# rsinghlab/GNN-Tumor-Seg

Measured on AMD Instinct MI355X. Metric: supervoxel-graphs/sec training, 7xSAGE-pool-256, 15k-node graphs, higher is better.
Workload: dtype f32; 1 GPU; C2: 7xGraphSAGE-pool-256 (8 SAGEConv), fwd+weighted-CE+bwd+AdamW, 4 x 15000-node/86350-edge lattice graphs per GPU, 4-chan feat, fp32; global_batch=4, nodes_per_batch=60000, edges_per_batch=345400, parallelism=dp1

## Files before the change

### gnn-tumor-seg_amd/csrc/gts_gemm.hip

```cpp
#include "gts_gemm_tiles.h"
#include "gts_gemm_panel.h"
#include "gts_gemm_wgrad.h"
#include "gts_gemm_small.h"

namespace gts {
namespace {

template <bool AKC, bool BKC>
int pick_plain_variant(const GemmArgs& p) {
  int variant = BKC ? g_fwd_variant : g_igrad_variant;
  if (p.rb <= 128 && variant < 9) return 0;
  const bool row_count_invariant = variant == -2;
  if (variant < 0) {
    const int64_t cols = (p.rb + 255) / 256;
    const int64_t big_tiles = static_cast<int64_t>((p.ra + 255) / 256) * cols;
    variant = big_tiles >= 192 ? 8 : 3;
    if constexpr (AKC && BKC) {
      const int h = panel_rows_for(p.ra, cols);
      const int64_t panels = static_cast<int64_t>((p.ra + h - 1) / h) * cols;
      const int64_t rows256 = (big_tiles + 255) / 256 * 256, rows_panel = (panels + 255) / 256 * h;
      if (variant == 8 && rows_panel < rows256 && !row_count_invariant) variant = 10;
      if (variant == 3 && panels >= 192 && panels <= 256 && !row_count_invariant) variant = 10;
    }
  }
  return variant;
}

template <bool BKC>
inline bool skinny_forward(const GemmArgs& p) {
  const bool automatic = BKC ? g_fwd_variant < 0 : g_igrad_variant <= 1;
  return automatic && (p.rb == 4 || p.rb == 8) && p.ldc == p.rb && p.kseg[0] + p.kseg[1] >= 64 && p.mask == nullptr &&
         p.c2 == nullptr && p.sc_l == nullptr && p.bits_out == nullptr &&
         (BKC || (p.ldb[0] == p.rb && (p.kseg[1] == 0 || p.ldb[1] == p.rb)));
}

inline bool tiny_forward(const GemmArgs& p) {
  return (p.rb == 4 || p.rb == 8) && p.ldc == p.rb && p.kseg[0] + p.kseg[1] <= 16 && p.mask == nullptr && p.c2 == nullptr &&
         p.sc_l == nullptr && p.bits_out == nullptr && g_fwd_variant < 0;
}

template <bool AKC, bool BKC>
int launch_plain_tiles(const GemmArgs& p, int variant, hipStream_t st) {
  if constexpr (AKC && BKC) {
    if (tiny_forward(p)) {
      const unsigned blocks = static_cast<unsigned>((p.ra + 255) / 256);
      if (p.rb == 4) tiny_fwd_kernel<4><<<blocks, 256, 0, st>>>(p);
      else tiny_fwd_kernel<8><<<blocks, 256, 0, st>>>(p);
      return launch_status();
    }
  }
  if constexpr (AKC) {
    if (skinny_forward<BKC>(p)) {
      const unsigned blocks = static_cast<unsigned>((p.ra + 15) / 16);
      if (p.rb == 4) skinny_fwd_kernel<4, BKC><<<blocks, 256, 0, st>>>(p);
      else skinny_fwd_kernel<8, BKC><<<blocks, 256, 0, st>>>(p);
      return launch_status();
    }
  }
  if (p.rb <= 64) return launch_tiles<128, 64, 2, 2, AKC, BKC>(p, 1, 1, st);
  if (p.rb <= 128) return launch_tiles<128, 128, 2, 2, AKC, BKC>(p, 1, 1, st);
  switch (variant) {
    case 3: return launch_tiles<64, 256, 2, 4, AKC, BKC>(p, 1, 1, st);
    case 5: return launch_tiles<256, 128, 4, 2, AKC, BKC>(p, 1, 1, st);
    case 8: return launch_tiles<256, 256, 4, 4, AKC, BKC, true>(p, 1, 1, st);
    default: return launch_tiles<128, 256, 2, 4, AKC, BKC>(p, 1, 1, st);
  }
}

template <bool AKC, bool BKC>
int launch_plain(const GemmArgs& p, hipStream_t st) {
  const int variant = pick_plain_variant<AKC, BKC>(p);
  if constexpr (AKC && BKC) {
    if (p.c2 != nullptr && !(variant == 10 && p.rb <= kC240 && p.rb2 <= kC240 && p.rb2 > 128)) {
      GemmArgs first = p, next{};
      first.c2 = nullptr;
      int rc = launch_plain<true, true>(first, st);
      if (rc != GTS_OK) return rc;
      next.a[0] = next.a[1] = p.c, next.b[0] = next.b[1] = p.b2, next.bp[0] = p.bp2;
      first.bp2 = nullptr;
      next.lda[0] = next.lda[1] = p.ldc, next.ldb[0] = next.ldb[1] = p.ldb2;
      next.kseg[0] = p.rb, next.kseg[1] = 0;
      next.ra = p.ra, next.rb = p.rb2, next.c = p.c2, next.ldc = p.ldc2, next.bias = p.bias2, next.relu = p.relu2;
      next.tiles_per_split = (p.rb + kBK - 1) / kBK;
      return launch_plain<true, true>(next, st);
    }
    if (variant == 10) {
      switch (panel_rows_for(p.ra, (p.rb + kC240 - 1) / kC240)) {
        case 144: return launch_panel_direct<3, 4, 1, NoProbe, 144>(p, st);
        case 192: return launch_panel_direct<3, 4, 1, NoProbe, 192>(p, st);
        default: return launch_panel_direct<3, 4, 1>(p, st);
      }
    }
  }
  int rc = launch_plain_tiles<AKC, BKC>(p, variant, st);
  if (rc != GTS_OK || p.bits_out == nullptr) return rc;
  const long long words = static_cast<long long>((p.ra + 3) / 4) * (p.rb >> 6);
  relu_bits_kernel<<<static_cast<unsigned>((words + 3) / 4), 256, 0, st>>>(p.c, p.bits_out, p.ra, p.rb);
  return launch_status();
}

struct PlainProblem {
  const float *a0, *b0, *a1, *b1;
  float* c;
  int64_t m, rb, k0, k1;
  bool missing() const { return !a0 || !b0 || !c || ((a1 == nullptr) != (b1 == nullptr)); }
  bool bad_shape() const {
    return m < 0 || rb <= 0 || k0 <= 0 || k1 < 0 || m >= (1LL << 31) || rb >= (1 << 20) || k0 >= (1 << 20) || k1 >= (1 << 20) ||
           !aligned4(k0) || !aligned4(k1) || (a1 && k1 == 0);
  }
  GemmArgs args(int64_t ldb0, int64_t ldb1, const float* const* packed) const {
    GemmArgs p{};
    p.a[0] = a0, p.b[0] = b0, p.lda[0] = p.kseg[0] = static_cast<int>(k0), p.ldb[0] = static_cast<int>(ldb0);
    p.a[1] = a1 ? a1 : a0, p.b[1] = b1 ? b1 : b0, p.lda[1] = static_cast<int>(k1), p.ldb[1] = static_cast<int>(ldb1);
    p.kseg[1] = a1 ? static_cast<int>(k1) : 0;
    p.ra = static_cast<int>(m), p.rb = static_cast<int>(rb), p.c = c, p.ldc = static_cast<int>(rb);
    p.tiles_per_split = (p.kseg[0] + kBK - 1) / kBK + (p.kseg[1] + kBK - 1) / kBK;
    if (packed != nullptr) p.bp[0] = packed[0], p.bp[1] = a1 ? packed[1] : nullptr;
    return p;
  }
};

void chain_second(GemmArgs* p, const float* b2, const float* bias2, float* c2, int64_t rb2, int relu2,
                  const float* const* packed) {
  p->b2 = b2, p->bias2 = bias2, p->c2 = c2, p->rb2 = static_cast<int>(rb2), p->ldb2 = p->rb;
  p->ldc2 = static_cast<int>(rb2), p->relu2 = relu2;
  if (packed != nullptr) p->bp2 = packed[2];
}

__global__ __launch_bounds__(kBlock) void sum_parts_kernel(const float* __restrict__ in_l, const float* __restrict__ in_r,
                                                           float* __restrict__ out_l, float* __restrict__ out_r,
                                                           int64_t n, int parts) {
  const int64_t i = static_cast<int64_t>(blockIdx.x) * kBlock + threadIdx.x;
  if (i >= n) return;
  float sl = 0.f, sr = 0.f;
  for (int q = 0; q < parts; ++q) sl += in_l[i * parts + q], sr += in_r[i * parts + q];
  out_l[i] = sl, out_r[i] = sr;
}

}
}

extern "C" int32_t gts_linear_fwd_f32(const float* a0, const float* w0, const float* a1, const float* w1, const float* bias,
                                      float* out, int64_t m, int64_t n, int64_t k0, int64_t k1, int32_t relu,
                                      uint64_t* relu_bits, const float* const* packed, void* stream) {
  using namespace gts;
  const PlainProblem q{a0, w0, a1, w1, out, m, n, k0, k1};
  if (q.missing()) return GTS_ERR_NULL;
  if (q.bad_shape() || (relu_bits && n % 64 != 0)) return GTS_ERR_SHAPE;
  if (m == 0) return GTS_OK;
  GemmArgs p = q.args(k0, k1, packed);
  p.bias = bias, p.relu = relu, p.bits_out = reinterpret_cast<unsigned long long*>(relu_bits);
  return launch_plain<true, true>(p, static_cast<hipStream_t>(stream));
}

extern "C" int32_t gts_relu_bits_pay(int64_t m, int64_t n) {
  using namespace gts;
  if (m <= 0 || n <= 0 || n % 64 != 0 || m >= (1LL << 31) || n >= (1 << 20)) return 0;
  GemmArgs p{};
  p.ra = static_cast<int>(m), p.rb = static_cast<int>(n);
  const int variant = pick_plain_variant<true, true>(p);
  return variant >= 10 && variant <= 12 ? 1 : 0;
}

extern "C" int64_t gts_relu_bits_bytes(int64_t m, int64_t n) {
  if (m < 0 || n <= 0 || n % 64 != 0) return 0;
  return (m + 3) / 4 * (n / 64) * 4 * static_cast<int64_t>(sizeof(uint64_t));
}

extern "C" int64_t gts_gat_fc_scores_workspace(int64_t m, int64_t heads, int64_t dim) {
  if (m <= 0 || heads <= 0 || dim <= 0 || dim % 64 != 0) return 0;
  return 2 * m * heads * (dim / 64) * static_cast<int64_t>(sizeof(float));
}

extern "C" int32_t gts_gat_fc_scores_f32(const float* h, const float* w_fc, const float* attn_l, const float* attn_r,
                                         float* ft, float* el, float* er, float* workspace, int64_t workspace_bytes,
                                         int64_t m, int64_t heads, int64_t dim, int64_t k, const float* w_fc_packed,
                                         void* stream) {
  using namespace gts;
  const int64_t n = heads * dim;
  const float* const packed[2] = {w_fc_packed, nullptr};
  const PlainProblem q{h, w_fc, nullptr, nullptr, ft, m, n, k, 0};
  if (q.missing() || !attn_l || !attn_r || !el || !er) return GTS_ERR_NULL;
  if (q.bad_shape() || heads <= 0 || dim <= 0) return GTS_ERR_SHAPE;
  if (m == 0) return GTS_OK;
  GemmArgs p = q.args(k, 0, packed);
  hipStream_t st = static_cast<hipStream_t>(stream);
  const int parts = static_cast<int>(dim / 64);
  const bool fuse = dim % 64 == 0 && pick_plain_variant<true, true>(p) == 10 &&
                    (parts == 1 || (workspace && workspace_bytes >= gts_gat_fc_scores_workspace(m, heads, dim)));
  if (!fuse) {
    const int rc = launch_plain<true, true>(p, st);
    return rc != GTS_OK ? rc : gts_gat_scores_f32(ft, attn_l, attn_r, el, er, m, heads, dim, stream);
  }
  p.sc_l = attn_l, p.sc_r = attn_r;
  p.sc_el = parts == 1 ? el : workspace, p.sc_er = parts == 1 ? er : workspace + m * heads * parts;
  const int rc = launch_plain<true, true>(p, st);
  if (rc != GTS_OK || parts == 1) return rc;
  const int64_t rows = m * heads;
  sum_parts_kernel<<<static_cast<unsigned>((rows + kBlock - 1) / kBlock), kBlock, 0, st>>>(p.sc_el, p.sc_er, el, er, rows, parts);
  return launch_status();
}

extern "C" int32_t gts_linear_fwd_chain_f32(const float* a0, const float* w0, const float* a1, const float* w1,
                                            const float* bias, float* out, const float* w2, const float* bias2, float* out2,
                                            int64_t m, int64_t n, int64_t k0, int64_t k1, int32_t relu, int64_t n2,
                                            int32_t relu2, uint64_t* relu_bits, const float* const* packed, void* stream) {
  using namespace gts;
  const PlainProblem q{a0, w0, a1, w1, out, m, n, k0, k1};
  if (q.missing() || !w2 || !out2) return GTS_ERR_NULL;
  if (q.bad_shape() || n2 <= 0 || n2 >= (1 << 20) || !aligned4(n) || (relu_bits && n % 64 != 0)) return GTS_ERR_SHAPE;
  if (m == 0) return GTS_OK;
  GemmArgs p = q.args(k0, k1, packed);
  p.bias = bias, p.relu = relu, p.bits_out = reinterpret_cast<unsigned long long*>(relu_bits);
  chain_second(&p, w2, bias2, out2, n2, relu2, packed);
  return launch_plain<true, true>(p, static_cast<hipStream_t>(stream));
}

extern "C" int32_t gts_linear_bwd_input_chain_t_f32(const float* g0, const float* w0t, const float* g1, const float* w1t,
                                                    const float* relu_mask, const uint64_t* relu_bits, float* gin,
                                                    const float* w2t, float* gin2, int64_t m, int64_t k, int64_t n0,
                                                    int64_t n1, int64_t k2, const float* const* packed, void* stream) {
  using namespace gts;
  const PlainProblem q{g0, w0t, g1, w1t, gin, m, k, n0, n1};
  if (q.missing() || !w2t || !gin2 || (relu_bits && !relu_mask)) return GTS_ERR_NULL;
  if (q.bad_shape() || k2 <= 0 || k2 >= (1 << 20) || !aligned4(k) || (relu_bits && k % 64 != 0)) return GTS_ERR_SHAPE;
  if (m == 0) return GTS_OK;
  GemmArgs p = q.args(n0, n1, packed);
  p.mask = relu_mask, p.bits_in = reinterpret_cast<const unsigned long long*>(relu_bits);
  chain_second(&p, w2t, nullptr, gin2, k2, 0, packed);
  return launch_plain<true, true>(p, static_cast<hipStream_t>(stream));
}

extern "C" int32_t gts_linear_bwd_input_f32(const float* g0, const float* w0, const float* g1, const float* w1,
                                            const float* relu_mask, float* gin, int64_t m, int64_t k, int64_t n0,
                                            int64_t n1, void* stream) {
  using namespace gts;
  const PlainProblem q{g0, w0, g1, w1, gin, m, k, n0, n1};
  if (q.missing()) return GTS_ERR_NULL;
  if (q.bad_shape() || !aligned4(k)) return GTS_ERR_SHAPE;
  if (m == 0) return GTS_OK;
  GemmArgs p = q.args(k, k, nullptr);
  p.mask = relu_mask;
  return launch_plain<true, false>(p, static_cast<hipStream_t>(stream));
}

extern "C" int32_t gts_linear_bwd_input_t_f32(const float* g0, const float* w0t, const float* g1, const float* w1t,
                                              const float* relu_mask, const uint64_t* relu_bits, float* gin, int64_t m,
                                              int64_t k, int64_t n0, int64_t n1, const float* const* packed, void* stream) {
  using namespace gts;
  const PlainProblem q{g0, w0t, g1, w1t, gin, m, k, n0, n1};
  if (q.missing() || (relu_bits && !relu_mask)) return GTS_ERR_NULL;
  if (q.bad_shape() || !aligned4(k) || (relu_bits && k % 64 != 0)) return GTS_ERR_SHAPE;
  if (m == 0) return GTS_OK;
  GemmArgs p = q.args(n0, n1, packed);
  p.mask = relu_mask, p.bits_in = reinterpret_cast<const unsigned long long*>(relu_bits);
  return launch_plain<true, true>(p, static_cast<hipStream_t>(stream));
}

static bool act_fold_in_epilogue(const gts::GemmArgs& p) {
  return gts::pick_plain_variant<true, true>(p) == 10 && p.rb % gts::kC240 == 0;
}

extern "C" int64_t gts_linear_bwd_input_t_act_workspace(int64_t m, int64_t k) {
  if (m <= 0 || k <= 0) return 0;
  const int64_t row_blocks = (m + 143) / 144 * 3;
  const int64_t pass = gts_gat_reduce_workspace(m, k) / 2;
  const int64_t fold = row_blocks * k * static_cast<int64_t>(sizeof(float));
  return fold > pass ? fold : pass;
}

extern "C" int32_t gts_linear_bwd_input_t_act_f32(const float* g0, const float* w0t, const float* g1, const float* w1t,
                                                  const float* act_out, int32_t activation, float* gin, float* g_bias,
                                                  float* workspace, int64_t workspace_bytes, int64_t m, int64_t k,
                                                  int64_t n0, int64_t n1, const float* const* packed, void* stream) {
  using namespace gts;
  const PlainProblem q{g0, w0t, g1, w1t, gin, m, k, n0, n1};
  if (q.missing() || !act_out || (g_bias && !workspace)) return GTS_ERR_NULL;
  if (activation != 1 && activation != 2) return GTS_ERR_ARGKIND;
  if (q.bad_shape() || !aligned4(k)) return GTS_ERR_SHAPE;
  if (g_bias && workspace_bytes < gts_linear_bwd_input_t_act_workspace(m, k)) return GTS_ERR_SHAPE;
  if (m == 0) return GTS_OK;
  hipStream_t st = static_cast<hipStream_t>(stream);
  GemmArgs p = q.args(n0, n1, packed);
  if (activation == 1 && g_bias && act_fold_in_epilogue(p)) {
    const int rows = panel_rows_for(p.ra, p.rb / kC240);
    const int row_blocks = (p.ra + rows - 1) / rows * 3;
    p.mask = act_out, p.mask_kind = 1, p.col_partial = workspace;
    const int rc = launch_plain<true, true>(p, st);
    if (rc != GTS_OK) return rc;
    return sum_chunks(workspace, g_bias, p.rb, row_blocks, st);
  }
  const int rc = launch_plain<true, true>(p, st);
  if (rc != GTS_OK) return rc;
  return gts_gat_act_bwd_f32(gin, act_out, activation, gin, g_bias, workspace, workspace_bytes, m, k, stream);
}

extern "C" int64_t gts_linear_bwd_weight_workspace(int64_t m, int64_t n, int64_t k, int32_t n_problems) {
  using namespace gts;
  if (m <= 0 || n <= 0 || k <= 0 || n_problems < 1 || n_problems > kMaxProblems) return 0;
  const int64_t splits = wgrad_plan(m, n, k, n_problems).splits;
  const int64_t slabs = n_problems * splits * (n * k + n);
  const int64_t skinny = skinny_workspace_floats(m, n, k) + kSkinnyChunks * (n < k ? n : 0);
  return (slabs > skinny ? slabs : skinny) * static_cast<int64_t>(sizeof(float));
}

extern "C" int32_t gts_linear_bwd_weight_f32(const float* const* g, const float* const* a, float* const* gw,
                                             float* const* gb, int32_t n_problems, float* workspace,
                                             int64_t workspace_bytes, int64_t m, int64_t n, int64_t k, void* stream) {
  using namespace gts;
  if (!g || !a || !gw || !workspace) return GTS_ERR_NULL;
  if (n_problems < 1 || n_problems > kMaxProblems) return GTS_ERR_ARGKIND;
  if (m <= 0 || n <= 0 || k <= 0 || m >= (1LL << 31) || n >= (1 << 20) || k >= (1 << 20) || !aligned4(n) || !aligned4(k))
    return GTS_ERR_SHAPE;
  if (workspace_bytes < gts_linear_bwd_weight_workspace(m, n, k, n_problems)) return GTS_ERR_SHAPE;
  bool any_bias = false;
  for (int q = 0; q < n_problems; ++q) {
    if (!g[q] || !a[q] || !gw[q]) return GTS_ERR_NULL;
    any_bias = any_bias || (gb && gb[q]);
  }
  hipStream_t st = static_cast<hipStream_t>(stream);
  if (skinny_workspace_floats(m, n, k) > 0) {
    for (int q = 0; q < n_problems; ++q)
      skinny_wgrad(g[q], a[q], gw[q], gb ? gb[q] : nullptr, workspace, m, n, k, st);
    return launch_status();
  }
  const WgradPlan plan = wgrad_plan(m, n, k, n_problems);
  const int splits = plan.splits;
  const int tiles = static_cast<int>((m + kBK - 1) / kBK);
  GemmArgs p{};
  for (int q = 0; q < n_problems; ++q) p.pa[q] = g[q], p.pb[q] = a[q];
  p.a[0] = p.a[1] = g[0], p.b[0] = p.b[1] = a[0];
  p.lda[0] = p.lda[1] = static_cast<int>(n), p.ldb[0] = p.ldb[1] = static_cast<int>(k);
  p.kseg[0] = static_cast<int>(m), p.kseg[1] = 0;
  p.ra = static_cast<int>(n), p.rb = static_cast<int>(k);
  p.c = workspace, p.ldc = static_cast<int>(k);
  p.colsum = any_bias ? workspace + static_cast<size_t>(n_problems) * splits * n * k : nullptr;
  for (int q = 0; q < n_problems && any_bias; ++q)
    if (gb[q]) p.colsum_mask |= 1u << q;
  p.n_problems = n_problems, p.n_splits = splits;
  p.tiles_per_split = (tiles + splits - 1) / splits;
  int rc = launch_wgrad(p, plan, st);
  if (rc != GTS_OK) return rc;
  ReduceArgs r{};
  r.splits = splits;
  int jobs = 0;
  for (int q = 0; q < n_problems; ++q, ++jobs) {
    r.slabs[jobs] = workspace + static_cast<size_t>(q) * splits * n * k;
    r.out[jobs] = gw[q], r.n4[jobs] = static_cast<int>(n * k / 4);
  }
  for (int q = 0; q < n_problems && any_bias; ++q) {
    if (!gb[q]) continue;
    r.slabs[jobs] = p.colsum + static_cast<size_t>(q) * splits * n;
    r.out[jobs] = gb[q], r.n4[jobs] = static_cast<int>(n / 4);
    ++jobs;
  }
  reduce_slabs_kernel<<<dim3(static_cast<unsigned>((n * k / 4 + 63) / 64), jobs), kBlock, 0, st>>>(r);
  return launch_status();
}
```

### gnn-tumor-seg_amd/csrc/gts_gemm_args.h

```cpp
#pragma once
#include "gts_common.h"

namespace gts {

inline int g_gemm_sched = 1;
inline int g_fwd_variant = -1;
inline int g_igrad_variant = 1;
inline int g_wgrad_variant = -1;
inline int g_panel_rows = 0;

namespace {

typedef float v16f __attribute__((ext_vector_type(16)));
typedef float v4f __attribute__((ext_vector_type(4)));

constexpr int kBK = 32;
constexpr int kMaxProblems = 32;
constexpr unsigned kOutOfRange = 0x7FFFFFF0u;

struct GemmArgs {
  const float* a[2];
  const float* b[2];
  int lda[2], ldb[2];
  int kseg[2];
  int ra, rb;
  float* c;
  int ldc;
  const float* bias;
  int relu;
  const float* mask;
  const float* pa[kMaxProblems];
  const float* pb[kMaxProblems];
  float* colsum;
  unsigned colsum_mask;
  int n_problems;
  int tiles_n;
  int n_splits;
  int tiles_per_split;
  int sched;
  const float* b2;
  const float* bias2;
  float* c2;
  int rb2, ldb2, ldc2, relu2;
  const float* sc_l;
  const float* sc_r;
  float* sc_el;
  float* sc_er;
  unsigned long long* bits_out;
  const unsigned long long* bits_in;
  int mask_kind;
  float* col_partial;
  const float* bp[2];
  const float* bp2;
};

struct NoProbe {
  __device__ __forceinline__ static void mark(int ) {}
};

inline bool aligned4(int64_t x) { return (x & 3) == 0; }

}
}
```

### gnn-tumor-seg_amd/csrc/gts_gemm_skinny.h

```cpp
#pragma once
#include "gts_gemm_args.h"

namespace gts {
namespace {

constexpr int kSkinnyMax = 9;
constexpr int kSkinnyChunks = 512;

template <int S>
__global__ __launch_bounds__(kBlock) void skinny_wgrad_kernel(const float* __restrict__ skinny, int s_cols,
                                                             const float* __restrict__ wide,
                                                             float* __restrict__ partial, int64_t m,
                                                             int w, int64_t rows_per_chunk) {
  __shared__ v4f red[kBlock];
  const int cols4 = w >> 2;
  const int lanes = cols4 >= kBlock ? 1 : kBlock / cols4;
  const int rl = cols4 >= kBlock ? 0 : threadIdx.x / cols4;
  const int64_t row0 = blockIdx.x * rows_per_chunk, row1 = min(m, row0 + rows_per_chunk);
  for (int q0 = 0; q0 < cols4; q0 += kBlock) {
    const int q = q0 + (cols4 >= kBlock ? threadIdx.x : threadIdx.x % cols4);
    const bool live = q < cols4 && rl < lanes;
    v4f acc[S];
#pragma unroll
    for (int i = 0; i < S; ++i) acc[i] = v4f{0.f, 0.f, 0.f, 0.f};
    if (live) {
#pragma unroll 4
      for (int64_t row = row0 + rl; row < row1; row += lanes) {
        const v4f f = *reinterpret_cast<const v4f*>(wide + static_cast<size_t>(row) * w + 4 * q);
#pragma unroll
        for (int i = 0; i < S; ++i) acc[i] += (i < s_cols ? skinny[row * s_cols + i] : 1.0f) * f;
      }
    }
#pragma unroll
    for (int i = 0; i < S; ++i) {
      v4f total = acc[i];
      if (lanes > 1) {
        __syncthreads();
        red[threadIdx.x] = acc[i];
        __syncthreads();
        if (rl == 0 && live) {
          for (int l = 1; l < lanes; ++l) total += red[l * cols4 + q];
        }
      }
      if (rl == 0 && live)
        *reinterpret_cast<v4f*>(partial + (static_cast<size_t>(blockIdx.x) * S + i) * w + 4 * q) = total;
    }
  }
}

__global__ __launch_bounds__(kBlock) void skinny_sum_kernel(const float* __restrict__ partial,
                                                           float* __restrict__ dst0,
                                                           float* __restrict__ dst1, int rows, int s_cols,
                                                           int w, int chunks, int transposed) {
  __shared__ float part[16][16];
  const int o = threadIdx.x & 15, lane = threadIdx.x >> 4;
  const int idx = blockIdx.x * 16 + o;
  const int total_out = rows * w;
  float acc = 0.f;
  if (idx < total_out) {
#pragma unroll 8
    for (int c = lane; c < chunks; c += 16) acc += partial[static_cast<size_t>(c) * total_out + idx];
  }
  part[lane][o] = acc;
  __syncthreads();
  if (lane != 0 || idx >= total_out) return;
  float sum = part[0][o];
#pragma unroll
  for (int l = 1; l < 16; ++l) sum += part[l][o];
  const int i = idx / w, j = idx - i * w;
  if (i < s_cols)
    dst0[transposed ? j * s_cols + i : i * w + j] = sum;
  else if (dst1 != nullptr)
    dst1[j] = sum;
}

}
}
```

### gnn-tumor-seg_amd/csrc/gts_gemm_wgrad.h

```cpp
#pragma once
#include <type_traits>

#include "gts_gemm_tiles.h"

namespace gts {
namespace {

typedef float v2f __attribute__((ext_vector_type(2)));

template <int O0, int O1>
__device__ __forceinline__ v2f lds_read2st64(unsigned addr) {
  static_assert(O0 >= 0 && O1 <= 255, "ds_read2st64_b32 offsets are 8 bits");
  v2f r;
  asm volatile("ds_read2st64_b32 %0, %1 offset0:%2 offset1:%3" : "=v"(r) : "v"(addr), "n"(O0), "n"(O1));
  return r;
}

template <class Probe = NoProbe>
__global__ __launch_bounds__(1024, 4) void wgrad_stream_kernel(const GemmArgs p) {
  constexpr int BM = 256, BN = 256, WM = 4, WN = 4, WTM = 64, WTN = 64, TM = 2, TN = 2;
  constexpr int kPlane = kBK * BM;
  static_assert(BM == BN && kPlane * 4 == 128 * 256, "image I of an operand sits 128 offset units above image 0");
  __shared__ float lds[4 * kPlane];
  const int lane = threadIdx.x & 63, wave = __builtin_amdgcn_readfirstlane(threadIdx.x >> 6);
  const int wm = wave / WN, wn = wave % WN;
  const int i = lane & 31, h = lane >> 5;
  const int problem = blockIdx.y / p.tiles_n, tile_n = blockIdx.y % p.tiles_n;
  const int m0 = blockIdx.x * BM, n0 = tile_n * BN;
  const float* g = kernarg_entry<const float*>(offsetof(GemmArgs, pa), problem);
  const float* act = kernarg_entry<const float*>(offsetof(GemmArgs, pb), problem);
  const int ldg = p.lda[0], lda = p.ldb[0];
  const int n_tiles_all = (p.kseg[0] + kBK - 1) / kBK;
  const int t_beg = min(n_tiles_all, static_cast<int>(blockIdx.z) * p.tiles_per_split);
  const int t_end = min(n_tiles_all, t_beg + p.tiles_per_split);
  const int row_beg = t_beg * kBK, rows = min(p.kseg[0], t_end * kBK) - row_beg;
  const int n_tiles = t_end - t_beg;
  const bool g_ok = m0 + 4 * lane < p.ra, a_ok = n0 + 4 * lane < p.rb;
  const unsigned vg0 = g_ok ? static_cast<unsigned>(wave * ldg + m0 + 4 * lane) * 4 : kOutOfRange;
  const unsigned vg1 = g_ok ? static_cast<unsigned>((wave + 16) * ldg + m0 + 4 * lane) * 4 : kOutOfRange;
  const unsigned va0 = a_ok ? static_cast<unsigned>(wave * lda + n0 + 4 * lane) * 4 : kOutOfRange;
  const unsigned va1 = a_ok ? static_cast<unsigned>((wave + 16) * lda + n0 + 4 * lane) * 4 : kOutOfRange;
  auto dma = [&](int t, int image) __attribute__((always_inline)) {
    const int r0 = row_beg + t * kBK, nr = min(kBK, rows - t * kBK);
    __amdgpu_buffer_rsrc_t rg = __builtin_amdgcn_make_buffer_rsrc(const_cast<float*>(g + static_cast<size_t>(r0) * ldg), 0,
                                                                  nr * ldg * 4, 0x00020000);
    __amdgpu_buffer_rsrc_t ract = __builtin_amdgcn_make_buffer_rsrc(const_cast<float*>(act + static_cast<size_t>(r0) * lda), 0,
                                                                    nr * lda * 4, 0x00020000);
    float* ia = lds + image * kPlane + wave * BM;
    float* ib = lds + (2 + image) * kPlane + wave * BN;
    __builtin_amdgcn_raw_ptr_buffer_load_lds(rg, ia, 16, vg0, 0, 0, 0);
    __builtin_amdgcn_raw_ptr_buffer_load_lds(rg, ia + 16 * BM, 16, vg1, 0, 0, 0);
    __builtin_amdgcn_raw_ptr_buffer_load_lds(ract, ib, 16, va0, 0, 0, 0);
    __builtin_amdgcn_raw_ptr_buffer_load_lds(ract, ib + 16 * BN, 16, va1, 0, 0, 0);
  };

  v16f acc[TM][TN];
#pragma unroll
  for (int tm = 0; tm < TM; ++tm)
#pragma unroll
    for (int tn = 0; tn < TN; ++tn)
#pragma unroll
      for (int r = 0; r < 16; ++r) acc[tm][tn][r] = 0.f;
  float csum[TM] = {0.f, 0.f};
  const bool want_colsum = p.colsum != nullptr && tile_n == 0 && wn == wm && ((p.colsum_mask >> problem) & 1u) != 0;

  const unsigned lds0 = static_cast<unsigned>(reinterpret_cast<uintptr_t>((__attribute__((address_space(3))) float*)lds));
  const unsigned a_addr0 = lds0 + static_cast<unsigned>(4 * h * BM + wm * WTM + i) * 4, a_addr1 = a_addr0 + 128;
  const unsigned b_addr0 = lds0 + static_cast<unsigned>(2 * kPlane + 4 * h * BN + wn * WTN + i) * 4, b_addr1 = b_addr0 + 128;
  v2f fa[2][TM], fb[2][TN];
  fa[0][0] = fa[0][1] = fa[1][0] = fa[1][1] = v2f{0.f, 0.f};
  fb[0][0] = fb[0][1] = fb[1][0] = fb[1][1] = v2f{0.f, 0.f};

  auto issue = [&](auto img_c, auto pair_c) __attribute__((always_inline)) {
    constexpr int IMG = decltype(img_c)::value, Q = decltype(pair_c)::value;
    constexpr int O = 4 * (8 * (Q / 2) + 2 * (Q % 2)) + 128 * IMG;
    fa[Q & 1][0] = lds_read2st64<O, O + 4>(a_addr0);
    fa[Q & 1][1] = lds_read2st64<O, O + 4>(a_addr1);
    fb[Q & 1][0] = lds_read2st64<O, O + 4>(b_addr0);
    fb[Q & 1][1] = lds_read2st64<O, O + 4>(b_addr1);
  };
  auto multiply = [&](int slot) __attribute__((always_inline)) {
#pragma unroll
    for (int e = 0; e < 2; ++e)
#pragma unroll
      for (int tm = 0; tm < TM; ++tm)
#pragma unroll
        for (int tn = 0; tn < TN; ++tn)
          acc[tm][tn] = __builtin_amdgcn_mfma_f32_32x32x2f32(fa[slot][tm][e], fb[slot][tn][e], acc[tm][tn], 0, 0, 0);
  };
  float half_sum[TM] = {0.f, 0.f};
  auto tile = [&](auto img_c, auto cs_c, int t) __attribute__((always_inline)) {
    constexpr int IMG = decltype(img_c)::value;
    constexpr bool CS = decltype(cs_c)::value;
    auto pair = [&](auto pair_c) __attribute__((always_inline)) {
      constexpr int Q = decltype(pair_c)::value, S = Q & 1;
      if constexpr (Q < 7) {
        issue(img_c, std::integral_constant<int, Q + 1>{});
        asm volatile("s_waitcnt lgkmcnt(4)" : "+v"(fa[S][0]), "+v"(fa[S][1]), "+v"(fb[S][0]), "+v"(fb[S][1]));
      } else {
        asm volatile("s_waitcnt vmcnt(0) lgkmcnt(0)\n\ts_barrier"
                     : "+v"(fa[S][0]), "+v"(fa[S][1]), "+v"(fb[S][0]), "+v"(fb[S][1]) : : "memory");
        if (t + 2 < n_tiles) dma(t + 2, IMG);
        if (t + 1 < n_tiles) issue(std::integral_constant<int, IMG ^ 1>{}, std::integral_constant<int, 0>{});
      }
      if constexpr (Q % 2 == 0) {
        if constexpr (Q == 0) __builtin_amdgcn_s_setprio(3);
        else if constexpr (Q == 2) __builtin_amdgcn_s_setprio(2);
        else if constexpr (Q == 4) __builtin_amdgcn_s_setprio(1);
        else __builtin_amdgcn_s_setprio(0);
      }
      if constexpr (CS) {
#pragma unroll
        for (int tm = 0; tm < TM; ++tm) {
          if constexpr (Q % 2 == 0) {
            asm volatile("v_add_f32 %0, %1, %2" : "=v"(half_sum[tm]) : "v"(fa[S][tm][0]), "v"(fa[S][tm][1]));
          } else {
            float upper;
            asm volatile("v_add_f32 %0, %1, %2" : "=v"(upper) : "v"(fa[S][tm][0]), "v"(fa[S][tm][1]));
            asm volatile("v_add_f32 %0, %1, %2" : "=v"(upper) : "v"(half_sum[tm]), "v"(upper));
            asm volatile("v_add_f32 %0, %1, %2" : "+v"(csum[tm]) : "v"(csum[tm]), "v"(upper));
          }
        }
      }
      multiply(S);
    };
    pair(std::integral_constant<int, 0>{}), pair(std::integral_constant<int, 1>{}), pair(std::integral_constant<int, 2>{}),
        pair(std::integral_constant<int, 3>{}), pair(std::integral_constant<int, 4>{}), pair(std::integral_constant<int, 5>{}),
        pair(std::integral_constant<int, 6>{}), pair(std::integral_constant<int, 7>{});
  };
  auto reduce = [&](auto cs_c) __attribute__((always_inline)) {
    int t = 0;
    for (; t + 1 < n_tiles; t += 2) {
      tile(std::integral_constant<int, 0>{}, cs_c, t);
      tile(std::integral_constant<int, 1>{}, cs_c, t + 1);
    }
    if (t < n_tiles) tile(std::integral_constant<int, 0>{}, cs_c, t);
  };

  Probe::mark(0);
  if (n_tiles > 0) {
    dma(0, 0);
    if (n_tiles > 1) dma(1, 1);
    asm volatile("s_waitcnt vmcnt(0)\n\ts_barrier" ::: "memory");
    issue(std::integral_constant<int, 0>{}, std::integral_constant<int, 0>{});
  }
  Probe::mark(1);
  if (want_colsum) reduce(std::true_type{});
  else reduce(std::false_type{});
  __builtin_amdgcn_s_setprio(0);
  Probe::mark(2);
  const size_t slab = static_cast<size_t>(problem) * p.n_splits + blockIdx.z;
  write_tile<BM, BN, WM, WN>(p, lds, p.c + slab * p.ra * p.ldc, acc, m0, n0);
  Probe::mark(3);
  if (want_colsum) {
#pragma unroll
    for (int tm = 0; tm < TM; ++tm) {
      const float total = csum[tm] + __shfl_xor(csum[tm], 32, kWave);
      const int row = m0 + wm * WTM + tm * 32 + i;
      if (h == 0 && row < p.ra) p.colsum[slab * p.ra + row] = total;
    }
  }
}

struct ReduceArgs {
  const float* slabs[2 * kMaxProblems];
  float* out[2 * kMaxProblems];
  int n4[2 * kMaxProblems];
  int splits;
};

__global__ __launch_bounds__(kBlock) void reduce_slabs_kernel(const ReduceArgs p) {
  __shared__ v4f part[4][64];
  const int col = threadIdx.x & 63, grp = threadIdx.x >> 6;
  const int q = blockIdx.y;
  const float* slabs = kernarg_entry<const float*>(offsetof(ReduceArgs, slabs), q);
  float* out = kernarg_entry<float*>(offsetof(ReduceArgs, out), q);
  const int n4 = kernarg_entry<int>(offsetof(ReduceArgs, n4), q);
  const int i = blockIdx.x * 64 + col;
  if (blockIdx.x * 64 >= n4) return;
  v4f acc = {0.f, 0.f, 0.f, 0.f};
  if (i < n4) {
    const v4f* src = reinterpret_cast<const v4f*>(slabs) + i;
#pragma unroll 8
    for (int s = grp; s < p.splits; s += 4) acc += src[static_cast<size_t>(s) * n4];
  }
  part[grp][col] = acc;
  __syncthreads();
  if (grp == 0 && i < n4) {
    const v4f total = (part[0][col] + part[1][col]) + (part[2][col] + part[3][col]);
    reinterpret_cast<v4f*>(out)[i] = total;
  }
}

}
}
#include "gts_gemm_skinny.h"
namespace gts {
namespace {

inline int64_t skinny_workspace_floats(int64_t m, int64_t n, int64_t k) {
  const int64_t small = n < k ? n : k, big = n < k ? k : n;
  if (small + 1 > kSkinnyMax || big < 64) return 0;
  return static_cast<int64_t>(kSkinnyChunks) * (small + 1) * big;
}

template <int S>
void launch_skinny(const float* skinny, int s_cols, const float* wide, float* partial, int64_t m, int w,
                   int chunks, int64_t rpc, hipStream_t st) {
  skinny_wgrad_kernel<S><<<chunks, kBlock, 0, st>>>(skinny, s_cols, wide, partial, m, w, rpc);
}

inline bool skinny_wgrad(const float* g, const float* a, float* gw, float* gb, float* workspace, int64_t m,
                  int64_t n, int64_t k, hipStream_t st) {
  if (skinny_workspace_floats(m, n, k) == 0) return false;
  const bool g_is_skinny = n < k;
  const float* skinny = g_is_skinny ? g : a;
  const float* wide = g_is_skinny ? a : g;
  const int s_cols = static_cast<int>(g_is_skinny ? n : k), w = static_cast<int>(g_is_skinny ? k : n);
  const bool ones_row = !g_is_skinny && gb != nullptr;
  const int rows = s_cols + (ones_row ? 1 : 0);
  const int64_t rpc = (m + kSkinnyChunks - 1) / kSkinnyChunks;
  const int chunks = static_cast<int>((m + rpc - 1) / rpc);
  switch (rows) {
    case 1: launch_skinny<1>(skinny, s_cols, wide, workspace, m, w, chunks, rpc, st); break;
    case 2: launch_skinny<2>(skinny, s_cols, wide, workspace, m, w, chunks, rpc, st); break;
    case 3: launch_skinny<3>(skinny, s_cols, wide, workspace, m, w, chunks, rpc, st); break;
    case 4: launch_skinny<4>(skinny, s_cols, wide, workspace, m, w, chunks, rpc, st); break;
    case 5: launch_skinny<5>(skinny, s_cols, wide, workspace, m, w, chunks, rpc, st); break;
    case 6: launch_skinny<6>(skinny, s_cols, wide, workspace, m, w, chunks, rpc, st); break;
    case 7: launch_skinny<7>(skinny, s_cols, wide, workspace, m, w, chunks, rpc, st); break;
    case 8: launch_skinny<8>(skinny, s_cols, wide, workspace, m, w, chunks, rpc, st); break;
    default: launch_skinny<9>(skinny, s_cols, wide, workspace, m, w, chunks, rpc, st); break;
  }
  skinny_sum_kernel<<<(rows * w + 15) / 16, kBlock, 0, st>>>(
      workspace, gw, ones_row ? gb : nullptr, rows, s_cols, w, chunks, g_is_skinny ? 0 : 1);
  if (g_is_skinny && gb != nullptr) {
    float* part = workspace + static_cast<size_t>(chunks) * rows * w;
    skinny_wgrad_kernel<1><<<chunks, kBlock, 0, st>>>(nullptr, 0, g, part, m, static_cast<int>(n), rpc);
    skinny_sum_kernel<<<(static_cast<int>(n) + 15) / 16, kBlock, 0, st>>>(
        part, nullptr, gb, 1, 0, static_cast<int>(n), chunks, 0);
  }
  return true;
}

struct WgradPlan {
  int variant, bm, bn, splits;
};

inline void wgrad_candidate(int variant, int64_t k, int* bm, int* bn, int64_t* slots) {
  *bm = 128, *bn = k <= 64 ? 64 : 128, *slots = 512;
  if (k <= 64) return;
  if (variant == 2) *bn = 256;
  if (variant == 4 || variant == 6) *bm = 256, *bn = 256, *slots = 256;
}

inline WgradPlan wgrad_plan(int64_t m, int64_t n, int64_t k, int n_problems) {
  const int64_t tiles = (m + kBK - 1) / kBK;
  static const int kMany[2] = {6, 2};
  static const int kFewLarge[2] = {6, 1};
  const bool few = n_problems <= 4;
  const bool large = n * k * n_problems >= (1 << 20);
  const int n_candidates = g_wgrad_variant >= 0 || (few && !large) ? 1 : 2;
  WgradPlan best{};
  double best_fill = -1.0;
  for (int c = 0; c < n_candidates; ++c) {
    WgradPlan plan{};
    plan.variant = g_wgrad_variant >= 0 ? g_wgrad_variant : (few ? (large ? kFewLarge[c] : 1) : kMany[c]);
    int64_t slots;
    wgrad_candidate(plan.variant, k, &plan.bm, &plan.bn, &slots);
    const int64_t out_tiles = ((n + plan.bm - 1) / plan.bm) * ((k + plan.bn - 1) / plan.bn) * n_problems;
    int64_t splits = out_tiles >= slots ? 1 : slots / out_tiles;
    if (splits > tiles) splits = tiles;
    plan.splits = static_cast<int>(splits < 1 ? 1 : splits);
    const int64_t groups = out_tiles * plan.splits;
    const int64_t rounds = (groups + slots - 1) / slots;
    const double fill = static_cast<double>(groups) / static_cast<double>(rounds * slots);
    if (fill > best_fill + 1e-9) best = plan, best_fill = fill;
  }
  return best;
}

inline int launch_wgrad(const GemmArgs& p, const WgradPlan& plan, hipStream_t st) {
  const int np = p.n_problems, splits = plan.splits;
  if (p.rb <= 64) return launch_tiles<128, 64, 2, 2, false, false>(p, np, splits, st);
  switch (plan.variant) {
    case 2: return launch_tiles<128, 256, 2, 4, false, false>(p, np, splits, st);
    case 4: return launch_tiles<256, 256, 4, 4, false, false, true>(p, np, splits, st);
    case 6: {
      GemmArgs q = p;
      q.tiles_n = (p.rb + 255) / 256;
      dim3 grid((p.ra + 255) / 256, q.tiles_n * np, splits);
      wgrad_stream_kernel<><<<grid, 1024, 0, st>>>(q);
      return launch_status();
    }
    default: return launch_tiles<128, 128, 2, 4, false, false>(p, np, splits, st);
  }
}

}
}
```

### gnn-tumor-seg_amd/csrc/gts_narrow.hip

```cpp
#include "gts_gemm_skinny.h"

namespace gts {
namespace {

constexpr int kFirstW = 256, kFirstS = 4;

__global__ __launch_bounds__(kBlock) void first_layer_bwd_kernel(const float* __restrict__ g, const float* __restrict__ x,
                                                                const float* __restrict__ m0,
                                                                const float* __restrict__ w_neigh, float* __restrict__ gm,
                                                                float* __restrict__ part_x, float* __restrict__ part_m,
                                                                int64_t m, int64_t rows_per_chunk) {
  constexpr int W = kFirstW, S = kFirstS;
  __shared__ v4f red[kWavesPerBlock - 1][2 * S + 1][kWave];
  const int lane = threadIdx.x & (kWave - 1), rl = threadIdx.x / kWave;
  const int64_t row0 = blockIdx.x * rows_per_chunk, row1 = min(m, row0 + rows_per_chunk);
  v4f wn[S];
#pragma unroll
  for (int e = 0; e < 4; ++e) {
    const v4f t = *reinterpret_cast<const v4f*>(w_neigh + static_cast<size_t>(4 * lane + e) * S);
#pragma unroll
    for (int j = 0; j < S; ++j) wn[j][e] = t[j];
  }
  v4f ax[S + 1], am[S];
#pragma unroll
  for (int i = 0; i <= S; ++i) ax[i] = v4f{0.f, 0.f, 0.f, 0.f};
#pragma unroll
  for (int i = 0; i < S; ++i) am[i] = v4f{0.f, 0.f, 0.f, 0.f};
  const bool upper32 = (lane & 32) != 0, upper16 = (lane & 16) != 0;
  auto take_row = [&](int64_t row, const v4f f, const v4f xs, const v4f ms) __attribute__((always_inline)) {
#pragma unroll
    for (int i = 0; i < S; ++i) ax[i] += xs[i] * f;
    ax[S] += 1.0f * f;
#pragma unroll
    for (int i = 0; i < S; ++i) am[i] += ms[i] * f;
    float d[S];
#pragma unroll
    for (int n = 0; n < S; ++n) {
      d[n] = 0.f;
#pragma unroll
      for (int e = 0; e < 4; ++e) d[n] = __builtin_fmaf(f[e], wn[n][e], d[n]);
    }
    const float keep0 = upper32 ? d[2] : d[0], keep1 = upper32 ? d[3] : d[1];
    const float send0 = upper32 ? d[0] : d[2], send1 = upper32 ? d[1] : d[3];
    const float a = keep0 + __shfl_xor(send0, 32, kWave), b = keep1 + __shfl_xor(send1, 32, kWave);
    float c = (upper16 ? b : a) + __shfl_xor(upper16 ? a : b, 16, kWave);
#pragma unroll
    for (int o = 8; o > 0; o >>= 1) c += __shfl_xor(c, o, kWave);
    if ((lane & 15) == 0) gm[static_cast<size_t>(row) * S + (lane >> 4)] = c;
  };
  constexpr int kAhead = 4;
  for (int64_t first = row0 + rl; first < row1; first += kAhead * kWavesPerBlock) {
    v4f f[kAhead], xs[kAhead], ms[kAhead];
#pragma unroll
    for (int u = 0; u < kAhead; ++u) {
      const int64_t row = first + u * kWavesPerBlock < row1 ? first + u * kWavesPerBlock : first;
      f[u] = *reinterpret_cast<const v4f*>(g + static_cast<size_t>(row) * W + 4 * lane);
      xs[u] = *reinterpret_cast<const v4f*>(x + static_cast<size_t>(row) * S);
      ms[u] = *reinterpret_cast<const v4f*>(m0 + static_cast<size_t>(row) * S);
    }
#pragma unroll
    for (int u = 0; u < kAhead; ++u)
      if (first + u * kWavesPerBlock < row1) take_row(first + u * kWavesPerBlock, f[u], xs[u], ms[u]);
  }
  if (rl > 0) {
#pragma unroll
    for (int i = 0; i <= S; ++i) red[rl - 1][i][lane] = ax[i];
#pragma unroll
    for (int i = 0; i < S; ++i) red[rl - 1][S + 1 + i][lane] = am[i];
  }
  __syncthreads();
  if (rl != 0) return;
#pragma unroll
  for (int i = 0; i <= S; ++i) {
    v4f total = ax[i];
    for (int l = 1; l < kWavesPerBlock; ++l) total += red[l - 1][i][lane];
    *reinterpret_cast<v4f*>(part_x + (static_cast<size_t>(blockIdx.x) * (S + 1) + i) * W + 4 * lane) = total;
  }
#pragma unroll
  for (int i = 0; i < S; ++i) {
    v4f total = am[i];
    for (int l = 1; l < kWavesPerBlock; ++l) total += red[l - 1][S + 1 + i][lane];
    *reinterpret_cast<v4f*>(part_m + (static_cast<size_t>(blockIdx.x) * S + i) * W + 4 * lane) = total;
  }
}

inline bool first_layer_shape(int64_t m, int64_t w, int64_t s0, int64_t s1) {
  return m > 0 && m < (1LL << 31) && w == kFirstW && s0 == kFirstS && s1 == kFirstS;
}

}
}

extern "C" int64_t gts_sage_first_layer_bwd_workspace(int64_t m, int64_t w, int64_t s0, int64_t s1) {
  using namespace gts;
  if (!first_layer_shape(m, w, s0, s1)) return 0;
  return static_cast<int64_t>(kSkinnyChunks) * (s0 + 1 + s1) * w * static_cast<int64_t>(sizeof(float));
}

extern "C" int32_t gts_sage_first_layer_bwd_f32(const float* g, const float* x, const float* m0, const float* w_neigh,
                                                float* gm, float* gw_self, float* g_bias, float* gw_neigh,
                                                float* workspace, int64_t workspace_bytes, int64_t m, int64_t w,
                                                int64_t s0, int64_t s1, void* stream) {
  using namespace gts;
  if (!g || !x || !m0 || !w_neigh || !gm || !gw_self || !g_bias || !gw_neigh || !workspace) return GTS_ERR_NULL;
  if (!first_layer_shape(m, w, s0, s1)) return GTS_ERR_SHAPE;
  if (workspace_bytes < gts_sage_first_layer_bwd_workspace(m, w, s0, s1)) return GTS_ERR_SHAPE;
  hipStream_t st = static_cast<hipStream_t>(stream);
  const int64_t rpc = (m + kSkinnyChunks - 1) / kSkinnyChunks;
  const int chunks = static_cast<int>((m + rpc - 1) / rpc);
  const int W = kFirstW, S = kFirstS;
  float* part_x = workspace;
  float* part_m = workspace + static_cast<size_t>(chunks) * (S + 1) * W;
  first_layer_bwd_kernel<<<chunks, kBlock, 0, st>>>(g, x, m0, w_neigh, gm, part_x, part_m, m, rpc);
  skinny_sum_kernel<<<((S + 1) * W + 15) / 16, kBlock, 0, st>>>(part_x, gw_self, g_bias, S + 1, S, W, chunks, 1);
  skinny_sum_kernel<<<(S * W + 15) / 16, kBlock, 0, st>>>(part_m, gw_neigh, nullptr, S, S, W, chunks, 1);
  return launch_status();
}
```

### gnn-tumor-seg_amd/csrc/gts_optim.hip

```cpp
#include "gts_common.h"

namespace gts {
namespace {

typedef float v4f __attribute__((ext_vector_type(4)));

struct AdamWConsts {
  float decay;
  float w1;
  float beta2, w2;
  float step_size;
  float inv_bc2_sqrt_den;
  float eps;
};

__device__ __forceinline__ void adamw_one(float& p, float g, float& m, float& v, const AdamWConsts& c) {
  p = p * c.decay;
  m = m + c.w1 * (g - m);
  v = c.beta2 * v + c.w2 * (g * g);
  const float denom = sqrtf(v) / c.inv_bc2_sqrt_den + c.eps;
  p = p - c.step_size * (m / denom);
}

__global__ __launch_bounds__(kBlock) void adamw_kernel(float* __restrict__ param,
                                                      const float* __restrict__ grad,
                                                      float* __restrict__ exp_avg,
                                                      float* __restrict__ exp_avg_sq, int64_t n,
                                                      AdamWConsts c, int vector_ok) {
  const int64_t n4 = vector_ok ? n / 4 : 0;
  for (int64_t q = static_cast<int64_t>(blockIdx.x) * kBlock + threadIdx.x; q < n4;
       q += static_cast<int64_t>(gridDim.x) * kBlock) {
    v4f p = reinterpret_cast<v4f*>(param)[q];
    const v4f g = reinterpret_cast<const v4f*>(grad)[q];
    v4f m = reinterpret_cast<v4f*>(exp_avg)[q];
    v4f v = reinterpret_cast<v4f*>(exp_avg_sq)[q];
#pragma unroll
    for (int e = 0; e < 4; ++e) {
      float pe = p[e], me = m[e], ve = v[e];
      adamw_one(pe, g[e], me, ve, c);
      p[e] = pe, m[e] = me, v[e] = ve;
    }
    reinterpret_cast<v4f*>(param)[q] = p;
    reinterpret_cast<v4f*>(exp_avg)[q] = m;
    reinterpret_cast<v4f*>(exp_avg_sq)[q] = v;
  }
  for (int64_t i = 4 * n4 + static_cast<int64_t>(blockIdx.x) * kBlock + threadIdx.x; i < n;
       i += static_cast<int64_t>(gridDim.x) * kBlock)
    adamw_one(param[i], grad[i], exp_avg[i], exp_avg_sq[i], c);
}

}
}

extern "C" int32_t gts_adamw_f32(float* param, const float* grad, float* exp_avg, float* exp_avg_sq,
                                 int64_t n, double lr, double beta1, double beta2, double eps,
                                 double weight_decay, int64_t step, void* stream) {
  using namespace gts;
  if (n < 0 || step < 1 || !(beta1 >= 0.0 && beta1 < 1.0) || !(beta2 >= 0.0 && beta2 < 1.0))
    return GTS_ERR_SHAPE;
  if (n == 0) return GTS_OK;
  if (!param || !grad || !exp_avg || !exp_avg_sq) return GTS_ERR_NULL;
  const double bc1 = 1.0 - pow(beta1, static_cast<double>(step));
  const double bc2 = 1.0 - pow(beta2, static_cast<double>(step));
  AdamWConsts c;
  c.decay = static_cast<float>(1.0 - lr * weight_decay);
  c.w1 = static_cast<float>(1.0 - beta1);
  c.beta2 = static_cast<float>(beta2);
  c.w2 = static_cast<float>(1.0 - beta2);
  c.step_size = static_cast<float>(lr / bc1);
  c.inv_bc2_sqrt_den = static_cast<float>(sqrt(bc2));
  c.eps = static_cast<float>(eps);
  const int vector_ok = ((reinterpret_cast<uintptr_t>(param) | reinterpret_cast<uintptr_t>(grad) |
                          reinterpret_cast<uintptr_t>(exp_avg) | reinterpret_cast<uintptr_t>(exp_avg_sq)) & 15) == 0;
  int64_t blocks = (n / 4 + kBlock - 1) / kBlock;
  blocks = blocks < 1 ? 1 : (blocks > 4096 ? 4096 : blocks);
  adamw_kernel<<<static_cast<unsigned>(blocks), kBlock, 0, static_cast<hipStream_t>(stream)>>>(
      param, grad, exp_avg, exp_avg_sq, n, c, vector_ok);
  return launch_status();
}
```

### gnn-tumor-seg_amd/csrc/gts_stack.hip

```cpp
#include <algorithm>
#include <vector>

#include "gts_gemm_args.h"

namespace {

constexpr int kMaxLayers = 64;

inline int64_t align256(int64_t bytes) { return (bytes + 255) & ~255LL; }

inline bool bad_stack(int64_t n_rows, const int64_t* widths, int32_t n_layers) {
  if (!widths || n_layers < 1 || n_layers > kMaxLayers || n_rows < 0 || n_rows >= (1LL << 31)) return true;
  for (int i = 0; i <= n_layers; ++i)
    if (widths[i] <= 0 || widths[i] % 4 != 0 || widths[i] >= (1 << 20)) return true;
  return false;
}

struct FwdPlan {
  int64_t m[kMaxLayers], arg[kMaxLayers], out[kMaxLayers], bits[kMaxLayers];
  int64_t p[2];
  int64_t wp[kMaxLayers][3];
  int64_t counters;
  int64_t total;
};

inline bool packs(int64_t out_cols) { return out_cols > 128; }

inline FwdPlan plan_forward(int64_t n, const int64_t* w, int n_layers, bool training, int arg_bytes, bool relu_bits) {
  FwdPlan p{};
  int64_t at = 0, widest = 0;
  auto take = [&](int64_t bytes) { const int64_t o = at; at += align256(bytes); return o; };
  for (int i = 0; i < n_layers; ++i) {
    const bool last = i == n_layers - 1;
    widest = std::max(widest, w[i]);
    p.m[i] = take(4 * n * w[i]);
    p.arg[i] = training ? take(static_cast<int64_t>(arg_bytes) * n * w[i]) : -1;
    p.out[i] = take(4 * n * w[i + 1]);
    const bool bits = relu_bits && training && !last && gts_relu_bits_pay(n, w[i + 1]) == 1;
    p.bits[i] = bits ? take(gts_relu_bits_bytes(n, w[i + 1])) : -1;
  }
  p.p[0] = take(4 * n * widest);
  p.p[1] = take(4 * n * widest);
  for (int i = 0; i < n_layers; ++i) {
    p.wp[i][0] = packs(w[i]) ? take(4 * gts_packed_weight_floats(w[i], w[i])) : -1;
    p.wp[i][1] = packs(w[i + 1]) ? take(4 * gts_packed_weight_floats(w[i + 1], w[i])) : -1;
    p.wp[i][2] = packs(w[i + 1]) ? take(4 * gts_packed_weight_floats(w[i + 1], w[i])) : -1;
  }
  p.counters = take(4 * GTS_CLUSTER_COUNTER_WORDS);
  p.total = at;
  return p;
}

inline bool chainable(int64_t n, int64_t k0, int64_t k1, int64_t n2) {
  return n % 4 == 0 && k0 % 4 == 0 && k1 % 4 == 0 && n <= 256 && n2 <= 256;
}

inline bool turns(int64_t rows, int64_t cols) { return cols >= 128 && rows % 4 == 0 && cols % 4 == 0; }

struct BwdPlan {
  int64_t wt[kMaxLayers][3];
  int64_t wtp[kMaxLayers][3];
  int64_t g[kMaxLayers], gp[kMaxLayers];
  int64_t gm[2];
  int64_t workspace, workspace_bytes;
  bool first_fused;
  int64_t counters;
  int64_t total;
};

struct ByShape {
  struct Group {
    int64_t rows, cols;
    std::vector<const float*> in[2];
    std::vector<float*> out[2];
    int count() const { return static_cast<int>(in[0].size()); }
  };
  std::vector<Group> groups;
  void add(int64_t rows, int64_t cols, const float* in0, const float* in1, float* out0, float* out1) {
    auto it = std::find_if(groups.begin(), groups.end(), [&](const Group& c) { return c.rows == rows && c.cols == cols; });
    if (it == groups.end()) it = groups.insert(it, Group{rows, cols, {}, {}});
    it->in[0].push_back(in0), it->in[1].push_back(in1), it->out[0].push_back(out0), it->out[1].push_back(out1);
  }
};

constexpr int kWeightSlot[3] = {0, 2, 3};
inline int64_t weight_rows(const int64_t* w, int i, int q) { return q == 0 ? w[i] : w[i + 1]; }

inline BwdPlan plan_backward(int64_t n, const int64_t* w, int n_layers) {
  BwdPlan p{};
  int64_t at = 0, widest = 0;
  auto take = [&](int64_t bytes) { const int64_t o = at; at += align256(bytes); return o; };
  ByShape wgrads;
  for (int i = 0; i < n_layers; ++i) {
    const int64_t fin = w[i];
    widest = std::max(widest, fin);
    for (int q = 0; q < 3; ++q) p.wt[i][q] = turns(weight_rows(w, i, q), fin) ? take(4 * weight_rows(w, i, q) * fin) : -1;
    for (int q = 0; q < 3; ++q)
      p.wtp[i][q] = p.wt[i][q] >= 0 ? take(4 * gts_packed_weight_floats(fin, weight_rows(w, i, q))) : -1;
    p.g[i] = i > 0 ? take(4 * n * fin) : -1;
    p.gp[i] = take(4 * n * fin);
    for (int q = 0; q < 3; ++q) wgrads.add(weight_rows(w, i, q), fin, nullptr, nullptr, nullptr, nullptr);
  }
  p.gm[0] = take(4 * n * widest);
  p.gm[1] = take(4 * n * widest);
  int64_t ws = 0;
  if (n > 0)
    for (const auto& grp : wgrads.groups)
      for (int first = 0; first < grp.count(); first += gts::kMaxProblems)
        ws = std::max(ws, gts_linear_bwd_weight_workspace(n, grp.rows, grp.cols, std::min(gts::kMaxProblems, grp.count() - first)));
  const int64_t first = n > 0 ? gts_sage_first_layer_bwd_workspace(n, w[1], w[0], w[0]) : 0;
  p.first_fused = first > 0;
  ws = std::max(ws, first);
  p.workspace_bytes = ws;
  p.workspace = take(ws);
  p.counters = take(4 * GTS_CLUSTER_COUNTER_WORDS);
  p.total = at;
  return p;
}

inline int32_t zero_counters(const int32_t* sched_rec, int64_t clusters, int32_t rows, int32_t srcs, int32_t loc_words,
                             int32_t backward, void* at, void* stream, uint32_t** counters) {
  *counters = nullptr;
  if (sched_rec == nullptr || gts_cluster_uses_counters(clusters, rows, srcs, loc_words, backward) == 0) return GTS_OK;
  if (hipMemsetAsync(at, 0, 4 * GTS_CLUSTER_COUNTER_WORDS, static_cast<hipStream_t>(stream)) != hipSuccess) return gts::launch_status();
  *counters = static_cast<uint32_t*>(at);
  return GTS_OK;
}

#define GTS_TRY(call)                    \
  do {                                   \
    const int32_t code_ = (call);        \
    if (code_ != GTS_OK) return code_;   \
  } while (0)

}

extern "C" int64_t gts_sage_pool_stack_fwd_arena(int64_t n_rows, const int64_t* widths, int32_t n_layers, int32_t training,
                                                 int32_t arg_bytes, int32_t relu_bits, int64_t* offsets) {
  if (bad_stack(n_rows, widths, n_layers) || (training && arg_bytes != 1 && arg_bytes != 4)) return -1;
  const FwdPlan p = plan_forward(n_rows, widths, n_layers, training != 0, arg_bytes, relu_bits != 0);
  if (offsets != nullptr) {
    for (int i = 0; i < n_layers; ++i)
      offsets[4 * i] = p.m[i], offsets[4 * i + 1] = p.arg[i], offsets[4 * i + 2] = p.out[i], offsets[4 * i + 3] = p.bits[i];
    offsets[4 * n_layers] = p.p[0], offsets[4 * n_layers + 1] = p.p[1];
  }
  return p.total;
}

extern "C" int32_t gts_sage_pool_stack_fwd_f32(const int32_t* indptr, const int32_t* indices, const int32_t* sched_rec,
                                               int64_t sched_clusters, int32_t sched_rows, int32_t sched_srcs,
                                               int32_t sched_loc_words, const float* x, const float* const* params,
                                               int64_t n_rows, const int64_t* widths, int32_t n_layers, int32_t training,
                                               int32_t arg_bytes, int32_t relu_bits, void* arena, int64_t arena_bytes,
                                               void* stream) {
  if (!indptr || !x || !params || !arena) return GTS_ERR_NULL;
  if (bad_stack(n_rows, widths, n_layers)) return GTS_ERR_SHAPE;
  if (training && arg_bytes != 1 && arg_bytes != 4) return GTS_ERR_ARGKIND;
  for (int i = 0; i < 5 * n_layers; ++i)
    if (!params[i]) return GTS_ERR_NULL;
  const bool train = training != 0;
  const FwdPlan plan = plan_forward(n_rows, widths, n_layers, train, arg_bytes, relu_bits != 0);
  if (arena_bytes < plan.total) return GTS_ERR_SHAPE;
  if (n_rows == 0) return GTS_OK;
  char* base = static_cast<char*>(arena);
  auto f32 = [&](int64_t off) { return reinterpret_cast<float*>(base + off); };
  uint32_t* counters;
  GTS_TRY(zero_counters(sched_rec, sched_clusters, sched_rows, sched_srcs, sched_loc_words, 0, base + plan.counters, stream, &counters));
  {
    ByShape packs;
    for (int i = 0; i < n_layers; ++i)
      for (int q = 0; q < 3; ++q)
        if (plan.wp[i][q] >= 0)
          packs.add(weight_rows(widths, i, q), widths[i], params[5 * i + kWeightSlot[q]], nullptr, f32(plan.wp[i][q]), nullptr);
    for (const auto& b : packs.groups)
      GTS_TRY(gts_pack_weights_f32(b.in[0].data(), b.out[0].data(), nullptr, b.count(), b.rows, b.cols, 0, stream));
  }
  auto wp = [&](int i, int q) -> const float* { return plan.wp[i][q] >= 0 ? f32(plan.wp[i][q]) : nullptr; };
  const float* h = x;
  float* p = nullptr;
  int cur = 0;
  for (int i = 0; i < n_layers; ++i) {
    const float* w_pool = params[5 * i];
    const float* b_pool = params[5 * i + 1];
    const float* w_self = params[5 * i + 2];
    const float* w_neigh = params[5 * i + 3];
    const float* bias = params[5 * i + 4];
    const int64_t fin = widths[i], fout = widths[i + 1];
    const bool last = i == n_layers - 1;
    if (p == nullptr) {
      p = f32(plan.p[cur]);
      const float* packed[2] = {wp(i, 0), nullptr};
      GTS_TRY(gts_linear_fwd_f32(h, w_pool, nullptr, nullptr, b_pool, p, n_rows, fin, fin, 0, 1, nullptr, packed, stream));
    }
    float* m = f32(plan.m[i]);
    void* arg = train ? static_cast<void*>(base + plan.arg[i]) : nullptr;
    const int ab = train ? arg_bytes : 0;
    if (sched_rec != nullptr && fin == 256 && ab != 4 && n_rows * 1024 < (1LL << 32)) {
      GTS_TRY(gts_spmm_max_fwd_cluster_f32(sched_rec, sched_clusters, sched_rows, sched_srcs, sched_loc_words, p, m, arg, ab,
                                           1, n_rows, fin, counters, stream));
    } else {
      GTS_TRY(gts_spmm_max_fwd_f32(indptr, indices, p, m, arg, ab, 1, n_rows, fin, stream));
    }
    uint64_t* bits = plan.bits[i] >= 0 ? reinterpret_cast<uint64_t*>(base + plan.bits[i]) : nullptr;
    float* out = f32(plan.out[i]);
    if (!last && chainable(fout, fin, fin, fout)) {
      float* p_next = f32(plan.p[cur ^ 1]);
      const float* packed[3] = {wp(i, 1), wp(i, 2), wp(i + 1, 0)};
      GTS_TRY(gts_linear_fwd_chain_f32(h, w_self, m, w_neigh, bias, out, params[5 * (i + 1)], params[5 * (i + 1) + 1], p_next,
                                       n_rows, fout, fin, fin, 1, fout, 1, bits, packed, stream));
      p = p_next, cur ^= 1;
    } else {
      const float* packed[2] = {wp(i, 1), wp(i, 2)};
      GTS_TRY(gts_linear_fwd_f32(h, w_self, m, w_neigh, bias, out, n_rows, fout, fin, fin, last ? 0 : 1, bits, packed, stream));
      p = nullptr;
    }
    h = out;
  }
  return GTS_OK;
}

extern "C" int64_t gts_sage_pool_stack_bwd_scratch(int64_t n_rows, const int64_t* widths, int32_t n_layers,
                                                   int32_t ) {
  if (bad_stack(n_rows, widths, n_layers)) return -1;
  return plan_backward(n_rows, widths, n_layers).total;
}

extern "C" int32_t gts_sage_pool_stack_bwd_f32(const int32_t* t_indptr, const int32_t* t_indices, const int32_t* t_slot,
                                               const int32_t* sched_rec, int64_t sched_clusters, int32_t sched_rows,
                                               int32_t sched_srcs, int32_t sched_loc_words, const float* gout, const float* x,
                                               const float* const* params, int64_t n_rows, const int64_t* widths,
                                               int32_t n_layers, int32_t arg_bytes, int32_t relu_bits, const void* fwd_arena,
                                               float* const* grads, float* gx, void* scratch, int64_t scratch_bytes,
                                               void* stream) {
  if (!t_indptr || !gout || !x || !params || !fwd_arena || !grads || !scratch) return GTS_ERR_NULL;
  if (bad_stack(n_rows, widths, n_layers)) return GTS_ERR_SHAPE;
  if (arg_bytes != 1 && arg_bytes != 4) return GTS_ERR_ARGKIND;
  for (int i = 0; i < 5 * n_layers; ++i)
    if (!params[i] || !grads[i]) return GTS_ERR_NULL;
  hipStream_t st = static_cast<hipStream_t>(stream);
  if (n_rows == 0) {
    for (int i = 0; i < n_layers; ++i) {
      const int64_t fin = widths[i], fout = widths[i + 1];
      const int64_t sizes[5] = {fin * fin, fin, fout * fin, fout * fin, fout};
      for (int q = 0; q < 5; ++q)
        if (hipMemsetAsync(grads[5 * i + q], 0, 4 * sizes[q], st) != hipSuccess) return gts::launch_status();
    }
    return GTS_OK;
  }
  const FwdPlan fwd = plan_forward(n_rows, widths, n_layers, true, arg_bytes, relu_bits != 0);
  const BwdPlan plan = plan_backward(n_rows, widths, n_layers);
  if (scratch_bytes < plan.total) return GTS_ERR_SHAPE;
  const char* acts = static_cast<const char*>(fwd_arena);
  char* base = static_cast<char*>(scratch);
  auto f32 = [&](int64_t off) { return reinterpret_cast<float*>(base + off); };
  uint32_t* counters;
  GTS_TRY(zero_counters(sched_rec, sched_clusters, sched_rows, sched_srcs, sched_loc_words, 1, base + plan.counters, stream, &counters));
  auto act = [&](int64_t off) { return reinterpret_cast<const float*>(acts + off); };
  auto input_of = [&](int i) { return i == 0 ? x : act(fwd.out[i - 1]); };

  {
    ByShape turned;
    for (int i = 0; i < n_layers; ++i)
      for (int q = 0; q < 3; ++q)
        if (plan.wt[i][q] >= 0)
          turned.add(weight_rows(widths, i, q), widths[i], params[5 * i + kWeightSlot[q]], nullptr, f32(plan.wt[i][q]),
                     f32(plan.wtp[i][q]));
    for (const auto& b : turned.groups)
      GTS_TRY(gts_pack_weights_f32(b.in[0].data(), b.out[1].data(), b.out[0].data(), b.count(), b.rows, b.cols, 1, stream));
  }
  auto wt = [&](int i, int q) -> const float* { return plan.wt[i][q] >= 0 ? f32(plan.wt[i][q]) : nullptr; };
  auto wtp = [&](int i, int q) -> const float* { return plan.wtp[i][q] >= 0 ? f32(plan.wtp[i][q]) : nullptr; };

  auto igrad = [&](const float* g0, const float* w0, const float* w0t, int64_t n0, const float* g1, const float* w1,
                   const float* w1t, int64_t n1, const float* relu_mask, const uint64_t* relu_bits, float* gin,
                   int64_t k, const float* w0tp, const float* w1tp) -> int32_t {
    if (w0t != nullptr && (g1 == nullptr || w1t != nullptr)) {
      const float* packed[2] = {w0tp, g1 ? w1tp : nullptr};
      return gts_linear_bwd_input_t_f32(g0, w0t, g1, g1 ? w1t : nullptr, relu_mask, relu_mask ? relu_bits : nullptr, gin,
                                        n_rows, k, n0, g1 ? n1 : 0, packed, stream);
    }
    return gts_linear_bwd_input_f32(g0, w0, g1, g1 ? w1 : nullptr, relu_mask, gin, n_rows, k, n0, g1 ? n1 : 0, stream);
  };

  ByShape wgrads;

  const float* g = gout;
  const float* gm = nullptr;
  int cur = 0;
  for (int i = n_layers - 1; i >= 0; --i) {
    const float* w_pool = params[5 * i];
    const float* w_self = params[5 * i + 2];
    const float* w_neigh = params[5 * i + 3];
    const int64_t fin = widths[i], fout = widths[i + 1];
    const float* h = input_of(i);
    const float* m = act(fwd.m[i]);
    const void* arg = acts + fwd.arg[i];
    const bool fused = i == 0 && plan.first_fused && gm == nullptr;
    const bool lowrank = i == n_layers - 1 && gm == nullptr && fout == 4 && fin == 256 && arg_bytes == 1;
    if (fused) {
      float* buf = f32(plan.gm[cur]);
      GTS_TRY(gts_sage_first_layer_bwd_f32(g, h, m, w_neigh, buf, grads[2], grads[4], grads[3], f32(plan.workspace),
                                           plan.workspace_bytes, n_rows, fout, fin, fin, stream));
      gm = buf;
    } else if (gm == nullptr && !lowrank) {
      float* buf = f32(plan.gm[cur]);
      GTS_TRY(igrad(g, w_neigh, wt(i, 2), fout, nullptr, nullptr, nullptr, 0, nullptr, nullptr, buf, fin, wtp(i, 2), nullptr));
      gm = buf;
    }
    float* gp = f32(plan.gp[i]);
    if (lowrank) {
      GTS_TRY(gts_spmm_max_bwd_lowrank_f32(t_indptr, t_indices, t_slot, g, w_neigh, arg, arg_bytes, gp, n_rows, fin, fout, stream));
    } else if (sched_rec != nullptr && fin == 256 && arg_bytes == 1 && n_rows * 1024 < (1LL << 32)) {
      GTS_TRY(gts_spmm_max_bwd_cluster_f32(sched_rec, sched_clusters, sched_rows, sched_srcs, sched_loc_words, gm, arg, 1, gp,
                                           n_rows, fin, counters, stream));
    } else {
      GTS_TRY(gts_spmm_max_bwd_f32(t_indptr, t_indices, t_slot, gm, arg, arg_bytes, nullptr, gp, n_rows, fin, stream));
    }
    gm = nullptr;
    wgrads.add(fin, fin, gp, h, grads[5 * i], grads[5 * i + 1]);
    if (!fused) {
      wgrads.add(fout, fin, g, h, grads[5 * i + 2], grads[5 * i + 4]);
      wgrads.add(fout, fin, g, m, grads[5 * i + 3], nullptr);
    }
    if (i > 0) {
      const int64_t below_in = widths[i - 1];
      const uint64_t* hbits = fwd.bits[i - 1] >= 0 ? reinterpret_cast<const uint64_t*>(acts + fwd.bits[i - 1]) : nullptr;
      float* g_next = f32(plan.g[i]);
      const float* below_t = wt(i - 1, 2);
      if (wt(i, 1) && wt(i, 0) && below_t && chainable(fin, fout, fin, below_in)) {
        float* gm_next = f32(plan.gm[cur ^ 1]);
        const float* packed[3] = {wtp(i, 1), wtp(i, 0), wtp(i - 1, 2)};
        GTS_TRY(gts_linear_bwd_input_chain_t_f32(g, wt(i, 1), gp, wt(i, 0), h, hbits, g_next, below_t, gm_next, n_rows, fin,
                                                 fout, fin, below_in, packed, stream));
        gm = gm_next, cur ^= 1;
      } else {
        GTS_TRY(igrad(g, w_self, wt(i, 1), fout, gp, w_pool, wt(i, 0), fin, h, hbits, g_next, fin, wtp(i, 1), wtp(i, 0)));
      }
      g = g_next;
    } else if (gx != nullptr) {
      GTS_TRY(igrad(g, w_self, wt(i, 1), fout, gp, w_pool, wt(i, 0), fin, nullptr, nullptr, gx, fin, wtp(i, 1), wtp(i, 0)));
    }
  }
  for (const auto& grp : wgrads.groups)
    for (int first = 0; first < grp.count(); first += gts::kMaxProblems)
      GTS_TRY(gts_linear_bwd_weight_f32(grp.in[0].data() + first, grp.in[1].data() + first, grp.out[0].data() + first,
                                        grp.out[1].data() + first, std::min(gts::kMaxProblems, grp.count() - first),
                                        f32(plan.workspace), plan.workspace_bytes, n_rows, grp.rows, grp.cols, stream));
  return GTS_OK;
}
```

### gnn-tumor-seg_amd/gts/dist.py

```python
import os

import torch
import torch.distributed as dist


COLLECTIVE_TIMER = None


def world():
    if dist.is_available() and dist.is_initialized():
        return dist.get_rank(), dist.get_world_size()
    return 0, 1


def init_from_env(backend=None):
    world_size = int(os.environ.get("WORLD_SIZE", "1"))
    rank = int(os.environ.get("RANK", "0"))
    local_rank = int(os.environ.get("LOCAL_RANK", "0"))
    use_gpu = torch.cuda.is_available()
    if use_gpu:
        local_rank = local_rank % torch.cuda.device_count()
        torch.cuda.set_device(local_rank)
    if world_size > 1 and not dist.is_initialized():
        os.environ.setdefault("MASTER_ADDR", "127.0.0.1")
        os.environ.setdefault("MASTER_PORT", "29500")
        os.environ.setdefault("HSA_ENABLE_IPC_MODE_LEGACY", "0")
        backend = backend or os.environ.get("GTS_DIST_BACKEND") or ("nccl" if use_gpu else "gloo")
        kwargs = {}
        if use_gpu and backend == "nccl":
            kwargs["device_id"] = torch.device("cuda", local_rank)
        dist.init_process_group(backend, rank=rank, world_size=world_size, **kwargs)
    return rank, world_size, local_rank


def shard_indices(perm, step, per_rank, rank, world_size, costs=None):
    g = per_rank * world_size
    chunk = list(perm[step * g:(step + 1) * g])
    if costs is None or world_size == 1:
        return chunk[rank::world_size]
    order = sorted(range(len(chunk)), key=lambda k: (-costs[chunk[k]], k))
    load, held = [0] * world_size, [[] for _ in range(world_size)]
    for k in order:
        r = min((r for r in range(world_size) if len(held[r]) < per_rank), key=lambda r: (load[r], r))
        held[r].append(k)
        load[r] += costs[chunk[k]]
    return [chunk[k] for k in sorted(held[rank])]


def sample_costs(dataset):
    indices = None
    while hasattr(dataset, "dataset") and hasattr(dataset, "indices"):
        own = list(dataset.indices)
        indices = own if indices is None else [own[i] for i in indices]
        dataset = dataset.dataset
    fn = getattr(dataset, "sample_costs", None)
    if fn is None:
        return None
    costs = list(fn())
    return costs if indices is None else [costs[i] for i in indices]


def rank_share(n_items):
    rank, w = world()
    return list(range(rank, n_items, w))


def gather_rows_in_order(n_items, mine):
    _, w = world()
    if w == 1:
        everyone = [mine]
    else:
        everyone = [None] * w
        dist.all_gather_object(everyone, mine)
    rows = {}
    for part in everyone:
        rows.update(part)
    missing = [i for i in range(n_items) if i not in rows]
    if missing:
        raise RuntimeError(f"items {missing[:8]} were evaluated by no rank")
    return [rows[i] for i in range(n_items)]


def broadcast_object(obj, src=0):
    if world()[1] == 1:
        return obj
    box = [obj]
    dist.broadcast_object_list(box, src=src)
    return box[0]


def assert_same_layout(params, what="parameters"):
    rank, w = world()
    if w == 1:
        return
    mine = [tuple(p.shape) for p in params]
    everyone = [None] * w
    dist.all_gather_object(everyone, mine)
    bad = [r for r, shapes in enumerate(everyone) if shapes != everyone[0]]
    if bad:
        raise RuntimeError(f"{what} differ between ranks: rank 0 holds {len(everyone[0])} tensors, "
                           f"ranks {bad} hold {[len(everyone[r]) for r in bad]} (or other shapes); "
                           "build the model from ONE set of hyper-parameters (gts.dist.broadcast_object)")


def broadcast_parameters(params, src=0):
    params = list(params)
    assert_same_layout(params)
    for p in params:
        dist.broadcast(p.data, src=src)


class FlatGradSync:

    def __init__(self, params, group=None):
        self.params = [p for p in params if p.requires_grad]
        if not self.params:
            raise ValueError("no trainable parameters")
        dev = self.params[0].device
        for p in self.params:
            if p.dtype != torch.float32 or p.device != dev:
                raise ValueError("FlatGradSync needs fp32 parameters on one device")
        self.n_grad = sum(p.numel() for p in self.params)
        self.group = group
        self.flat = None
        self._scalars = None
        self._sink = None

    def flat_gradients(self):
        if self.flat is None:
            raise RuntimeError("call all_reduce_and_normalise() first")
        return self.flat[:self.n_grad]

    def zero_grad(self):
        for p in self.params:
            p.grad = None

    def weighted_ce_backward(self, logits, labels, class_weights, cross_entropy_sum=None):
        if cross_entropy_sum is not None:
            num, den = cross_entropy_sum(logits, labels, class_weights)
            num.backward()
            self._scalars = (den.detach().reshape(1), num.detach().reshape(1))
            return
        from . import nn, ops
        grad, stats = ops.weighted_ce_numerator_grad(logits, labels, class_weights)
        if self._sink is None:
            self._sink = nn.GradSink(self.params, extra=2)
        self._sink.new_buffer()
        with nn.grad_sink(self._sink):
            logits.backward(grad)
        self._scalars = (stats[1:2], stats[0:1])

    def empty_step(self, device=None):
        for p in self.params:
            p.grad = None
        if self._sink is not None:
            self._sink.filled = False
        zeros = torch.zeros(2, dtype=torch.float32, device=device or self.params[0].device)
        self._scalars = (zeros[0:1], zeros[1:2])

    def all_reduce_and_normalise(self):
        if self._scalars is None:
            raise RuntimeError("call weighted_ce_backward() first")
        if self._sink is not None and self._sink.filled:
            self.flat = self._sink.flat
            self.flat[self.n_grad:self.n_grad + 1].copy_(self._scalars[0])
            self.flat[self.n_grad + 1:].copy_(self._scalars[1])
            self._sink.filled = False
        else:
            pieces = [(p.grad if p.grad is not None else torch.zeros_like(p)).reshape(-1) for p in self.params]
            self.flat = torch.cat(pieces + [t.to(pieces[0].dtype) for t in self._scalars])
        self._scalars = None
        _, w = world()
        if w > 1:
            reduce = lambda: dist.all_reduce(self.flat, op=dist.ReduceOp.SUM, group=self.group)
            if COLLECTIVE_TIMER is not None:
                COLLECTIVE_TIMER(reduce)
            else:
                reduce()
        den = self.flat[self.n_grad]
        loss = self.flat[self.n_grad + 1] / den
        self.flat[:self.n_grad].div_(den)
        off = 0
        for p in self.params:
            p.grad = self.flat[off:off + p.numel()].view_as(p)
            off += p.numel()
        return loss
```

### gnn-tumor-seg_amd/gts/nn.py

```python
import os

import torch
import torch.nn as nn
import torch.nn.functional as F

from . import dense, ops
from .graph import _DeviceSchedule


class GraphError(RuntimeError):
    """Counterpart of dgl.DGLError for the checks the layers make."""


def _is_relu(fn):
    return fn in (F.relu, torch.relu, torch.nn.functional.relu)


class _SagePoolLayer(torch.autograd.Function):

    @staticmethod
    def forward(ctx, g, h, w_pool, b_pool, w_self, w_neigh, bias, relu_out, need_bwd):
        h = h.contiguous()
        p = dense.linear_fwd(h, w_pool, bias=b_pool, relu=True)
        m, arg = ops.spmm_max_fwd(g, p, want_arg=need_bwd, relu_input=True)
        out = dense.linear_fwd(h, w_self, m, w_neigh, bias=bias, relu=relu_out)
        if need_bwd:
            ctx.g, ctx.relu_out = g, relu_out
            ctx.save_for_backward(h, m, arg, out if relu_out else None, w_pool, w_self, w_neigh)
        return out

    @staticmethod
    def backward(ctx, gout):
        h, m, arg, out, w_pool, w_self, w_neigh = ctx.saved_tensors
        if not ctx.relu_out:
            g = gout.contiguous()
        elif out.shape[1] % 4 == 0 and out.shape[0] > 0:
            g, _ = ops.gat_act_bwd(gout.contiguous(), out, 2, want_bias_grad=False)
        else:
            g = dense.relu_bwd(gout, out)
        need = ctx.needs_input_grad
        gm = dense.linear_bwd_input(g, w_neigh)
        gp = ops.spmm_max_bwd(ctx.g, gm, arg)
        g_ws, g_wn, g_wp, g_bias, g_bp = _pool_layer_weight_grads(g, gp, h, m, w_pool, w_self)
        gh = dense.linear_bwd_input(g, w_self, gp, w_pool) if need[1] else None
        return None, gh, g_wp, g_bp, g_ws, g_wn, g_bias, None, None


class _SageSumLayer(torch.autograd.Function):

    @staticmethod
    def forward(ctx, g, h, w_self, w_neigh, bias, mode, relu_out, need_bwd):
        h = h.contiguous()
        d = g.dev()
        fin, fout = w_neigh.shape[1], w_neigh.shape[0]
        lin_first = fin > fout
        div = d.deg_clamped if mode == "mean" else d.deg_plus1
        src = dense.linear_fwd(h, w_neigh) if lin_first else h
        neigh = ops.spmm_sum_raw(g, src, div_out=div, add_self=(mode == "gcn"))
        last_w = _identity(fout, h.device) if lin_first else w_neigh
        if w_self is not None:
            out = dense.linear_fwd(h, w_self, neigh, last_w, bias=bias, relu=relu_out)
        else:
            out = dense.linear_fwd(neigh, last_w, bias=bias, relu=relu_out)
        if need_bwd:
            ctx.g, ctx.mode, ctx.relu_out, ctx.lin_first = g, mode, relu_out, lin_first
            ctx.has_bias = bias is not None
            ctx.save_for_backward(h, neigh if not lin_first else None, out if relu_out else None, w_self, w_neigh)
        return out

    @staticmethod
    def backward(ctx, gout):
        h, neigh, out, w_self, w_neigh = ctx.saved_tensors
        g, mode = ctx.g, ctx.mode
        d = g.dev()
        div = d.deg_clamped if mode == "mean" else d.deg_plus1
        need = ctx.needs_input_grad
        g_pre, g_bias = ops.gat_act_bwd(gout.contiguous(), out, 2 if ctx.relu_out else 0, want_bias_grad=ctx.has_bias)

        def reduce_bwd(t, accum=None):
            return ops.spmm_sum_raw(g, t, transposed=True, div_in=div, add_self=(mode == "gcn"), accum=accum)

        g_ws = None
        if ctx.lin_first:
            gt = reduce_bwd(g_pre)
            if w_self is not None:
                (g_ws, _), (g_wn, _) = dense.linear_bwd_weight_multi([(g_pre, h, False), (gt, h, False)])
                gh = dense.linear_bwd_input(g_pre, w_self, gt, w_neigh) if need[1] else None
            else:
                g_wn, _ = dense.linear_bwd_weight(gt, h)
                gh = dense.linear_bwd_input(gt, w_neigh) if need[1] else None
        else:
            if w_self is not None:
                (g_ws, _), (g_wn, _) = dense.linear_bwd_weight_multi([(g_pre, h, False), (g_pre, neigh, False)])
            else:
                g_wn, _ = dense.linear_bwd_weight(g_pre, neigh)
            gh = None
            if need[1]:
                gneigh = dense.linear_bwd_input(g_pre, w_neigh)
                gself = dense.linear_bwd_input(g_pre, w_self) if w_self is not None else None
                gh = reduce_bwd(gneigh, accum=gself)
        return None, gh, g_ws, g_wn, g_bias, None, None, None


_identities = {}


def _identity(n, device):
    key = (n, device)
    if key not in _identities:
        _identities[key] = torch.eye(n, dtype=torch.float32, device=device)
    return _identities[key]


RELU_MASK_BITS = os.environ.get("GTS_RELU_BITS", "1") != "0"


def _chainable(a0, w0, a1, w2):
    n, k0, k1, n2 = w0.shape[0], a0.shape[1], a1.shape[1], w2.shape[0]
    return n % 4 == 0 and k0 % 4 == 0 and k1 % 4 == 0 and n <= 256 and n2 <= 256 and w2.shape[1] == n


def _pool_layer_weight_grads(g, gp, h, m, w_pool, w_self):
    if w_pool.shape == w_self.shape:
        (g_ws, g_bias), (g_wn, _), (g_wp, g_bp) = dense.linear_bwd_weight_multi(
            [(g, h, True), (g, m, False), (gp, h, True)])
    else:
        (g_ws, g_bias), (g_wn, _) = dense.linear_bwd_weight_multi([(g, h, True), (g, m, False)])
        g_wp, g_bp = dense.linear_bwd_weight(gp, h, want_bias_grad=True)
    return g_ws, g_wn, g_wp, g_bias, g_bp


def _pack_by_shape(weights, transposed, want_plain=False):
    by_shape, plain, fragment = {}, {}, {}
    for w in weights:
        by_shape.setdefault(tuple(w.shape), []).append(w)
    for ws in by_shape.values():
        copies = dense.pack_weights(ws, transposed=transposed, want_plain=want_plain)
        if want_plain:
            plain.update((id(w), wt) for w, wt in zip(ws, copies[0]))
            copies = copies[1]
        fragment.update((id(w), wp) for w, wp in zip(ws, copies))
    return (plain, fragment) if want_plain else fragment


class _SagePoolStack(torch.autograd.Function):

    @staticmethod
    def forward(ctx, g, x, need_bwd, *params):
        n_layers = len(params) // 5
        h = x.contiguous()
        saved = []
        hbits = None
        p = None
        fragment = _pack_by_shape([w for i in range(n_layers) for w in (params[5 * i], params[5 * i + 2], params[5 * i + 3])
                                   if w.shape[0] > 128 and w.shape[1] % 4 == 0], transposed=False)
        for i in range(n_layers):
            w_pool, b_pool, w_self, w_neigh, bias = params[5 * i:5 * i + 5]
            last = i == n_layers - 1
            if p is None:
                p = dense.linear_fwd(h, w_pool, bias=b_pool, relu=True, packed=(fragment.get(id(w_pool)), None))
            m, arg = ops.spmm_max_fwd(g, p, want_arg=need_bwd, relu_input=True)
            p = None
            nxt = params[5 * (i + 1):5 * (i + 1) + 2] if not last else None
            obits = dense.relu_bits_empty(h.shape[0], w_self.shape[0], h.device) \
                if RELU_MASK_BITS and need_bwd and not last and dense.relu_bits_pay(h.shape[0], w_self.shape[0]) else None
            if nxt is not None and _chainable(h, w_self, m, nxt[0]):
                out, p = dense.linear_fwd_chain(h, w_self, m, w_neigh, bias, True, nxt[0], nxt[1], True, relu_bits=obits,
                                                packed=(fragment.get(id(w_self)), fragment.get(id(w_neigh)), fragment.get(id(nxt[0]))))
            else:
                out = dense.linear_fwd(h, w_self, m, w_neigh, bias=bias, relu=not last, relu_bits=obits,
                                       packed=(fragment.get(id(w_self)), fragment.get(id(w_neigh))))
            saved += [h, m, arg, hbits]
            h, hbits = out, obits
        if need_bwd:
            ctx.g, ctx.n_layers = g, n_layers
            ctx.save_for_backward(*saved, *params)
        return h

    @staticmethod
    def backward(ctx, gout):
        n = ctx.n_layers
        tensors = ctx.saved_tensors
        acts, params = tensors[:4 * n], tensors[4 * n:]
        grads = [None] * (5 * n)
        g = gout.contiguous()
        gx = None
        deferred = {}

        turned, turned_fragment = _pack_by_shape(
            [w for w in (params[5 * i + j] for i in range(n) for j in (0, 2, 3))
             if w.shape[1] >= 128 and w.shape[0] % 4 == 0 and w.shape[1] % 4 == 0], transposed=True, want_plain=True)

        def igrad(g0, w0, g1=None, w1=None, relu_mask=None, relu_bits=None):
            if id(w0) in turned and (w1 is None or id(w1) in turned) and g0.is_contiguous():
                return dense.linear_bwd_input_t(g0, turned[id(w0)], g1, turned[id(w1)] if w1 is not None else None,
                                                relu_mask=relu_mask, relu_bits=relu_bits,
                                                packed=(turned_fragment[id(w0)], turned_fragment[id(w1)] if w1 is not None else None))
            return dense.linear_bwd_input(g0, w0, g1, w1, relu_mask=relu_mask)

        def defer(grad_out, act, slot, bias_slot):
            key = (grad_out.shape[1], act.shape[1])
            deferred.setdefault(key, []).append((grad_out, act, bias_slot is not None, slot, bias_slot))

        gm = None
        for i in reversed(range(n)):
            h, m, arg, hbits = acts[4 * i:4 * i + 4]
            w_pool, _b_pool, w_self, w_neigh, _bias = params[5 * i:5 * i + 5]
            narrow = gm is None and not ops.INSTRUMENTED
            fused = narrow and i == 0 and dense.first_layer_bwd_applies(g, h, m, w_neigh)
            if fused:
                gm, grads[2], grads[4], grads[3] = dense.sage_first_layer_bwd(g, h, m, w_neigh)
            elif narrow and i == n - 1 and ops.lowrank_bwd_applies(g, w_neigh, arg):
                gp = ops.spmm_max_bwd_lowrank(ctx.g, g, w_neigh, arg)
            elif gm is None:
                gm = igrad(g, w_neigh)
            if gm is not None:
                gp = ops.spmm_max_bwd(ctx.g, gm, arg)
            gm = None
            defer(gp, h, 5 * i, 5 * i + 1)
            if not fused:
                defer(g, h, 5 * i + 2, 5 * i + 4)
                defer(g, m, 5 * i + 3, None)
            if i > 0:
                below = params[5 * (i - 1) + 3]
                if all(id(w) in turned for w in (w_self, w_pool, below)) and _chainable(g, w_self.t(), gp, below.t()):
                    g, gm = dense.linear_bwd_input_chain_t(g, turned[id(w_self)], gp, turned[id(w_pool)], h,
                                                           turned[id(below)], relu_bits=hbits,
                                                           packed=(turned_fragment[id(w_self)], turned_fragment[id(w_pool)],
                                                                   turned_fragment[id(below)]))
                else:
                    g = igrad(g, w_self, gp, w_pool, relu_mask=h, relu_bits=hbits)
            elif ctx.needs_input_grad[1]:
                gx = igrad(g, w_self, gp, w_pool)
        for problems in deferred.values():
            results = dense.linear_bwd_weight_multi([(go, act, want) for go, act, want, _, _ in problems])
            for (gw, gb), (_, _, _, slot, bias_slot) in zip(results, problems):
                grads[slot] = gw
                if bias_slot is not None:
                    grads[bias_slot] = gb
        return (None, gx, None, *grads)


STACK_IN_ONE_CALL = os.environ.get("GTS_STACK_C", "1") != "0"


class GradSink:

    def __init__(self, params, extra=0):
        self.params = list(params)
        self.offsets, at = {}, 0
        for p in self.params:
            self.offsets[id(p)] = at
            at += p.numel()
        self.n, self.extra = at, int(extra)
        self.flat, self.filled = None, False

    def new_buffer(self):
        self.flat = torch.empty(self.n + self.extra, dtype=torch.float32, device=self.params[0].device)
        self.filled = False
        return self.flat


_active_sink = None


class grad_sink:
    def __init__(self, sink):
        self.sink = sink

    def __enter__(self):
        global _active_sink
        self.previous, _active_sink = _active_sink, self.sink
        return self.sink

    def __exit__(self, *exc):
        global _active_sink
        _active_sink = self.previous
        return False


_stack_tables = {}


def _stack_table(params, in_feats):
    import ctypes

    ptrs = [p.data_ptr() for p in params]
    key = (in_feats, *ptrs, *[tuple(p.shape) for p in params])
    hit = _stack_tables.get(key)
    if hit is None:
        n_layers = len(params) // 5
        widths = [in_feats] + [params[5 * i + 2].shape[0] for i in range(n_layers)]
        hit = ((ctypes.c_void_p * (5 * n_layers))(*ptrs), (ctypes.c_int64 * (n_layers + 1))(*widths), widths)
        if len(_stack_tables) > 64:
            _stack_tables.clear()
        _stack_tables[key] = hit
    return hit


class _SagePoolStackCall(torch.autograd.Function):

    @staticmethod
    def forward(ctx, g, x, need_bwd, *params):
        import ctypes

        from . import _lib
        from ._lib import check, current_stream, ptr

        lib = _lib.load()
        x = x.contiguous()
        n, n_layers = x.shape[0], len(params) // 5
        table, c_widths, widths = _stack_table(params, x.shape[1])
        relu_bits, ab = 1 if RELU_MASK_BITS else 0, g.arg_bytes
        d = g.dev()
        offsets = (ctypes.c_int64 * (4 * n_layers + 2))()
        total = lib.gts_sage_pool_stack_fwd_arena(n, c_widths, n_layers, 1 if need_bwd else 0, ab, relu_bits, offsets)
        if total < 0:
            raise _lib.GtsError("gts_sage_pool_stack_fwd_arena rejected the stack's shape")
        arena = torch.empty(max(int(total), 16), dtype=torch.uint8, device=x.device)
        ds = ops._cluster_schedule(g, "in", n, 256, ab if need_bwd else 0) if 256 in widths[:-1] else None
        check(lib.gts_sage_pool_stack_fwd_f32(
            ptr(d.indptr), ptr(d.indices), *_DeviceSchedule.launch_args(ds), ptr(x), table, n, c_widths, n_layers,
            1 if need_bwd else 0, ab, relu_bits, arena.data_ptr(), int(total), current_stream()),
            "gts_sage_pool_stack_fwd_f32")
        at = int(offsets[4 * (n_layers - 1) + 2])
        out = arena[at:at + 4 * n * widths[-1]].view(torch.float32).view(n, widths[-1])
        if need_bwd:
            ctx.g, ctx.widths, ctx.relu_bits, ctx.ab = g, widths, relu_bits, ab
            ctx.param_ids = [id(p) for p in params]
            ctx.save_for_backward(x, arena, *params)
        return out

    @staticmethod
    def backward(ctx, gout):
        import ctypes

        from . import _lib
        from ._lib import check, current_stream, ptr

        lib = _lib.load()
        x, arena, *params = ctx.saved_tensors
        g, widths, relu_bits, ab = ctx.g, ctx.widths, ctx.relu_bits, ctx.ab
        n, n_layers = x.shape[0], len(params) // 5
        gout = gout.contiguous()
        d = g.dev()
        sink = _active_sink
        if sink is not None and (len(ctx.param_ids) != len(sink.params) or
                                 not all(i in sink.offsets for i in ctx.param_ids)):
            sink = None
        sizes = [p.numel() for p in params]
        if sink is not None:
            flat, starts = sink.flat, [sink.offsets[i] for i in ctx.param_ids]
        else:
            flat = torch.empty(sum(sizes), dtype=torch.float32, device=x.device)
            starts = [0] * len(sizes)
            for q in range(1, len(sizes)):
                starts[q] = starts[q - 1] + sizes[q - 1]
        base = flat.data_ptr()
        grads = (ctypes.c_void_p * (5 * n_layers))(*[base + 4 * s for s in starts])
        table, c_widths, _ = _stack_table(params, x.shape[1])
        need = lib.gts_sage_pool_stack_bwd_scratch(n, c_widths, n_layers, relu_bits)
        scratch = torch.empty(max(int(need), 16), dtype=torch.uint8, device=x.device)
        gx = torch.empty_like(x) if ctx.needs_input_grad[1] else None
        ds = ops._cluster_schedule(g, "out", n, 256, ab) if 256 in widths[:-1] else None
        check(lib.gts_sage_pool_stack_bwd_f32(
            ptr(d.t_indptr), ptr(d.t_indices), ptr(d.t_slot), *_DeviceSchedule.launch_args(ds), ptr(gout), ptr(x), table, n,
            c_widths, n_layers, ab, relu_bits, arena.data_ptr(), grads, ptr(gx), scratch.data_ptr(), int(need),
            current_stream()), "gts_sage_pool_stack_bwd_f32")
        if sink is not None:
            sink.filled = True
            return (None, gx, None, *([None] * len(params)))
        return (None, gx, None, *[flat[s:s + k].view_as(p) for s, k, p in zip(starts, sizes, params)])


def sage_pool_stack(graph, features, layers):
    for i, layer in enumerate(layers):
        last = i == len(layers) - 1
        if not isinstance(layer, SAGEConv) or layer._aggre_type != "pool" or layer.bias is None \
                or layer.norm is not None or (layer.feat_drop.p > 0 and layer.training):
            return None
        if (layer.activation is not None) if last else (not _is_relu(layer.activation)):
            return None
    params = []
    for layer in layers:
        params += [layer.fc_pool.weight, layer.fc_pool.bias, layer.fc_self.weight,
                   layer.fc_neigh.weight, layer.bias]
    need_bwd = torch.is_grad_enabled() and (features.requires_grad or any(p.requires_grad for p in params))
    one_call = STACK_IN_ONE_CALL and not ops.INSTRUMENTED and features.shape[1] % 4 == 0 \
        and all(p.shape[-1] % 4 == 0 and p.shape[0] % 4 == 0 and p.is_contiguous() for p in params) \
        and features.dtype == torch.float32 and features.is_cuda
    return (_SagePoolStackCall if one_call else _SagePoolStack).apply(graph, features, need_bwd, *params)


class SAGEConv(nn.Module):

    def __init__(self, in_feats, out_feats, aggregator_type, feat_drop=0.0, bias=True, norm=None,
                 activation=None):
        super().__init__()
        if aggregator_type not in ("mean", "gcn", "pool"):
            raise KeyError(f"Invalid aggregator_type. Must be one of mean, gcn, pool. "
                           f"But got {aggregator_type!r} instead.")
        self._in_src_feats = self._in_dst_feats = int(in_feats)
        self._out_feats = int(out_feats)
        self._aggre_type = aggregator_type
        self.norm = norm
        self.feat_drop = nn.Dropout(feat_drop)
        self.activation = activation
        if aggregator_type == "pool":
            self.fc_pool = nn.Linear(in_feats, in_feats)
        if aggregator_type != "gcn":
            self.fc_self = nn.Linear(in_feats, out_feats, bias=False)
        self.fc_neigh = nn.Linear(in_feats, out_feats, bias=False)
        if bias:
            self.bias = nn.Parameter(torch.zeros(out_feats))
        else:
            self.register_buffer("bias", None)
        self.reset_parameters()

    def reset_parameters(self):
        gain = nn.init.calculate_gain("relu")
        if self._aggre_type == "pool":
            nn.init.xavier_uniform_(self.fc_pool.weight, gain=gain)
        if self._aggre_type != "gcn":
            nn.init.xavier_uniform_(self.fc_self.weight, gain=gain)
        nn.init.xavier_uniform_(self.fc_neigh.weight, gain=gain)

    def _load_from_state_dict(self, state_dict, prefix, *args, **kwargs):
        legacy = [prefix + "fc_self.bias", prefix + "fc_neigh.bias"]
        if prefix + "bias" not in state_dict and any(k in state_dict for k in legacy):
            folded = sum(state_dict.pop(k) for k in legacy if k in state_dict)
            state_dict[prefix + "bias"] = folded
        super()._load_from_state_dict(state_dict, prefix, *args, **kwargs)

    def forward(self, graph, feat):
        h = self.feat_drop(feat)
        fused_relu = _is_relu(self.activation)
        if self._aggre_type == "pool":
            bias = self.bias if self.bias is not None else torch.zeros(
                self._out_feats, dtype=h.dtype, device=h.device)
            need_bwd = torch.is_grad_enabled() and (
                h.requires_grad or any(p.requires_grad for p in self.parameters()))
            rst = _SagePoolLayer.apply(graph, h, self.fc_pool.weight, self.fc_pool.bias,
                                       self.fc_self.weight, self.fc_neigh.weight, bias,
                                       fused_relu, need_bwd)
        elif self._out_feats % 4 == 0 and h.shape[0] > 0:
            need_bwd = torch.is_grad_enabled() and (
                h.requires_grad or any(p.requires_grad for p in self.parameters()))
            w_self = self.fc_self.weight if self._aggre_type != "gcn" else None
            rst = _SageSumLayer.apply(graph, h, w_self, self.fc_neigh.weight, self.bias, self._aggre_type,
                                      fused_relu, need_bwd)
        else:
            lin_before_mp = self._in_src_feats > self._out_feats
            src = dense.linear(h, self.fc_neigh.weight) if lin_before_mp else h
            neigh = ops.spmm_reduce(graph, src, self._aggre_type)
            if not lin_before_mp:
                neigh = dense.linear(neigh, self.fc_neigh.weight)
            rst = neigh if self._aggre_type == "gcn" else dense.linear(h, self.fc_self.weight) + neigh
            if self.bias is not None:
                rst = rst + self.bias
            if fused_relu:
                rst = torch.relu(rst)
        if self.activation is not None and not fused_relu:
            rst = self.activation(rst)
        if self.norm is not None:
            rst = self.norm(rst)
        return rst


FUSE_GAT_LAYER = os.environ.get("GTS_FUSE_GAT", "1") != "0"
FUSE_GAT_SCORES = os.environ.get("GTS_FUSE_GAT_SCORES", "1") != "0"


FOLD_GAT_ACT_BWD = os.environ.get("GTS_FOLD_GAT_ACT", "1") != "0"


PACK_GAT_WEIGHTS = os.environ.get("GTS_PACK_GAT", "1") != "0"


def _turn(ws):
    if PACK_GAT_WEIGHTS:
        plain, packed = dense.pack_weights(ws, transposed=True, want_plain=True)
        return plain, tuple(packed) if len(packed) > 1 else (packed[0], None)
    return dense.transpose_batch(ws), (None, None)


class ActLink:
    __slots__ = ("folded", "g_bias", "armed")

    def __init__(self):
        self.folded, self.g_bias, self.armed = False, None, 0


class _GATLayer(torch.autograd.Function):

    @staticmethod
    def forward(ctx, g, h, w_fc, attn_l, attn_r, bias, w_res, identity_res, slope, act_code, heads, dim,
                need_bwd, below=None, above=None):
        h = h.contiguous()
        n = h.shape[0]
        al, ar = attn_l.reshape(heads, dim), attn_r.reshape(heads, dim)
        if FUSE_GAT_SCORES and h.shape[1] % 4 == 0:
            ft, el, er = ops.gat_fc_scores(h, w_fc, al, ar, heads, dim)
        else:
            ft = dense.linear_fwd(h, w_fc).view(n, heads, dim)
            el, er = ops.gat_scores(ft, al, ar)
        if w_res is not None:
            res = dense.linear_fwd(h, w_res)
        elif identity_res:
            res = h
        else:
            res = None
        out, attn = ops._gat_fwd(g, ft, el, er, slope, bias, res, act_code)
        if need_bwd:
            ctx.g, ctx.slope, ctx.act, ctx.identity_res = g, slope, act_code, identity_res
            ctx.save_for_backward(h, ft, el, er, attn, out if act_code else None, w_fc, al, ar, w_res)
            ctx.attn_shape = attn_l.shape
            ctx.below, ctx.above = below, above if act_code == 1 else None
            if ctx.above is not None:
                ctx.above.armed = act_code
        return out

    @staticmethod
    def backward(ctx, gout):
        h, ft, el, er, attn, out, w_fc, al, ar, w_res = ctx.saved_tensors
        n, heads, dim = ft.shape
        need = ctx.needs_input_grad
        if ctx.above is not None and ctx.above.folded:
            g_pre, g_bias = gout.reshape(n, heads * dim), ctx.above.g_bias if need[5] else None
            ctx.above.folded, ctx.above.g_bias, ctx.above.armed = False, None, 0
        else:
            g_pre, g_bias = ops.gat_act_bwd(gout.reshape(n, heads * dim),
                                            out.view(n, heads * dim) if out is not None else None, ctx.act,
                                            want_bias_grad=need[5])
        gft, gel, ger = ops._gat_bwd(ctx.g, ft, el, er, attn, g_pre.view(n, heads, dim), ctx.slope, al, ar)
        g_al, g_ar = ops.gat_param_grad(ft, gel, ger)
        gft2 = gft.view(n, heads * dim)
        g_wres = None
        turn = need[1] and w_fc.shape[1] >= 128 and w_fc.shape[0] % 4 == 0 \
            and w_fc.shape[1] % 4 == 0 and n >= 4096
        fold = turn and ctx.below is not None and ctx.below.armed == 1 and not ctx.identity_res and FOLD_GAT_ACT_BWD
        act_below = ctx.below.armed if fold else 0
        if w_res is not None:
            (g_wfc, _), (g_wres, _) = dense.linear_bwd_weight_multi([(gft2, h, False), (g_pre, h, False)])
            if fold:
                wt, wtp = _turn([w_fc, w_res])
                gh, ctx.below.g_bias = dense.linear_bwd_input_t_act(gft2, wt[0], h, act_below, g_pre, wt[1], packed=wtp)
                ctx.below.folded = True
            elif turn:
                wt, wtp = _turn([w_fc, w_res])
                gh = dense.linear_bwd_input_t(gft2, wt[0], g_pre, wt[1], packed=wtp)
            else:
                gh = dense.linear_bwd_input(gft2, w_fc, g_pre, w_res) if need[1] else None
        else:
            g_wfc, _ = dense.linear_bwd_weight(gft2, h)
            if fold:
                wt, wtp = _turn([w_fc])
                gh, ctx.below.g_bias = dense.linear_bwd_input_t_act(gft2, wt[0], h, act_below, packed=(wtp[0], None))
                ctx.below.folded = True
            elif turn:
                wt, wtp = _turn([w_fc])
                gh = dense.linear_bwd_input_t(gft2, wt[0], packed=(wtp[0], None))
            else:
                gh = dense.linear_bwd_input(gft2, w_fc) if need[1] else None
            if gh is not None and ctx.identity_res:
                gh = gh + g_pre
        return (None, gh, g_wfc, g_al.view(ctx.attn_shape), g_ar.view(ctx.attn_shape), g_bias, g_wres,
                None, None, None, None, None, None, None, None)


class GATConv(nn.Module):

    def __init__(self, in_feats, out_feats, num_heads, feat_drop=0.0, attn_drop=0.0,
                 negative_slope=0.2, residual=False, activation=None,
                 allow_zero_in_degree=False, bias=True):
        super().__init__()
        self._in_feats, self._out_feats, self._num_heads = int(in_feats), int(out_feats), int(num_heads)
        self._allow_zero_in_degree = allow_zero_in_degree
        self.fc = nn.Linear(in_feats, out_feats * num_heads, bias=False)
        self.attn_l = nn.Parameter(torch.empty(1, num_heads, out_feats))
        self.attn_r = nn.Parameter(torch.empty(1, num_heads, out_feats))
        self.feat_drop = nn.Dropout(feat_drop)
        self.attn_drop = nn.Dropout(attn_drop)
        self.negative_slope = negative_slope
        if bias:
            self.bias = nn.Parameter(torch.empty(num_heads * out_feats))
        else:
            self.register_buffer("bias", None)
        if residual:
            if in_feats != out_feats * num_heads:
                self.res_fc = nn.Linear(in_feats, num_heads * out_feats, bias=False)
            else:
                self.res_fc = nn.Identity()
        else:
            self.register_buffer("res_fc", None)
        self.activation = activation
        self.reset_parameters()

    def reset_parameters(self):
        gain = nn.init.calculate_gain("relu")
        nn.init.xavier_normal_(self.fc.weight, gain=gain)
        nn.init.xavier_normal_(self.attn_l, gain=gain)
        nn.init.xavier_normal_(self.attn_r, gain=gain)
        if self.bias is not None:
            nn.init.constant_(self.bias, 0)
        if isinstance(self.res_fc, nn.Linear):
            nn.init.xavier_normal_(self.res_fc.weight, gain=gain)

    def forward(self, graph, feat, below=None, above=None):
        if not self._allow_zero_in_degree and graph.min_in_degree == 0:
            raise GraphError(
                "There are 0-in-degree nodes in the graph, output for those nodes will be invalid. "
                "Adding self-loop on the input graph resolves the issue; setting "
                "allow_zero_in_degree=True suppresses the check.")
        if self.attn_drop.p > 0 and self.training:
            raise NotImplementedError("attention dropout is not built (the reference never sets it: "
                                      "model/networks.py:77-78 passes no dropout to GAT)")
        n = feat.shape[0]
        h = self.feat_drop(feat)
        if above is not None:
            above.armed = 0
        act_code = 0 if self.activation is None else 1 if self.activation in (F.elu, torch.nn.functional.elu) else -1
        if FUSE_GAT_LAYER and act_code >= 0 and self._out_feats % 4 == 0 and feat.dim() == 2:
            w_res = self.res_fc.weight if isinstance(self.res_fc, nn.Linear) else None
            identity_res = isinstance(self.res_fc, nn.Identity)
            need_bwd = torch.is_grad_enabled() and (
                h.requires_grad or any(p.requires_grad for p in self.parameters()))
            if self.feat_drop.p > 0 and self.training:
                below = None
            return _GATLayer.apply(graph, h, self.fc.weight, self.attn_l, self.attn_r, self.bias, w_res,
                                   identity_res, self.negative_slope, act_code, self._num_heads,
                                   self._out_feats, need_bwd, below, above)
        ft = dense.linear(h, self.fc.weight).view(n, self._num_heads, self._out_feats)
        el = (ft * self.attn_l).sum(dim=-1)
        er = (ft * self.attn_r).sum(dim=-1)
        rst = ops.gat_aggregate(graph, ft, el, er, self.negative_slope)
        if self.res_fc is not None:
            res = dense.linear(h, self.res_fc.weight) if isinstance(self.res_fc, nn.Linear) else h
            rst = rst + res.view(n, -1, self._out_feats)
        if self.bias is not None:
            rst = rst + self.bias.view(1, self._num_heads, self._out_feats)
        if self.activation is not None:
            rst = self.activation(rst)
        return rst
```

### gnn-tumor-seg_amd/gts/optim.py

```python
import torch

from . import _lib
from ._lib import check, current_stream, ptr


class FlatAdamW(torch.optim.Optimizer):
    def __init__(self, params, lr=1e-3, betas=(0.9, 0.999), eps=1e-8, weight_decay=1e-2):
        params = [p for p in params if p.requires_grad]
        if not params:
            raise ValueError("optimizer got an empty parameter list")
        dev = params[0].device
        for p in params:
            if p.dtype != torch.float32 or p.device != dev or not p.is_cuda:
                raise _lib.GtsError("FlatAdamW needs fp32 parameters on one AMD GPU (no CPU fallback)")
        super().__init__(params, dict(lr=lr, betas=betas, eps=eps, weight_decay=weight_decay))
        self._params = params
        self._sizes = [p.numel() for p in params]
        self.n = sum(self._sizes)
        self.flat_param = torch.cat([p.detach().reshape(-1) for p in params])
        off = 0
        for p, n in zip(params, self._sizes):
            p.data = self.flat_param[off:off + n].view_as(p)
            off += n
        self.exp_avg = torch.zeros_like(self.flat_param)
        self.exp_avg_sq = torch.zeros_like(self.flat_param)
        self.steps = 0

    def _still_flat(self):
        base, off = self.flat_param.data_ptr(), 0
        for p, n in zip(self._params, self._sizes):
            if p.data_ptr() != base + 4 * off:
                return False
            off += n
        return True

    @torch.no_grad()
    def step(self, closure=None, flat_grad=None):
        loss = None
        if closure is not None:
            with torch.enable_grad():
                loss = closure()
        if not self._still_flat():
            raise _lib.GtsError("parameters were re-allocated after FlatAdamW was built (e.g. net.to(...)): "
                                "create the optimizer after moving the network")
        if flat_grad is None:
            missing = [i for i, p in enumerate(self._params) if p.grad is None]
            if missing:
                raise _lib.GtsError(f"parameters {missing} received no gradient this step")
            flat_grad = torch.cat([p.grad.reshape(-1) for p in self._params])
        if flat_grad.numel() != self.n or flat_grad.dtype != torch.float32 or not flat_grad.is_contiguous():
            raise _lib.GtsError("flat_grad must be one contiguous fp32 tensor with one entry per parameter")
        group = self.param_groups[0]
        self.steps += 1
        check(_lib.load().gts_adamw_f32(ptr(self.flat_param), ptr(flat_grad), ptr(self.exp_avg),
                                        ptr(self.exp_avg_sq), self.n, float(group["lr"]),
                                        float(group["betas"][0]), float(group["betas"][1]), float(group["eps"]),
                                        float(group["weight_decay"]), self.steps, current_stream()),
              "gts_adamw_f32")
        return loss
```

### include/gts_hip.h

```cpp
#ifndef GTS_HIP_H
#define GTS_HIP_H

#include <stdint.h>

#ifdef __cplusplus
extern "C" {
#endif

#define GTS_OK 0
#define GTS_ERR_NULL (-1)
#define GTS_ERR_SHAPE (-2)
#define GTS_ERR_ARGKIND (-3)

int32_t gts_abi_version(void);
const char* gts_error_string(int32_t code);

int32_t gts_spmm_max_fwd_f32(const int32_t* indptr, const int32_t* indices, const float* x,
                             float* out, void* arg, int32_t arg_bytes, int32_t relu_input,
                             int64_t n_dst, int64_t n_feat, void* stream);

int32_t gts_spmm_max_bwd_f32(const int32_t* t_indptr, const int32_t* t_indices,
                             const int32_t* t_slot, const float* gout, const void* arg,
                             int32_t arg_bytes, const float* relu_src, float* gx,
                             int64_t n_src, int64_t n_feat, void* stream);
int32_t gts_spmm_max_bwd_lowrank_f32(const int32_t* t_indptr, const int32_t* t_indices,
                                     const int32_t* t_slot, const float* g, const float* w, const void* arg,
                                     int32_t arg_bytes, float* gx, int64_t n_src, int64_t n_feat,
                                     int64_t rank, void* stream);

int64_t gts_cluster_record_words(int32_t max_rows, int32_t max_srcs, int32_t loc_words, int32_t with_tag);
int32_t gts_cluster_schedule(const int32_t* indptr, const int32_t* indices, const int32_t* t_indptr,
                             const int32_t* t_indices, const int32_t* edge_tag, int64_t n_rows,
                             int32_t max_rows, int32_t max_srcs, int32_t max_edges, int32_t* rec,
                             int64_t rec_capacity, int64_t* n_clusters, int64_t* n_staged,
                             int32_t* max_cluster_edges);
int64_t gts_cluster_lds_bytes(int32_t max_rows, int32_t max_srcs, int32_t loc_words, int32_t kind);
int32_t gts_spmm_max_fwd_cluster_f32(const int32_t* rec, int64_t n_clusters, int32_t max_rows, int32_t max_srcs,
                                     int32_t loc_words, const float* x, float* out, void* arg,
                                     int32_t arg_bytes, int32_t relu_input, int64_t n_rows, int64_t n_feat,
                                     uint32_t* counters, void* stream);
int32_t gts_spmm_max_bwd_cluster_f32(const int32_t* rec, int64_t n_clusters, int32_t max_rows, int32_t max_srcs,
                                     int32_t loc_words, const float* gout, const void* arg, int32_t arg_bytes,
                                     float* gx, int64_t n_rows, int64_t n_feat, uint32_t* counters, void* stream);
#define GTS_CLUSTER_COUNTER_WORDS 256
int32_t gts_cluster_uses_counters(int64_t n_clusters, int32_t max_rows, int32_t max_srcs, int32_t loc_words, int32_t backward);

int32_t gts_spmm_sum_f32(const int32_t* indptr, const int32_t* indices, const float* x,
                         float* out, const float* div_in, const float* div_out, const float* accum,
                         int32_t add_self, int64_t n_out, int64_t n_feat, void* stream);

int32_t gts_gat_fwd_f32(const int32_t* indptr, const int32_t* indices, const float* ft,
                        const float* el, const float* er, float negative_slope, const float* bias,
                        const float* residual, int32_t activation, float* out, float* attn,
                        int64_t n, int64_t heads, int64_t dim, void* stream);
int32_t gts_gat_scores_f32(const float* ft, const float* attn_l, const float* attn_r, float* el,
                           float* er, int64_t n, int64_t heads, int64_t dim, void* stream);

int32_t gts_gat_bwd_edge_f32(const int32_t* indptr, const int32_t* indices, const float* ft,
                             const float* el, const float* er, const float* attn,
                             const float* gout, float negative_slope, float* ge, float* ger,
                             int64_t n, int64_t heads, int64_t dim, void* stream);
int32_t gts_gat_bwd_src_f32(const int32_t* t_indptr, const int32_t* t_indices,
                            const int32_t* t_pos, const float* attn, const float* ge,
                            const float* gout, const float* attn_l, const float* attn_r,
                            const float* ger, float* gft, float* gel, int64_t n, int64_t heads,
                            int64_t dim, void* stream);
int64_t gts_gat_reduce_workspace(int64_t n, int64_t cols);
int32_t gts_gat_act_bwd_f32(const float* gout, const float* out, int32_t activation, float* g_pre,
                            float* g_bias, float* workspace, int64_t workspace_bytes, int64_t n,
                            int64_t cols, void* stream);
int32_t gts_gat_param_grad_f32(const float* ft, const float* gel, const float* ger, float* g_attn_l,
                               float* g_attn_r, float* workspace, int64_t workspace_bytes, int64_t n,
                               int64_t heads, int64_t dim, void* stream);

int64_t gts_gat_cluster_workspace(int64_t n_clusters, int32_t max_rows, int32_t loc_words, int64_t heads, int32_t backward);
int32_t gts_gat_attn_f32(const int32_t* indptr, const int32_t* indices, const float* el, const float* er,
                         float negative_slope, float* attn, int64_t n, int64_t heads, int64_t max_degree, void* stream);
int32_t gts_gat_fwd_cluster_f32(const int32_t* indptr, const int32_t* indices, const int32_t* rec, int64_t n_clusters,
                                int32_t max_rows, int32_t max_srcs, int32_t loc_words, int32_t tagged, const float* ft,
                                const float* el, const float* er, float negative_slope, const float* bias,
                                int32_t activation, float* out, float* attn, float* workspace, int64_t workspace_bytes,
                                int64_t n, int64_t heads, int64_t dim, int64_t max_degree, void* stream);
int32_t gts_gat_bwd_edge_cluster_f32(const int32_t* indptr, const int32_t* indices, const int32_t* rec, int64_t n_clusters,
                                     int32_t max_rows, int32_t max_srcs, int32_t loc_words, int32_t tagged, const float* ft,
                                     const float* el, const float* er, const float* attn, const float* gout,
                                     float negative_slope, float* ge, float* ger, float* workspace, int64_t workspace_bytes,
                                     int64_t n, int64_t heads, int64_t dim, int64_t max_degree, void* stream);
int32_t gts_gat_bwd_src_cluster_f32(const int32_t* t_indptr, const int32_t* t_pos, const int32_t* rec, int64_t n_clusters,
                                    int32_t max_rows, int32_t max_srcs, int32_t loc_words, int32_t tagged,
                                    const float* attn, const float* ge, const float* gout, const float* attn_lr,
                                    const float* ger, float* gft, float* gel, float* workspace, int64_t workspace_bytes,
                                    int64_t n, int64_t heads, int64_t dim, int64_t max_degree, void* stream);

int32_t gts_project_rows_i16(const int16_t* svs, const void* table, const void* bg_row,
                             void* out, int64_t n_vox, int64_t n_rows, int32_t row_bytes,
                             void* stream);
int32_t gts_project_argmax_i16(const int16_t* svs, const float* logits, const int16_t* relabel,
                               int16_t* out, int64_t n_vox, int64_t n_rows, int64_t n_classes,
                               void* stream);

int32_t gts_project_argmax_occupancy_i16(const int16_t* svs, const float* logits, int16_t* out,
                                         uint8_t* occupancy, int64_t dim_x, int64_t dim_y,
                                         int64_t dim_z, int64_t n_rows, int64_t n_classes,
                                         void* stream);

int32_t gts_crop_concat_f32(const float* img, const int16_t* svs, const float* table,
                            const float* bg_row, const int32_t* xs, const int32_t* ys,
                            const int32_t* zs, float* out, int64_t cx, int64_t cy, int64_t cz,
                            int64_t dim_y, int64_t dim_z, int64_t n_rows, int64_t img_channels,
                            int64_t row_channels, void* stream);
int32_t gts_argmax_scatter_i16(const float* scores, const int16_t* relabel, const int32_t* xs,
                               const int32_t* ys, const int32_t* zs, int16_t* out, int64_t cx,
                               int64_t cy, int64_t cz, int64_t dim_y, int64_t dim_z,
                               int64_t n_classes, void* stream);
int32_t gts_crop_concat_rows_f32(const float* img, const int16_t* svs, const float* table,
                                 const float* bg_row, const int32_t* xs, const int32_t* ys,
                                 const int32_t* zs, float* out, int64_t cx, int64_t cy, int64_t cz,
                                 int64_t dim_y, int64_t dim_z, int64_t n_rows, int64_t img_channels,
                                 int64_t row_channels, void* stream);
int32_t gts_crop_concat_rows_bwd_f32(const float* dx, const int32_t* list_ptr, const int32_t* list_vox,
                                     const int32_t* inv_x, const int32_t* inv_y, const int32_t* inv_z,
                                     float* d_table, int64_t cx, int64_t cy, int64_t cz, int64_t dim_x,
                                     int64_t dim_y, int64_t dim_z, int64_t n_rows, int64_t img_channels,
                                     int64_t row_channels, void* stream);

int32_t gts_adamw_f32(float* param, const float* grad, float* exp_avg, float* exp_avg_sq, int64_t n,
                      double lr, double beta1, double beta2, double eps, double weight_decay,
                      int64_t step, void* stream);

int64_t gts_label_confusion_workspace(int64_t n);
int32_t gts_label_confusion_i16(const int16_t* pred, const int16_t* truth, int64_t* counts,
                                void* workspace, int64_t workspace_bytes, int64_t n, void* stream);

int64_t gts_relu_bits_bytes(int64_t m, int64_t n);
int32_t gts_relu_bits_pay(int64_t m, int64_t n);
int32_t gts_linear_fwd_f32(const float* a0, const float* w0, const float* a1, const float* w1,
                           const float* bias, float* out, int64_t m, int64_t n, int64_t k0,
                           int64_t k1, int32_t relu, uint64_t* relu_bits, const float* const* packed,
                           void* stream);
int64_t gts_packed_weight_floats(int64_t n, int64_t k);
int32_t gts_pack_weights_f32(const float* const* src, float* const* dst, float* const* plain_t, int32_t n_mats,
                             int64_t rows, int64_t cols, int32_t transposed, void* stream);
int32_t gts_linear_bwd_input_f32(const float* g0, const float* w0, const float* g1, const float* w1,
                                 const float* relu_mask, float* gin, int64_t m, int64_t k,
                                 int64_t n0, int64_t n1, void* stream);
int32_t gts_linear_bwd_input_t_f32(const float* g0, const float* w0t, const float* g1, const float* w1t,
                                   const float* relu_mask, const uint64_t* relu_bits, float* gin, int64_t m,
                                   int64_t k, int64_t n0, int64_t n1, const float* const* packed, void* stream);
int64_t gts_linear_bwd_input_t_act_workspace(int64_t m, int64_t k);
int32_t gts_linear_bwd_input_t_act_f32(const float* g0, const float* w0t, const float* g1, const float* w1t,
                                       const float* act_out, int32_t activation, float* gin, float* g_bias,
                                       float* workspace, int64_t workspace_bytes, int64_t m, int64_t k,
                                       int64_t n0, int64_t n1, const float* const* packed,
                                       void* stream);
int64_t gts_gat_fc_scores_workspace(int64_t m, int64_t heads, int64_t dim);
int32_t gts_gat_fc_scores_f32(const float* h, const float* w_fc, const float* attn_l, const float* attn_r,
                              float* ft, float* el, float* er, float* workspace, int64_t workspace_bytes,
                              int64_t m, int64_t heads, int64_t dim, int64_t k, const float* w_fc_packed, void* stream);
int32_t gts_linear_fwd_chain_f32(const float* a0, const float* w0, const float* a1, const float* w1,
                                 const float* bias, float* out, const float* w2, const float* bias2,
                                 float* out2, int64_t m, int64_t n, int64_t k0, int64_t k1, int32_t relu,
                                 int64_t n2, int32_t relu2, uint64_t* relu_bits, const float* const* packed,
                                 void* stream);
int32_t gts_linear_bwd_input_chain_t_f32(const float* g0, const float* w0t, const float* g1,
                                         const float* w1t, const float* relu_mask, const uint64_t* relu_bits,
                                         float* gin, const float* w2t, float* gin2, int64_t m, int64_t k,
                                         int64_t n0, int64_t n1, int64_t k2, const float* const* packed,
                                         void* stream);
int32_t gts_transpose_batch_f32(const float* const* src, float* const* dst, int32_t n_mats,
                                int64_t rows, int64_t cols, void* stream);
int64_t gts_linear_bwd_weight_workspace(int64_t m, int64_t n, int64_t k, int32_t n_problems);
int32_t gts_linear_bwd_weight_f32(const float* const* g, const float* const* a, float* const* gw,
                                  float* const* gb, int32_t n_problems, float* workspace,
                                  int64_t workspace_bytes, int64_t m, int64_t n, int64_t k,
                                  void* stream);
int64_t gts_sage_first_layer_bwd_workspace(int64_t m, int64_t w, int64_t s0, int64_t s1);
int32_t gts_sage_first_layer_bwd_f32(const float* g, const float* x, const float* m0, const float* w_neigh, float* gm,
                                     float* gw_self, float* g_bias, float* gw_neigh, float* workspace,
                                     int64_t workspace_bytes, int64_t m, int64_t w, int64_t s0, int64_t s1, void* stream);

int64_t gts_sage_pool_stack_fwd_arena(int64_t n_rows, const int64_t* widths, int32_t n_layers, int32_t training,
                                      int32_t arg_bytes, int32_t relu_bits, int64_t* offsets);
int32_t gts_sage_pool_stack_fwd_f32(const int32_t* indptr, const int32_t* indices, const int32_t* sched_rec,
                                    int64_t sched_clusters, int32_t sched_rows, int32_t sched_srcs,
                                    int32_t sched_loc_words, const float* x, const float* const* params,
                                    int64_t n_rows, const int64_t* widths, int32_t n_layers, int32_t training,
                                    int32_t arg_bytes, int32_t relu_bits, void* arena, int64_t arena_bytes, void* stream);
int64_t gts_sage_pool_stack_bwd_scratch(int64_t n_rows, const int64_t* widths, int32_t n_layers, int32_t relu_bits);
int32_t gts_sage_pool_stack_bwd_f32(const int32_t* t_indptr, const int32_t* t_indices, const int32_t* t_slot,
                                    const int32_t* sched_rec, int64_t sched_clusters, int32_t sched_rows,
                                    int32_t sched_srcs, int32_t sched_loc_words, const float* gout, const float* x,
                                    const float* const* params, int64_t n_rows, const int64_t* widths,
                                    int32_t n_layers, int32_t arg_bytes, int32_t relu_bits, const void* fwd_arena,
                                    float* const* grads, float* gx, void* scratch, int64_t scratch_bytes,
                                    void* stream);

int64_t gts_weighted_ce_workspace(int64_t n);
int32_t gts_weighted_ce_f32(const float* logits, const int64_t* labels, const float* class_w,
                            float* grad_unscaled, float* workspace, int64_t workspace_bytes,
                            float* out3, int64_t n, int64_t n_classes, void* stream);

#define GTS_DICE_CE_MAX_GROUPS 8
#define GTS_DICE_CE_STATS_FLOATS 40
#define GTS_DICE_CE_STATS_LOSS 0
#define GTS_DICE_CE_STATS_CE 1
#define GTS_DICE_CE_STATS_LDICE 2
#define GTS_DICE_CE_STATS_CE_NUM 3
#define GTS_DICE_CE_STATS_CE_DEN 4
#define GTS_DICE_CE_STATS_DICE 8
#define GTS_DICE_CE_STATS_I 16
#define GTS_DICE_CE_STATS_S 24
#define GTS_DICE_CE_STATS_T 32
int64_t gts_dice_ce_workspace(int64_t n, int32_t n_groups);
int32_t gts_dice_ce_fwd_f32(const float* logits, const int64_t* labels, const float* class_w,
                            const uint32_t* group_masks, int32_t n_groups, double ce_weight,
                            double dice_weight, double smooth, float* stats, void* workspace,
                            int64_t workspace_bytes, int64_t n, int64_t n_classes, void* stream);
int32_t gts_dice_ce_bwd_f32(const float* logits, const int64_t* labels, const float* class_w,
                            const uint32_t* group_masks, int32_t n_groups, double ce_weight,
                            double dice_weight, double smooth, const float* stats,
                            const float* grad_scale, float* grad, int64_t n, int64_t n_classes,
                            void* stream);

int32_t gts_augment_crop_f32(const float* x, const int64_t* labels, const float* params, float* x_out,
                             int64_t* labels_out, int64_t cx, int64_t cy, int64_t cz, int64_t channels,
                             int64_t image_channels, int32_t flip_mask, uint64_t seed, uint64_t step,
                             void* stream);
int32_t gts_augment_features_f32(const float* feats, const int64_t* row_ptr, const int64_t* row_ptr_host,
                                 const float* params, float* out, int64_t n_rows, int64_t n_feats,
                                 int64_t modalities, int64_t n_graphs, double sigma, uint64_t seed,
                                 uint64_t step, void* stream);

int32_t gts_augment_spatial_f32(const float* x, const int64_t* labels, const float* params,
                                const double* matrix, float* x_out, int64_t* labels_out, int64_t cx,
                                int64_t cy, int64_t cz, int64_t channels, int64_t image_channels,
                                int32_t flip_mask, uint64_t seed, uint64_t step, void* stream);
int32_t gts_augment_spatial_bwd_f32(const float* dy, const double* matrix, float* dx, int64_t cx, int64_t cy,
                                    int64_t cz, int64_t channels, int32_t flip_mask, void* stream);

#define GTS_OPT_GEMM_TILE 1
#define GTS_OPT_WGRAD_TILE 2
#define GTS_OPT_IGRAD_TILE 3
#define GTS_OPT_PROJECT_STREAMING 6
#define GTS_OPT_SPMM_ROWS_PER_WAVE 4
#define GTS_OPT_SPMM_STREAMING 5
#define GTS_OPT_GEMM_SCHED 7
#define GTS_OPT_CLUSTER_STREAMING 8
#define GTS_OPT_GAT_WALK 14
#define GTS_OPT_GAT_CLUSTER_WAVES 15
#define GTS_OPT_GAT_CLUSTER_GROUP 16
#define GTS_OPT_GAT_CLUSTER_DEALING 17
#define GTS_OPT_CLUSTER_DEALING 18
#define GTS_OPT_PANEL_ROWS 13
#define GTS_OPT_CLUSTER_RING 10
#define GTS_OPT_CLUSTER_PER_CU 11
#define GTS_OPT_CLUSTER_CONSUMERS 12
int32_t gts_set_option(int32_t option, int32_t value);
int32_t gts_get_option(int32_t option);

#define GTS_COLLATE_MAX_SCHEDULES 6
typedef struct {
  int64_t n_nodes, n_edges;
  const int32_t *indptr, *indices, *t_indptr, *t_indices, *t_slot, *t_pos;
  const void* features;
  const void* labels;
  int32_t feat_bytes;
  int32_t label_bytes;
  const int32_t* sched_rec[GTS_COLLATE_MAX_SCHEDULES];
  int64_t sched_clusters[GTS_COLLATE_MAX_SCHEDULES];
  int32_t sched_loc_words[GTS_COLLATE_MAX_SCHEDULES];
} gts_collate_member_t;
typedef struct {
  int32_t max_rows, max_srcs, tagged, reserved;
} gts_collate_kind_t;
typedef struct {
  int64_t total_bytes, n_nodes, n_edges;
  int64_t features, labels;
  int64_t csr[8];
  int64_t sched[GTS_COLLATE_MAX_SCHEDULES];
  int64_t sched_clusters[GTS_COLLATE_MAX_SCHEDULES];
  int32_t sched_loc_words[GTS_COLLATE_MAX_SCHEDULES];
  int32_t sched_record_words[GTS_COLLATE_MAX_SCHEDULES];
} gts_collate_plan_t;
int32_t gts_collate_plan(const gts_collate_member_t* members, int32_t n_members, int64_t feat_width,
                         const gts_collate_kind_t* kinds, int32_t n_kinds, gts_collate_plan_t* plan);
int32_t gts_collate_batch(const gts_collate_member_t* members, int32_t n_members, int64_t feat_width,
                          const gts_collate_kind_t* kinds, int32_t n_kinds, void* dst, int64_t dst_bytes,
                          int32_t n_threads, gts_collate_plan_t* plan);

#define GTS_GG_MAX_SV 32767
#define GTS_GG_MAX_K 32
#define GTS_GG_MAX_RADIUS 16
int32_t gts_gg_gaussian_f64(const double* in, double* out, double* tmp, const double* weights, int32_t radius,
                            double scale, int64_t d, int64_t h, int64_t w, int64_t c, void* stream);
int32_t gts_gg_slic_assign_f64(const double* img, const double* centres, int32_t n_centres, int64_t d, int64_t h,
                               int64_t w, int64_t c, int32_t step_z, int32_t step_y, int32_t step_x,
                               double spatial_weight, int32_t* labels, uint64_t* best, uint32_t* winner,
                               void* stream);
int32_t gts_gg_slic_update_f64(const double* img, const int32_t* labels, double* centres, int32_t n_centres,
                               int64_t d, int64_t h, int64_t w, int64_t c, int32_t* bbox, void* stream);
int32_t gts_gg_enforce_connectivity(const int32_t* labels, int32_t* out, int64_t d, int64_t h, int64_t w,
                                    int64_t min_size, int64_t max_size, int64_t* queue, int32_t* n_labels);
int64_t gts_gg_sv_stats_workspace(int64_t n_vox, int32_t n_sv);
int32_t gts_gg_sv_stats(const int32_t* partition, const float* intensities, const int16_t* vox_labels, int64_t d,
                        int64_t h, int64_t w, int64_t c, int32_t n_sv, double* feats, double* centroids,
                        int32_t* sv_labels, void* scratch, void* stream);
int32_t gts_gg_discard_f64(const double* feats, const double* centroids, const int32_t* sv_labels, int32_t n_sv,
                           int32_t n_feat, const int32_t* partition, int64_t n_vox, int32_t* remap, int32_t* keep,
                           double* node_feats, double* node_centroids, int32_t* node_labels, int16_t* new_partition,
                           int32_t* n_nodes, void* stream);
int32_t gts_gg_knn_candidates_f64(const double* positions, int32_t n, int32_t k, int32_t* cand, void* stream);
int32_t gts_gg_knn_greedy(const int32_t* cand, int32_t n, int32_t k, int32_t* picks, int32_t* got, int64_t* n_edges);
int64_t gts_gg_touching_workspace(int32_t n);
int32_t gts_gg_touching_count_i16(const int16_t* partition, int64_t d, int64_t h, int64_t w, int32_t n, void* scratch,
                                  int32_t* indptr, void* stream);
int32_t gts_gg_touching_emit(const void* scratch, int32_t n, const int32_t* indptr, int32_t* cols, void* stream);

int64_t gts_conv3d_fwd_workspace(int32_t cin, int32_t cout);
int32_t gts_conv3d_fwd_f32(const float* x, const float* w, const float* bias, float* y, int64_t cx, int64_t cy,
                           int64_t cz, int32_t cin, int32_t cout, int32_t relu, void* workspace,
                           int64_t workspace_bytes, void* stream);
int64_t gts_conv3d_bwd_data_workspace(int64_t cx, int64_t cy, int64_t cz, int32_t cin, int32_t cout);
int32_t gts_conv3d_bwd_data_f32(const float* dy, const float* w, const float* h, float* dx, int64_t cx, int64_t cy,
                                int64_t cz, int32_t cin, int32_t cout, void* workspace, int64_t workspace_bytes,
                                void* stream);
int64_t gts_conv3d_bwd_weight_workspace(int64_t cx, int64_t cy, int64_t cz, int32_t cin, int32_t cout);
int32_t gts_conv3d_bwd_weight_f32(const float* x, const float* dy, float* dw, float* db, int64_t cx, int64_t cy,
                                  int64_t cz, int32_t cin, int32_t cout, void* workspace, int64_t workspace_bytes,
                                  void* stream);

int64_t gts_hd95_workspace(int64_t X, int64_t Y, int64_t Z);
int32_t gts_hd95_order_stats_i16(const int16_t* pred, const int16_t* truth, int64_t X, int64_t Y, int64_t Z,
                                 int32_t all_border, int64_t* out, void* workspace, int64_t workspace_bytes,
                                 void* stream);

int64_t gts_surface_workspace(int64_t X, int64_t Y, int64_t Z, const int64_t* units);
int32_t gts_surface_stats_i16(const int16_t* pred, const int16_t* truth, int64_t X, int64_t Y, int64_t Z,
                              int32_t all_border, const int64_t* units, const int64_t* thresholds,
                              int32_t n_thresholds, int64_t* out, void* workspace, int64_t workspace_bytes,
                              void* stream);

int64_t gts_components_workspace(int64_t X, int64_t Y, int64_t Z);
int32_t gts_components_roots_i16(const int16_t* labels, int64_t X, int64_t Y, int64_t Z, int32_t connectivity,
                                 int32_t* roots_out, void* workspace, int64_t workspace_bytes, void* stream);
int32_t gts_components_filter_i16(const int16_t* labels_in, int64_t X, int64_t Y, int64_t Z, int32_t connectivity,
                                  int64_t min_voxels, int32_t et_label, int64_t et_min_voxels, int32_t et_replacement,
                                  int16_t* labels_out, int64_t* stats, void* workspace, int64_t workspace_bytes,
                                  void* stream);

int64_t gts_lesionwise_workspace(int64_t X, int64_t Y, int64_t Z);
int64_t gts_lesionwise_table_ints(int64_t X, int64_t Y, int64_t Z);
int32_t gts_lesionwise_dilate_i16(const int16_t* labels, int64_t X, int64_t Y, int64_t Z, int32_t region,
                                  int32_t dilation, int16_t* mask_out, void* workspace, int64_t workspace_bytes,
                                  void* stream);
int32_t gts_lesionwise_tables_i16(const int16_t* truth, const int32_t* pred_roots, const int32_t* dilated_roots,
                                  int64_t X, int64_t Y, int64_t Z, int32_t region, int32_t* tables_out,
                                  int64_t tables_ints, void* workspace, int64_t workspace_bytes, void* stream);
int32_t gts_lesionwise_masks_i16(const int16_t* truth, const int32_t* pred_roots, const int32_t* dilated_roots,
                                 int64_t X, int64_t Y, int64_t Z, int32_t region, int32_t lesion_root,
                                 const int32_t* matched_roots, int64_t n_matched, const int64_t* box, int16_t* mask_m,
                                 int16_t* mask_g, void* stream);

int32_t gts_intake_occupancy(const void* src, int32_t dtype, int64_t X, int64_t Y, int64_t Z, int32_t* flag_x,
                             int32_t* flag_y, int32_t* flag_z, uint64_t* nonfinite, void* stream);
int64_t gts_intake_select_workspace(void);
int32_t gts_intake_order_stats(const void* src, int32_t dtype, int64_t X, int64_t Y, int64_t Z, const int32_t* xs,
                               int64_t cx, const int32_t* ys, int64_t cy, const int32_t* zs, int64_t cz,
                               int64_t rank_lo, int64_t rank_hi, float* out, void* workspace, int64_t workspace_bytes,
                               void* stream);
int32_t gts_intake_standardize(const void* src, int32_t dtype, int64_t X, int64_t Y, int64_t Z, const int32_t* xs,
                               int64_t cx, const int32_t* ys, int64_t cy, const int32_t* zs, int64_t cz,
                               const float* params, float* out, void* stream);

int64_t gts_dataset_stats_workspace(int64_t X, int64_t Y, int64_t Z);
int32_t gts_dataset_stats_mask(const void* src, int32_t dtype, const int16_t* labels, int64_t X, int64_t Y, int64_t Z,
                               uint64_t* counts, void* workspace, int64_t workspace_bytes, void* stream);
int32_t gts_dataset_stats_order_stats(const void* src, int32_t dtype, int64_t X, int64_t Y, int64_t Z, int64_t n,
                                      int64_t rank_lo, int64_t rank_hi, float* out, void* workspace,
                                      int64_t workspace_bytes, void* stream);
int32_t gts_dataset_stats_moments(const void* src, int32_t dtype, int64_t X, int64_t Y, int64_t Z, int64_t n,
                                  const float* top, double* out, void* workspace, int64_t workspace_bytes,
                                  void* stream);

int32_t gts_conform_gather(const void* src, int32_t dtype, int64_t C, int64_t X, int64_t Y, int64_t Z, int32_t axis0,
                           int32_t axis1, int32_t axis2, int64_t OX, int64_t OY, int64_t OZ, const int32_t* idx0,
                           const int32_t* idx1, const double* t, int32_t mode, void* dst, void* stream);

int32_t gts_softmax_accumulate_f32(const float* const* sets, int64_t n_sets, float* acc, int64_t rows,
                                   int64_t classes, int32_t overwrite, void* stream);
int32_t gts_argmax_scatter_rows_i16(const float* scores, const int16_t* relabel, const int32_t* xs,
                                    const int32_t* ys, const int32_t* zs, int16_t* out, int64_t cx, int64_t cy,
                                    int64_t cz, int64_t dim_y, int64_t dim_z, int64_t n_classes, void* stream);

int32_t gts_region_uncertainty_rows_u8(const float* sums, const int32_t* xs, const int32_t* ys, const int32_t* zs,
                                       uint8_t* out, int64_t cx, int64_t cy, int64_t cz, int64_t dim_x,
                                       int64_t dim_y, int64_t dim_z, int64_t n_classes, int64_t terms, void* stream);
int32_t gts_region_uncertainty_nodes_u8(const int16_t* svs, const float* sums, uint8_t* out, int64_t n_vox,
                                        int64_t n_rows, int64_t n_classes, int64_t terms, void* stream);
#define GTS_UNCERTAINTY_BINS 102
#define GTS_UNCERTAINTY_HIST_WORDS 1632
int32_t gts_uncertainty_histogram(const int16_t* pred, const int16_t* truth, const uint8_t* unc, int64_t* hist,
                                  int64_t n, void* stream);

#define GTS_REGISTER_MAX_MATRICES 16
int32_t gts_affine_resample(const void* src, int32_t dtype, int64_t X, int64_t Y, int64_t Z, const double* matrix,
                            int64_t OX, int64_t OY, int64_t OZ, float* dst, int32_t path, void* stream);
int32_t gts_joint_histogram(const float* fixed, int64_t FX, int64_t FY, int64_t FZ, const void* moving, int32_t dtype,
                            int64_t X, int64_t Y, int64_t Z, const double* matrices, int64_t K, int64_t stride,
                            int64_t bins, double lo_f, double scale_f, double lo_m, double scale_m, int64_t* counts,
                            int64_t grid_blocks, void* stream);

#define GTS_BIAS_BINS 200
#define GTS_BIAS_MAX_SPANS 32
int64_t gts_bias_workspace(int64_t X, int64_t Y, int64_t Z, int64_t spans);
int32_t gts_bias_log(const void* src, int32_t dtype, int64_t X, int64_t Y, int64_t Z, double threshold, float* u,
                     uint64_t* count, void* stream);
int32_t gts_bias_range(const float* u, int64_t X, int64_t Y, int64_t Z, const double* weights, const int32_t* cells,
                       const double* lattice, int64_t spans0, int64_t levels, double* range, void* workspace,
                       int64_t workspace_bytes, int64_t grid_blocks, void* stream);
int32_t gts_bias_histogram(const float* u, int64_t X, int64_t Y, int64_t Z, const double* weights, const int32_t* cells,
                           const double* lattice, int64_t spans0, int64_t levels, double lo, double hi, int64_t* counts,
                           int64_t grid_blocks, void* stream);
int32_t gts_bias_fit(const float* u, int64_t X, int64_t Y, int64_t Z, const double* weights, const int32_t* cells,
                     const double* lattice, int64_t spans0, int64_t levels, int64_t level, const double* fit_weights,
                     double lo, double hi, const double* table, double* out, void* workspace, int64_t workspace_bytes,
                     int64_t grid_blocks, void* stream);
int32_t gts_bias_mean(const float* u, int64_t X, int64_t Y, int64_t Z, const double* weights, const int32_t* cells,
                      const double* lattice, int64_t spans0, int64_t levels, double* out, void* workspace,
                      int64_t workspace_bytes, int64_t grid_blocks, void* stream);
int32_t gts_bias_apply(const void* src, int32_t dtype, int64_t X, int64_t Y, int64_t Z, const double* weights,
                       const int32_t* cells, const double* lattice, int64_t spans0, int64_t levels, double mean,
                       float* out, float* field_out, int64_t grid_blocks, void* stream);

#ifdef __cplusplus
}
#endif
#endif
```

Before: 972.8 graphs/s.

## Batch wgrad finishing reductions and keep packed weight forms updated in AdamW

Weight-gradient partial-sum reductions from the whole SAGE stack are collected as finish jobs and run in one batched finish_sums kernel, replacing a small reduce launch per layer. The Python side also caches packed and transposed weight forms per parameter set, and a new AdamW variant rewrites those forms in the same optimizer pass. Forward and backward can then read the forms directly instead of repacking weights each step. This cuts kernel launches and repacking work, but adds cache invalidation logic that can go stale if parameters change outside the optimizer.

```diff
diff --git a/gnn-tumor-seg_amd/csrc/gts_gemm.hip b/gnn-tumor-seg_amd/csrc/gts_gemm.hip
--- a/gnn-tumor-seg_amd/csrc/gts_gemm.hip
+++ b/gnn-tumor-seg_amd/csrc/gts_gemm.hip
@@ -1,3 +1,5 @@
+#include <algorithm>
+
 #include "gts_gemm_tiles.h"
 #include "gts_gemm_panel.h"
 #include "gts_gemm_wgrad.h"
@@ -304,24 +306,21 @@
   return (slabs > skinny ? slabs : skinny) * static_cast<int64_t>(sizeof(float));
 }
 
-extern "C" int32_t gts_linear_bwd_weight_f32(const float* const* g, const float* const* a, float* const* gw,
-                                             float* const* gb, int32_t n_problems, float* workspace,
-                                             int64_t workspace_bytes, int64_t m, int64_t n, int64_t k, void* stream) {
-  using namespace gts;
-  if (!g || !a || !gw || !workspace) return GTS_ERR_NULL;
-  if (n_problems < 1 || n_problems > kMaxProblems) return GTS_ERR_ARGKIND;
-  if (m <= 0 || n <= 0 || k <= 0 || m >= (1LL << 31) || n >= (1 << 20) || k >= (1 << 20) || !aligned4(n) || !aligned4(k))
-    return GTS_ERR_SHAPE;
-  if (workspace_bytes < gts_linear_bwd_weight_workspace(m, n, k, n_problems)) return GTS_ERR_SHAPE;
+namespace gts {
+namespace {
+
+inline int64_t skinny_problem_floats(int64_t m, int64_t n, int64_t k) {
+  return skinny_workspace_floats(m, n, k) + kSkinnyChunks * (n < k ? n : 0);
+}
+
+int wgrad_run(const float* const* g, const float* const* a, float* const* gw, float* const* gb, int n_problems,
+              float* workspace, int64_t m, int64_t n, int64_t k, hipStream_t st, std::vector<FinishJob>* jobs) {
   bool any_bias = false;
-  for (int q = 0; q < n_problems; ++q) {
-    if (!g[q] || !a[q] || !gw[q]) return GTS_ERR_NULL;
-    any_bias = any_bias || (gb && gb[q]);
-  }
-  hipStream_t st = static_cast<hipStream_t>(stream);
+  for (int q = 0; q < n_problems; ++q) any_bias = any_bias || (gb && gb[q]);
   if (skinny_workspace_floats(m, n, k) > 0) {
+    const int64_t stride = jobs != nullptr ? skinny_problem_floats(m, n, k) : 0;
     for (int q = 0; q < n_problems; ++q)
-      skinny_wgrad(g[q], a[q], gw[q], gb ? gb[q] : nullptr, workspace, m, n, k, st);
+      skinny_wgrad(g[q], a[q], gw[q], gb ? gb[q] : nullptr, workspace + q * stride, m, n, k, st, jobs);
     return launch_status();
   }
   const WgradPlan plan = wgrad_plan(m, n, k, n_problems);
@@ -341,19 +340,82 @@
   p.tiles_per_split = (tiles + splits - 1) / splits;
   int rc = launch_wgrad(p, plan, st);
   if (rc != GTS_OK) return rc;
+  if (jobs != nullptr) {
+    for (int q = 0; q < n_problems; ++q)
+      jobs->push_back(FinishJob{workspace + static_cast<size_t>(q) * splits * n * k, gw[q], nullptr,
+                                static_cast<int>(n * k / 4), splits, 0, 0, 0});
+    for (int q = 0; q < n_problems && any_bias; ++q)
+      if (gb[q])
+        jobs->push_back(FinishJob{p.colsum + static_cast<size_t>(q) * splits * n, gb[q], nullptr, static_cast<int>(n / 4),
+                                  splits, 0, 0, 0});
+    return GTS_OK;
+  }
   ReduceArgs r{};
   r.splits = splits;
-  int jobs = 0;
-  for (int q = 0; q < n_problems; ++q, ++jobs) {
-    r.slabs[jobs] = workspace + static_cast<size_t>(q) * splits * n * k;
-    r.out[jobs] = gw[q], r.n4[jobs] = static_cast<int>(n * k / 4);
+  int n_jobs = 0;
+  for (int q = 0; q < n_problems; ++q, ++n_jobs) {
+    r.slabs[n_jobs] = workspace + static_cast<size_t>(q) * splits * n * k;
+    r.out[n_jobs] = gw[q], r.n4[n_jobs] = static_cast<int>(n * k / 4);
   }
   for (int q = 0; q < n_problems && any_bias; ++q) {
     if (!gb[q]) continue;
-    r.slabs[jobs] = p.colsum + static_cast<size_t>(q) * splits * n;
-    r.out[jobs] = gb[q], r.n4[jobs] = static_cast<int>(n / 4);
-    ++jobs;
-  }
-  reduce_slabs_kernel<<<dim3(static_cast<unsigned>((n * k / 4 + 63) / 64), jobs), kBlock, 0, st>>>(r);
+    r.slabs[n_jobs] = p.colsum + static_cast<size_t>(q) * splits * n;
+    r.out[n_jobs] = gb[q], r.n4[n_jobs] = static_cast<int>(n / 4);
+    ++n_jobs;
+  }
+  reduce_slabs_kernel<<<dim3(static_cast<unsigned>((n * k / 4 + 63) / 64), n_jobs), kBlock, 0, st>>>(r);
   return launch_status();
 }
+
+inline bool wgrad_bad_shape(int64_t m, int64_t n, int64_t k) {
+  return m <= 0 || n <= 0 || k <= 0 || m >= (1LL << 31) || n >= (1 << 20) || k >= (1 << 20) || !aligned4(n) || !aligned4(k);
+}
+
+}
+
+int64_t wgrad_partials_workspace(int64_t m, int64_t n, int64_t k, int n_problems) {
+  if (wgrad_bad_shape(m, n, k) || n_problems < 1 || n_problems > kMaxProblems) return 0;
+  if (skinny_workspace_floats(m, n, k) > 0) return n_problems * skinny_problem_floats(m, n, k) * static_cast<int64_t>(sizeof(float));
+  return gts_linear_bwd_weight_workspace(m, n, k, n_problems);
+}
+
+int wgrad_partials(const float* const* g, const float* const* a, float* const* gw, float* const* gb, int n_problems,
+                   float* workspace, int64_t m, int64_t n, int64_t k, hipStream_t st, std::vector<FinishJob>* jobs) {
+  if (!g || !a || !gw || !workspace || !jobs) return GTS_ERR_NULL;
+  if (n_problems < 1 || n_problems > kMaxProblems) return GTS_ERR_ARGKIND;
+  if (wgrad_bad_shape(m, n, k)) return GTS_ERR_SHAPE;
+  for (int q = 0; q < n_problems; ++q)
+    if (!g[q] || !a[q] || !gw[q]) return GTS_ERR_NULL;
+  return wgrad_run(g, a, gw, gb, n_problems, workspace, m, n, k, st, jobs);
+}
+
+int finish_sums(const std::vector<FinishJob>& jobs, hipStream_t st) {
+  for (size_t first = 0; first < jobs.size(); first += kMaxFinishJobs) {
+    const int count = static_cast<int>(std::min<size_t>(kMaxFinishJobs, jobs.size() - first));
+    FinishArgs r{};
+    int blocks = 1;
+    for (int q = 0; q < count; ++q) {
+      const FinishJob& j = jobs[first + q];
+      r.src[q] = j.src, r.dst0[q] = j.dst0, r.dst1[q] = j.dst1;
+      r.count[q] = j.count, r.parts[q] = j.parts, r.w[q] = j.w, r.s_cols[q] = j.s_cols, r.transposed[q] = j.transposed;
+      blocks = std::max(blocks, j.w == 0 ? (j.count + 63) / 64 : (j.count + 15) / 16);
+    }
+    finish_sums_kernel<<<dim3(static_cast<unsigned>(blocks), count), kBlock, 0, st>>>(r);
+  }
+  return launch_status();
+}
+
+}
+
+extern "C" int32_t gts_linear_bwd_weight_f32(const float* const* g, const float* const* a, float* const* gw,
+                                             float* const* gb, int32_t n_problems, float* workspace,
+                                             int64_t workspace_bytes, int64_t m, int64_t n, int64_t k, void* stream) {
+  using namespace gts;
+  if (!g || !a || !gw || !workspace) return GTS_ERR_NULL;
+  if (n_problems < 1 || n_problems > kMaxProblems) return GTS_ERR_ARGKIND;
+  if (wgrad_bad_shape(m, n, k)) return GTS_ERR_SHAPE;
+  if (workspace_bytes < gts_linear_bwd_weight_workspace(m, n, k, n_problems)) return GTS_ERR_SHAPE;
+  for (int q = 0; q < n_problems; ++q)
+    if (!g[q] || !a[q] || !gw[q]) return GTS_ERR_NULL;
+  return wgrad_run(g, a, gw, gb, n_problems, workspace, m, n, k, static_cast<hipStream_t>(stream), nullptr);
+}
diff --git a/gnn-tumor-seg_amd/csrc/gts_gemm_args.h b/gnn-tumor-seg_amd/csrc/gts_gemm_args.h
--- a/gnn-tumor-seg_amd/csrc/gts_gemm_args.h
+++ b/gnn-tumor-seg_amd/csrc/gts_gemm_args.h
@@ -1,4 +1,6 @@
 #pragma once
+#include <vector>
+
 #include "gts_common.h"
 
 namespace gts {
@@ -8,6 +10,22 @@
 inline int g_igrad_variant = 1;
 inline int g_wgrad_variant = -1;
 inline int g_panel_rows = 0;
+
+struct FinishJob {
+  const float* src;
+  float* dst0;
+  float* dst1;
+  int count, parts;
+  int w, s_cols, transposed;
+};
+
+int64_t wgrad_partials_workspace(int64_t m, int64_t n, int64_t k, int n_problems);
+int wgrad_partials(const float* const* g, const float* const* a, float* const* gw, float* const* gb, int n_problems,
+                   float* workspace, int64_t m, int64_t n, int64_t k, hipStream_t st, std::vector<FinishJob>* jobs);
+int first_layer_bwd_partials(const float* g, const float* x, const float* m0, const float* w_neigh, float* gm, float* gw_self,
+                             float* g_bias, float* gw_neigh, float* workspace, int64_t m, hipStream_t st,
+                             std::vector<FinishJob>* jobs);
+int finish_sums(const std::vector<FinishJob>& jobs, hipStream_t st);
 
 namespace {
 
diff --git a/gnn-tumor-seg_amd/csrc/gts_gemm_skinny.h b/gnn-tumor-seg_amd/csrc/gts_gemm_skinny.h
--- a/gnn-tumor-seg_amd/csrc/gts_gemm_skinny.h
+++ b/gnn-tumor-seg_amd/csrc/gts_gemm_skinny.h
@@ -48,14 +48,12 @@
   }
 }
 
-__global__ __launch_bounds__(kBlock) void skinny_sum_kernel(const float* __restrict__ partial,
-                                                           float* __restrict__ dst0,
-                                                           float* __restrict__ dst1, int rows, int s_cols,
-                                                           int w, int chunks, int transposed) {
+__device__ __forceinline__ void skinny_sum_body(const float* __restrict__ partial, float* __restrict__ dst0,
+                                                float* __restrict__ dst1, int total_out, int s_cols, int w, int chunks,
+                                                int transposed) {
   __shared__ float part[16][16];
   const int o = threadIdx.x & 15, lane = threadIdx.x >> 4;
   const int idx = blockIdx.x * 16 + o;
-  const int total_out = rows * w;
   float acc = 0.f;
   if (idx < total_out) {
 #pragma unroll 8
@@ -74,5 +72,12 @@
     dst1[j] = sum;
 }
 
+__global__ __launch_bounds__(kBlock) void skinny_sum_kernel(const float* __restrict__ partial,
+                                                           float* __restrict__ dst0,
+                                                           float* __restrict__ dst1, int rows, int s_cols,
+                                                           int w, int chunks, int transposed) {
+  skinny_sum_body(partial, dst0, dst1, rows * w, s_cols, w, chunks, transposed);
+}
+
 }
 }
diff --git a/gnn-tumor-seg_amd/csrc/gts_gemm_wgrad.h b/gnn-tumor-seg_amd/csrc/gts_gemm_wgrad.h
--- a/gnn-tumor-seg_amd/csrc/gts_gemm_wgrad.h
+++ b/gnn-tumor-seg_amd/csrc/gts_gemm_wgrad.h
@@ -169,20 +169,16 @@
   int splits;
 };
 
-__global__ __launch_bounds__(kBlock) void reduce_slabs_kernel(const ReduceArgs p) {
+__device__ __forceinline__ void reduce_slabs_body(const float* slabs, float* out, int n4, int splits) {
   __shared__ v4f part[4][64];
   const int col = threadIdx.x & 63, grp = threadIdx.x >> 6;
-  const int q = blockIdx.y;
-  const float* slabs = kernarg_entry<const float*>(offsetof(ReduceArgs, slabs), q);
-  float* out = kernarg_entry<float*>(offsetof(ReduceArgs, out), q);
-  const int n4 = kernarg_entry<int>(offsetof(ReduceArgs, n4), q);
   const int i = blockIdx.x * 64 + col;
   if (blockIdx.x * 64 >= n4) return;
   v4f acc = {0.f, 0.f, 0.f, 0.f};
   if (i < n4) {
     const v4f* src = reinterpret_cast<const v4f*>(slabs) + i;
 #pragma unroll 8
-    for (int s = grp; s < p.splits; s += 4) acc += src[static_cast<size_t>(s) * n4];
+    for (int s = grp; s < splits; s += 4) acc += src[static_cast<size_t>(s) * n4];
   }
   part[grp][col] = acc;
   __syncthreads();
@@ -192,11 +188,45 @@
   }
 }
 
+__global__ __launch_bounds__(kBlock) void reduce_slabs_kernel(const ReduceArgs p) {
+  const int q = blockIdx.y;
+  const float* slabs = kernarg_entry<const float*>(offsetof(ReduceArgs, slabs), q);
+  float* out = kernarg_entry<float*>(offsetof(ReduceArgs, out), q);
+  const int n4 = kernarg_entry<int>(offsetof(ReduceArgs, n4), q);
+  reduce_slabs_body(slabs, out, n4, p.splits);
+}
+
 }
 }
 #include "gts_gemm_skinny.h"
 namespace gts {
 namespace {
+
+constexpr int kMaxFinishJobs = 80;
+
+struct FinishArgs {
+  const float* src[kMaxFinishJobs];
+  float* dst0[kMaxFinishJobs];
+  float* dst1[kMaxFinishJobs];
+  int count[kMaxFinishJobs], parts[kMaxFinishJobs], w[kMaxFinishJobs], s_cols[kMaxFinishJobs], transposed[kMaxFinishJobs];
+};
+
+__global__ __launch_bounds__(kBlock) void finish_sums_kernel(const FinishArgs ) {
+  const int q = blockIdx.y;
+  const float* src = kernarg_entry<const float*>(offsetof(FinishArgs, src), q);
+  float* dst0 = kernarg_entry<float*>(offsetof(FinishArgs, dst0), q);
+  const int count = kernarg_entry<int>(offsetof(FinishArgs, count), q);
+  const int parts = kernarg_entry<int>(offsetof(FinishArgs, parts), q);
+  const int w = kernarg_entry<int>(offsetof(FinishArgs, w), q);
+  if (w == 0) {
+    reduce_slabs_body(src, dst0, count, parts);
+    return;
+  }
+  if (blockIdx.x * 16 >= count) return;
+  skinny_sum_body(src, dst0, kernarg_entry<float*>(offsetof(FinishArgs, dst1), q), count,
+                  kernarg_entry<int>(offsetof(FinishArgs, s_cols), q), w, parts,
+                  kernarg_entry<int>(offsetof(FinishArgs, transposed), q));
+}
 
 inline int64_t skinny_workspace_floats(int64_t m, int64_t n, int64_t k) {
   const int64_t small = n < k ? n : k, big = n < k ? k : n;
@@ -211,7 +241,7 @@
 }
 
 inline bool skinny_wgrad(const float* g, const float* a, float* gw, float* gb, float* workspace, int64_t m,
-                  int64_t n, int64_t k, hipStream_t st) {
+                  int64_t n, int64_t k, hipStream_t st, std::vector<FinishJob>* jobs = nullptr) {
   if (skinny_workspace_floats(m, n, k) == 0) return false;
   const bool g_is_skinny = n < k;
   const float* skinny = g_is_skinny ? g : a;
@@ -232,13 +262,19 @@
     case 8: launch_skinny<8>(skinny, s_cols, wide, workspace, m, w, chunks, rpc, st); break;
     default: launch_skinny<9>(skinny, s_cols, wide, workspace, m, w, chunks, rpc, st); break;
   }
-  skinny_sum_kernel<<<(rows * w + 15) / 16, kBlock, 0, st>>>(
-      workspace, gw, ones_row ? gb : nullptr, rows, s_cols, w, chunks, g_is_skinny ? 0 : 1);
+  if (jobs != nullptr)
+    jobs->push_back(FinishJob{workspace, gw, ones_row ? gb : nullptr, rows * w, chunks, w, s_cols, g_is_skinny ? 0 : 1});
+  else
+    skinny_sum_kernel<<<(rows * w + 15) / 16, kBlock, 0, st>>>(
+        workspace, gw, ones_row ? gb : nullptr, rows, s_cols, w, chunks, g_is_skinny ? 0 : 1);
   if (g_is_skinny && gb != nullptr) {
     float* part = workspace + static_cast<size_t>(chunks) * rows * w;
     skinny_wgrad_kernel<1><<<chunks, kBlock, 0, st>>>(nullptr, 0, g, part, m, static_cast<int>(n), rpc);
-    skinny_sum_kernel<<<(static_cast<int>(n) + 15) / 16, kBlock, 0, st>>>(
-        part, nullptr, gb, 1, 0, static_cast<int>(n), chunks, 0);
+    if (jobs != nullptr)
+      jobs->push_back(FinishJob{part, nullptr, gb, static_cast<int>(n), chunks, static_cast<int>(n), 0, 0});
+    else
+      skinny_sum_kernel<<<(static_cast<int>(n) + 15) / 16, kBlock, 0, st>>>(
+          part, nullptr, gb, 1, 0, static_cast<int>(n), chunks, 0);
   }
   return true;
 }
diff --git a/gnn-tumor-seg_amd/csrc/gts_narrow.hip b/gnn-tumor-seg_amd/csrc/gts_narrow.hip
--- a/gnn-tumor-seg_amd/csrc/gts_narrow.hip
+++ b/gnn-tumor-seg_amd/csrc/gts_narrow.hip
@@ -88,7 +88,35 @@
   return m > 0 && m < (1LL << 31) && w == kFirstW && s0 == kFirstS && s1 == kFirstS;
 }
 
+int first_layer_bwd_run(const float* g, const float* x, const float* m0, const float* w_neigh, float* gm, float* gw_self,
+                        float* g_bias, float* gw_neigh, float* workspace, int64_t m, hipStream_t st,
+                        std::vector<FinishJob>* jobs) {
+  const int64_t rpc = (m + kSkinnyChunks - 1) / kSkinnyChunks;
+  const int chunks = static_cast<int>((m + rpc - 1) / rpc);
+  const int W = kFirstW, S = kFirstS;
+  float* part_x = workspace;
+  float* part_m = workspace + static_cast<size_t>(chunks) * (S + 1) * W;
+  first_layer_bwd_kernel<<<chunks, kBlock, 0, st>>>(g, x, m0, w_neigh, gm, part_x, part_m, m, rpc);
+  if (jobs != nullptr) {
+    jobs->push_back(FinishJob{part_x, gw_self, g_bias, (S + 1) * W, chunks, W, S, 1});
+    jobs->push_back(FinishJob{part_m, gw_neigh, nullptr, S * W, chunks, W, S, 1});
+    return launch_status();
+  }
+  skinny_sum_kernel<<<((S + 1) * W + 15) / 16, kBlock, 0, st>>>(part_x, gw_self, g_bias, S + 1, S, W, chunks, 1);
+  skinny_sum_kernel<<<(S * W + 15) / 16, kBlock, 0, st>>>(part_m, gw_neigh, nullptr, S, S, W, chunks, 1);
+  return launch_status();
 }
+
+}
+
+int first_layer_bwd_partials(const float* g, const float* x, const float* m0, const float* w_neigh, float* gm, float* gw_self,
+                             float* g_bias, float* gw_neigh, float* workspace, int64_t m, hipStream_t st,
+                             std::vector<FinishJob>* jobs) {
+  if (!g || !x || !m0 || !w_neigh || !gm || !gw_self || !g_bias || !gw_neigh || !workspace || !jobs) return GTS_ERR_NULL;
+  if (!first_layer_shape(m, kFirstW, kFirstS, kFirstS)) return GTS_ERR_SHAPE;
+  return first_layer_bwd_run(g, x, m0, w_neigh, gm, gw_self, g_bias, gw_neigh, workspace, m, st, jobs);
+}
+
 }
 
 extern "C" int64_t gts_sage_first_layer_bwd_workspace(int64_t m, int64_t w, int64_t s0, int64_t s1) {
@@ -105,14 +133,6 @@
   if (!g || !x || !m0 || !w_neigh || !gm || !gw_self || !g_bias || !gw_neigh || !workspace) return GTS_ERR_NULL;
   if (!first_layer_shape(m, w, s0, s1)) return GTS_ERR_SHAPE;
   if (workspace_bytes < gts_sage_first_layer_bwd_workspace(m, w, s0, s1)) return GTS_ERR_SHAPE;
-  hipStream_t st = static_cast<hipStream_t>(stream);
-  const int64_t rpc = (m + kSkinnyChunks - 1) / kSkinnyChunks;
-  const int chunks = static_cast<int>((m + rpc - 1) / rpc);
-  const int W = kFirstW, S = kFirstS;
-  float* part_x = workspace;
-  float* part_m = workspace + static_cast<size_t>(chunks) * (S + 1) * W;
-  first_layer_bwd_kernel<<<chunks, kBlock, 0, st>>>(g, x, m0, w_neigh, gm, part_x, part_m, m, rpc);
-  skinny_sum_kernel<<<((S + 1) * W + 15) / 16, kBlock, 0, st>>>(part_x, gw_self, g_bias, S + 1, S, W, chunks, 1);
-  skinny_sum_kernel<<<(S * W + 15) / 16, kBlock, 0, st>>>(part_m, gw_neigh, nullptr, S, S, W, chunks, 1);
-  return launch_status();
+  return first_layer_bwd_run(g, x, m0, w_neigh, gm, gw_self, g_bias, gw_neigh, workspace, m, static_cast<hipStream_t>(stream),
+                             nullptr);
 }
diff --git a/gnn-tumor-seg_amd/csrc/gts_optim.hip b/gnn-tumor-seg_amd/csrc/gts_optim.hip
--- a/gnn-tumor-seg_amd/csrc/gts_optim.hip
+++ b/gnn-tumor-seg_amd/csrc/gts_optim.hip
@@ -1,3 +1,6 @@
+#include <algorithm>
+#include <cstddef>
+
 #include "gts_common.h"
 
 namespace gts {
@@ -49,17 +52,105 @@
     adamw_one(param[i], grad[i], exp_avg[i], exp_avg_sq[i], c);
 }
 
-}
-}
-
-extern "C" int32_t gts_adamw_f32(float* param, const float* grad, float* exp_avg, float* exp_avg_sq,
-                                 int64_t n, double lr, double beta1, double beta2, double eps,
-                                 double weight_decay, int64_t step, void* stream) {
-  using namespace gts;
-  if (n < 0 || step < 1 || !(beta1 >= 0.0 && beta1 < 1.0) || !(beta2 >= 0.0 && beta2 < 1.0))
-    return GTS_ERR_SHAPE;
-  if (n == 0) return GTS_OK;
-  if (!param || !grad || !exp_avg || !exp_avg_sq) return GTS_ERR_NULL;
+constexpr int kMaxFormMats = 32;
+constexpr int kFormTileRows = 16, kFormTileCols = 64;
+
+struct FormsArgs {
+  long long mat_off[kMaxFormMats];
+  int rows[kMaxFormMats], cols[kMaxFormMats];
+  float* packed[kMaxFormMats];
+  float* t_plain[kMaxFormMats];
+  float* t_packed[kMaxFormMats];
+  long long gap_a[kMaxFormMats + 1], gap_b[kMaxFormMats + 1];
+  int n_mats;
+};
+
+__global__ __launch_bounds__(kBlock) void adamw_forms_kernel(const FormsArgs f, float* __restrict__ param,
+                                                            const float* __restrict__ grad, float* __restrict__ exp_avg,
+                                                            float* __restrict__ exp_avg_sq, AdamWConsts c) {
+  const int job = blockIdx.y;
+  if (job >= f.n_mats) {
+    const int gap = job - f.n_mats;
+    const long long a = kernarg_entry<long long>(offsetof(FormsArgs, gap_a), gap);
+    const long long b = kernarg_entry<long long>(offsetof(FormsArgs, gap_b), gap);
+    for (long long q = a / 4 + static_cast<long long>(blockIdx.x) * kBlock + threadIdx.x; 4 * q < b;
+         q += static_cast<long long>(gridDim.x) * kBlock) {
+      if (4 * q >= a && 4 * q + 4 <= b) {
+        v4f p = reinterpret_cast<v4f*>(param)[q];
+        const v4f g = reinterpret_cast<const v4f*>(grad)[q];
+        v4f m = reinterpret_cast<v4f*>(exp_avg)[q];
+        v4f v = reinterpret_cast<v4f*>(exp_avg_sq)[q];
+#pragma unroll
+        for (int e = 0; e < 4; ++e) {
+          float pe = p[e], me = m[e], ve = v[e];
+          adamw_one(pe, g[e], me, ve, c);
+          p[e] = pe, m[e] = me, v[e] = ve;
+        }
+        reinterpret_cast<v4f*>(param)[q] = p;
+        reinterpret_cast<v4f*>(exp_avg)[q] = m;
+        reinterpret_cast<v4f*>(exp_avg_sq)[q] = v;
+      } else {
+        for (long long i = max(a, 4 * q); i < min(b, 4 * q + 4); ++i) adamw_one(param[i], grad[i], exp_avg[i], exp_avg_sq[i], c);
+      }
+    }
+    return;
+  }
+  __shared__ float tile[kFormTileRows][kFormTileCols + 1];
+  const long long off = kernarg_entry<long long>(offsetof(FormsArgs, mat_off), job);
+  const int rows = kernarg_entry<int>(offsetof(FormsArgs, rows), job);
+  const int cols = kernarg_entry<int>(offsetof(FormsArgs, cols), job);
+  float* packed = kernarg_entry<float*>(offsetof(FormsArgs, packed), job);
+  float* t_plain = kernarg_entry<float*>(offsetof(FormsArgs, t_plain), job);
+  float* t_packed = kernarg_entry<float*>(offsetof(FormsArgs, t_packed), job);
+  const int tiles_c = (cols + kFormTileCols - 1) / kFormTileCols;
+  const int tiles = ((rows + kFormTileRows - 1) / kFormTileRows) * tiles_c;
+  if (static_cast<int>(blockIdx.x) >= tiles) return;
+  const int r0 = (blockIdx.x / tiles_c) * kFormTileRows, c0 = (blockIdx.x % tiles_c) * kFormTileCols;
+  {
+    const int tr = threadIdx.x >> 4, tc = 4 * (threadIdx.x & 15);
+    const int row = r0 + tr, col = c0 + tc;
+    if (row < rows && col < cols) {
+      const long long q = (off + static_cast<long long>(row) * cols + col) >> 2;
+      v4f p = reinterpret_cast<v4f*>(param)[q];
+      const v4f g = reinterpret_cast<const v4f*>(grad)[q];
+      v4f m = reinterpret_cast<v4f*>(exp_avg)[q];
+      v4f v = reinterpret_cast<v4f*>(exp_avg_sq)[q];
+#pragma unroll
+      for (int e = 0; e < 4; ++e) {
+        float pe = p[e], me = m[e], ve = v[e];
+        adamw_one(pe, g[e], me, ve, c);
+        p[e] = pe, m[e] = me, v[e] = ve;
+      }
+      reinterpret_cast<v4f*>(param)[q] = p;
+      reinterpret_cast<v4f*>(exp_avg)[q] = m;
+      reinterpret_cast<v4f*>(exp_avg_sq)[q] = v;
+      if (packed != nullptr) {
+        const size_t at = (static_cast<size_t>(row >> 4) * ((cols + 15) >> 4) + (col >> 4)) * 64 + (row & 15) + 16 * ((col & 15) >> 2);
+        reinterpret_cast<v4f*>(packed)[at] = p;
+      }
+#pragma unroll
+      for (int e = 0; e < 4; ++e) tile[tr][tc + e] = p[e];
+    }
+  }
+  if (t_plain == nullptr && t_packed == nullptr) return;
+  __syncthreads();
+  const int col = c0 + (threadIdx.x >> 2), r4 = threadIdx.x & 3, row = r0 + 4 * r4;
+  if (col >= cols || row >= rows) return;
+  v4f t;
+#pragma unroll
+  for (int e = 0; e < 4; ++e) t[e] = tile[4 * r4 + e][col - c0];
+  if (t_plain != nullptr) *reinterpret_cast<v4f*>(t_plain + static_cast<size_t>(col) * rows + row) = t;
+  if (t_packed != nullptr) {
+    const size_t at = (static_cast<size_t>(col >> 4) * ((rows + 15) >> 4) + (row >> 4)) * 64 + (col & 15) + 16 * r4;
+    reinterpret_cast<v4f*>(t_packed)[at] = t;
+  }
+}
+
+inline bool bad_adamw(int64_t n, int64_t step, double beta1, double beta2) {
+  return n < 0 || step < 1 || !(beta1 >= 0.0 && beta1 < 1.0) || !(beta2 >= 0.0 && beta2 < 1.0);
+}
+
+inline AdamWConsts adamw_consts(double lr, double beta1, double beta2, double eps, double weight_decay, int64_t step) {
   const double bc1 = 1.0 - pow(beta1, static_cast<double>(step));
   const double bc2 = 1.0 - pow(beta2, static_cast<double>(step));
   AdamWConsts c;
@@ -70,6 +161,20 @@
   c.step_size = static_cast<float>(lr / bc1);
   c.inv_bc2_sqrt_den = static_cast<float>(sqrt(bc2));
   c.eps = static_cast<float>(eps);
+  return c;
+}
+
+}
+}
+
+extern "C" int32_t gts_adamw_f32(float* param, const float* grad, float* exp_avg, float* exp_avg_sq,
+                                 int64_t n, double lr, double beta1, double beta2, double eps,
+                                 double weight_decay, int64_t step, void* stream) {
+  using namespace gts;
+  if (bad_adamw(n, step, beta1, beta2)) return GTS_ERR_SHAPE;
+  if (n == 0) return GTS_OK;
+  if (!param || !grad || !exp_avg || !exp_avg_sq) return GTS_ERR_NULL;
+  const AdamWConsts c = adamw_consts(lr, beta1, beta2, eps, weight_decay, step);
   const int vector_ok = ((reinterpret_cast<uintptr_t>(param) | reinterpret_cast<uintptr_t>(grad) |
                           reinterpret_cast<uintptr_t>(exp_avg) | reinterpret_cast<uintptr_t>(exp_avg_sq)) & 15) == 0;
   int64_t blocks = (n / 4 + kBlock - 1) / kBlock;
@@ -78,3 +183,58 @@
       param, grad, exp_avg, exp_avg_sq, n, c, vector_ok);
   return launch_status();
 }
+
+extern "C" int32_t gts_adamw_forms_f32(float* param, const float* grad, float* exp_avg, float* exp_avg_sq, int64_t n,
+                                       double lr, double beta1, double beta2, double eps, double weight_decay, int64_t step,
+                                       const int64_t* mat_offset, const int64_t* mat_rows, const int64_t* mat_cols,
+                                       float* const* packed, float* const* t_plain, float* const* t_packed, int32_t n_mats,
+                                       void* stream) {
+  using namespace gts;
+  if (n_mats < 0) return GTS_ERR_SHAPE;
+  if (n_mats == 0) return gts_adamw_f32(param, grad, exp_avg, exp_avg_sq, n, lr, beta1, beta2, eps, weight_decay, step, stream);
+  if (bad_adamw(n, step, beta1, beta2)) return GTS_ERR_SHAPE;
+  if (!param || !grad || !exp_avg || !exp_avg_sq || !mat_offset || !mat_rows || !mat_cols) return GTS_ERR_NULL;
+  auto misaligned = [](const void* p) { return (reinterpret_cast<uintptr_t>(p) & 15) != 0; };
+  if (misaligned(param) || misaligned(grad) || misaligned(exp_avg) || misaligned(exp_avg_sq)) return GTS_ERR_SHAPE;
+  int64_t end = 0;
+  for (int q = 0; q < n_mats; ++q) {
+    const int64_t off = mat_offset[q], rows = mat_rows[q], cols = mat_cols[q];
+    if (rows <= 0 || cols <= 0 || rows >= (1 << 20) || cols >= (1 << 20) || off < end || off + rows * cols > n) return GTS_ERR_SHAPE;
+    if ((off | rows | cols) & 3) return GTS_ERR_SHAPE;
+    if ((packed && misaligned(packed[q])) || (t_plain && misaligned(t_plain[q])) || (t_packed && misaligned(t_packed[q])))
+      return GTS_ERR_SHAPE;
+    end = off + rows * cols;
+  }
+  const AdamWConsts c = adamw_consts(lr, beta1, beta2, eps, weight_decay, step);
+  hipStream_t st = static_cast<hipStream_t>(stream);
+  int64_t from = 0;
+  for (int first = 0; first < n_mats; first += kMaxFormMats) {
+    const int count = n_mats - first < kMaxFormMats ? n_mats - first : kMaxFormMats;
+    const bool last = first + count == n_mats;
+    FormsArgs f{};
+    f.n_mats = count;
+    int64_t blocks = 1, at = from;
+    int gaps = 0;
+    auto gap = [&](int64_t a, int64_t b) {
+      if (a >= b) return;
+      f.gap_a[gaps] = a, f.gap_b[gaps] = b, ++gaps;
+      blocks = std::max(blocks, std::min<int64_t>(64, ((b + 3) / 4 - a / 4 + kBlock - 1) / kBlock));
+    };
+    for (int q = 0; q < count; ++q) {
+      const int64_t off = mat_offset[first + q], rows = mat_rows[first + q], cols = mat_cols[first + q];
+      gap(at, off);
+      f.mat_off[q] = off, f.rows[q] = static_cast<int>(rows), f.cols[q] = static_cast<int>(cols);
+      f.packed[q] = packed ? packed[first + q] : nullptr;
+      f.t_plain[q] = t_plain ? t_plain[first + q] : nullptr;
+      f.t_packed[q] = t_packed ? t_packed[first + q] : nullptr;
+      blocks = std::max(blocks, ((rows + kFormTileRows - 1) / kFormTileRows) * ((cols + kFormTileCols - 1) / kFormTileCols));
+      at = off + rows * cols;
+    }
+    if (last) gap(at, n);
+    from = at;
+    if (blocks >= (1LL << 31)) return GTS_ERR_SHAPE;
+    adamw_forms_kernel<<<dim3(static_cast<unsigned>(blocks), static_cast<unsigned>(count + gaps)), kBlock, 0, st>>>(
+        f, param, grad, exp_avg, exp_avg_sq, c);
+  }
+  return launch_status();
+}
diff --git a/gnn-tumor-seg_amd/csrc/gts_stack.hip b/gnn-tumor-seg_amd/csrc/gts_stack.hip
--- a/gnn-tumor-seg_amd/csrc/gts_stack.hip
+++ b/gnn-tumor-seg_amd/csrc/gts_stack.hip
@@ -62,7 +62,13 @@
   int64_t wtp[kMaxLayers][3];
   int64_t g[kMaxLayers], gp[kMaxLayers];
   int64_t gm[2];
-  int64_t workspace, workspace_bytes;
+  struct Partials {
+    int64_t rows, cols;
+    int first;
+    int64_t at, bytes;
+  };
+  std::vector<Partials> wgrad_ws;
+  int64_t first_ws;
   bool first_fused;
   int64_t counters;
   int64_t total;
@@ -103,16 +109,17 @@
   }
   p.gm[0] = take(4 * n * widest);
   p.gm[1] = take(4 * n * widest);
-  int64_t ws = 0;
   if (n > 0)
     for (const auto& grp : wgrads.groups)
-      for (int first = 0; first < grp.count(); first += gts::kMaxProblems)
-        ws = std::max(ws, gts_linear_bwd_weight_workspace(n, grp.rows, grp.cols, std::min(gts::kMaxProblems, grp.count() - first)));
+      for (int first = 0; first < grp.count(); first += gts::kMaxProblems) {
+        int64_t bytes = 0;
+        for (int count = 1; count <= std::min(gts::kMaxProblems, grp.count() - first); ++count)
+          bytes = std::max(bytes, gts::wgrad_partials_workspace(n, grp.rows, grp.cols, count));
+        p.wgrad_ws.push_back({grp.rows, grp.cols, first, take(bytes), bytes});
+      }
   const int64_t first = n > 0 ? gts_sage_first_layer_bwd_workspace(n, w[1], w[0], w[0]) : 0;
   p.first_fused = first > 0;
-  ws = std::max(ws, first);
-  p.workspace_bytes = ws;
-  p.workspace = take(ws);
+  p.first_ws = take(first);
   p.counters = take(4 * GTS_CLUSTER_COUNTER_WORDS);
   p.total = at;
   return p;
@@ -147,12 +154,12 @@
   return p.total;
 }
 
-extern "C" int32_t gts_sage_pool_stack_fwd_f32(const int32_t* indptr, const int32_t* indices, const int32_t* sched_rec,
-                                               int64_t sched_clusters, int32_t sched_rows, int32_t sched_srcs,
-                                               int32_t sched_loc_words, const float* x, const float* const* params,
-                                               int64_t n_rows, const int64_t* widths, int32_t n_layers, int32_t training,
-                                               int32_t arg_bytes, int32_t relu_bits, void* arena, int64_t arena_bytes,
-                                               void* stream) {
+extern "C" int32_t gts_sage_pool_stack_fwd_forms_f32(const int32_t* indptr, const int32_t* indices, const int32_t* sched_rec,
+                                                     int64_t sched_clusters, int32_t sched_rows, int32_t sched_srcs,
+                                                     int32_t sched_loc_words, const float* x, const float* const* params,
+                                                     int64_t n_rows, const int64_t* widths, int32_t n_layers,
+                                                     int32_t training, int32_t arg_bytes, int32_t relu_bits, void* arena,
+                                                     int64_t arena_bytes, const float* const* packed_forms, void* stream) {
   if (!indptr || !x || !params || !arena) return GTS_ERR_NULL;
   if (bad_stack(n_rows, widths, n_layers)) return GTS_ERR_SHAPE;
   if (training && arg_bytes != 1 && arg_bytes != 4) return GTS_ERR_ARGKIND;
@@ -166,16 +173,19 @@
   auto f32 = [&](int64_t off) { return reinterpret_cast<float*>(base + off); };
   uint32_t* counters;
   GTS_TRY(zero_counters(sched_rec, sched_clusters, sched_rows, sched_srcs, sched_loc_words, 0, base + plan.counters, stream, &counters));
+  auto given = [&](int i, int q) -> const float* { return packed_forms != nullptr ? packed_forms[3 * i + q] : nullptr; };
   {
     ByShape packs;
     for (int i = 0; i < n_layers; ++i)
       for (int q = 0; q < 3; ++q)
-        if (plan.wp[i][q] >= 0)
+        if (plan.wp[i][q] >= 0 && given(i, q) == nullptr)
           packs.add(weight_rows(widths, i, q), widths[i], params[5 * i + kWeightSlot[q]], nullptr, f32(plan.wp[i][q]), nullptr);
     for (const auto& b : packs.groups)
       GTS_TRY(gts_pack_weights_f32(b.in[0].data(), b.out[0].data(), nullptr, b.count(), b.rows, b.cols, 0, stream));
   }
-  auto wp = [&](int i, int q) -> const float* { return plan.wp[i][q] >= 0 ? f32(plan.wp[i][q]) : nullptr; };
+  auto wp = [&](int i, int q) -> const float* {
+    return plan.wp[i][q] < 0 ? nullptr : given(i, q) != nullptr ? given(i, q) : f32(plan.wp[i][q]);
+  };
   const float* h = x;
   float* p = nullptr;
   int cur = 0;
@@ -219,19 +229,31 @@
   return GTS_OK;
 }
 
+extern "C" int32_t gts_sage_pool_stack_fwd_f32(const int32_t* indptr, const int32_t* indices, const int32_t* sched_rec,
+                                               int64_t sched_clusters, int32_t sched_rows, int32_t sched_srcs,
+                                               int32_t sched_loc_words, const float* x, const float* const* params,
+                                               int64_t n_rows, const int64_t* widths, int32_t n_layers, int32_t training,
+                                               int32_t arg_bytes, int32_t relu_bits, void* arena, int64_t arena_bytes,
+                                               void* stream) {
+  return gts_sage_pool_stack_fwd_forms_f32(indptr, indices, sched_rec, sched_clusters, sched_rows, sched_srcs, sched_loc_words, x,
+                                           params, n_rows, widths, n_layers, training, arg_bytes, relu_bits, arena, arena_bytes,
+                                           nullptr, stream);
+}
+
 extern "C" int64_t gts_sage_pool_stack_bwd_scratch(int64_t n_rows, const int64_t* widths, int32_t n_layers,
                                                    int32_t ) {
   if (bad_stack(n_rows, widths, n_layers)) return -1;
   return plan_backward(n_rows, widths, n_layers).total;
 }
 
-extern "C" int32_t gts_sage_pool_stack_bwd_f32(const int32_t* t_indptr, const int32_t* t_indices, const int32_t* t_slot,
-                                               const int32_t* sched_rec, int64_t sched_clusters, int32_t sched_rows,
-                                               int32_t sched_srcs, int32_t sched_loc_words, const float* gout, const float* x,
-                                               const float* const* params, int64_t n_rows, const int64_t* widths,
-                                               int32_t n_layers, int32_t arg_bytes, int32_t relu_bits, const void* fwd_arena,
-                                               float* const* grads, float* gx, void* scratch, int64_t scratch_bytes,
-                                               void* stream) {
+extern "C" int32_t gts_sage_pool_stack_bwd_forms_f32(const int32_t* t_indptr, const int32_t* t_indices, const int32_t* t_slot,
+                                                     const int32_t* sched_rec, int64_t sched_clusters, int32_t sched_rows,
+                                                     int32_t sched_srcs, int32_t sched_loc_words, const float* gout,
+                                                     const float* x, const float* const* params, int64_t n_rows,
+                                                     const int64_t* widths, int32_t n_layers, int32_t arg_bytes,
+                                                     int32_t relu_bits, const void* fwd_arena, float* const* grads, float* gx,
+                                                     void* scratch, int64_t scratch_bytes, const float* const* t_plain_forms,
+                                                     const float* const* t_packed_forms, void* stream) {
   if (!t_indptr || !gout || !x || !params || !fwd_arena || !grads || !scratch) return GTS_ERR_NULL;
   if (bad_stack(n_rows, widths, n_layers)) return GTS_ERR_SHAPE;
   if (arg_bytes != 1 && arg_bytes != 4) return GTS_ERR_ARGKIND;
@@ -258,18 +280,26 @@
   auto act = [&](int64_t off) { return reinterpret_cast<const float*>(acts + off); };
   auto input_of = [&](int i) { return i == 0 ? x : act(fwd.out[i - 1]); };
 
+  auto given = [&](int i, int q) {
+    return t_plain_forms != nullptr && t_packed_forms != nullptr && t_plain_forms[3 * i + q] != nullptr &&
+           t_packed_forms[3 * i + q] != nullptr;
+  };
   {
     ByShape turned;
     for (int i = 0; i < n_layers; ++i)
       for (int q = 0; q < 3; ++q)
-        if (plan.wt[i][q] >= 0)
+        if (plan.wt[i][q] >= 0 && !given(i, q))
           turned.add(weight_rows(widths, i, q), widths[i], params[5 * i + kWeightSlot[q]], nullptr, f32(plan.wt[i][q]),
                      f32(plan.wtp[i][q]));
     for (const auto& b : turned.groups)
       GTS_TRY(gts_pack_weights_f32(b.in[0].data(), b.out[1].data(), b.out[0].data(), b.count(), b.rows, b.cols, 1, stream));
   }
-  auto wt = [&](int i, int q) -> const float* { return plan.wt[i][q] >= 0 ? f32(plan.wt[i][q]) : nullptr; };
-  auto wtp = [&](int i, int q) -> const float* { return plan.wtp[i][q] >= 0 ? f32(plan.wtp[i][q]) : nullptr; };
+  auto wt = [&](int i, int q) -> const float* {
+    return plan.wt[i][q] < 0 ? nullptr : given(i, q) ? t_plain_forms[3 * i + q] : f32(plan.wt[i][q]);
+  };
+  auto wtp = [&](int i, int q) -> const float* {
+    return plan.wtp[i][q] < 0 ? nullptr : given(i, q) ? t_packed_forms[3 * i + q] : f32(plan.wtp[i][q]);
+  };
 
   auto igrad = [&](const float* g0, const float* w0, const float* w0t, int64_t n0, const float* g1, const float* w1,
                    const float* w1t, int64_t n1, const float* relu_mask, const uint64_t* relu_bits, float* gin,
@@ -283,6 +313,7 @@
   };
 
   ByShape wgrads;
+  std::vector<gts::FinishJob> sums;
 
   const float* g = gout;
   const float* gm = nullptr;
@@ -299,8 +330,8 @@
     const bool lowrank = i == n_layers - 1 && gm == nullptr && fout == 4 && fin == 256 && arg_bytes == 1;
     if (fused) {
       float* buf = f32(plan.gm[cur]);
-      GTS_TRY(gts_sage_first_layer_bwd_f32(g, h, m, w_neigh, buf, grads[2], grads[4], grads[3], f32(plan.workspace),
-                                           plan.workspace_bytes, n_rows, fout, fin, fin, stream));
+      GTS_TRY(gts::first_layer_bwd_partials(g, h, m, w_neigh, buf, grads[2], grads[4], grads[3], f32(plan.first_ws), n_rows, st,
+                                            &sums));
       gm = buf;
     } else if (gm == nullptr && !lowrank) {
       float* buf = f32(plan.gm[cur]);
@@ -342,9 +373,27 @@
     }
   }
   for (const auto& grp : wgrads.groups)
-    for (int first = 0; first < grp.count(); first += gts::kMaxProblems)
-      GTS_TRY(gts_linear_bwd_weight_f32(grp.in[0].data() + first, grp.in[1].data() + first, grp.out[0].data() + first,
-                                        grp.out[1].data() + first, std::min(gts::kMaxProblems, grp.count() - first),
-                                        f32(plan.workspace), plan.workspace_bytes, n_rows, grp.rows, grp.cols, stream));
-  return GTS_OK;
-}
+    for (int first = 0; first < grp.count(); first += gts::kMaxProblems) {
+      const int count = std::min(gts::kMaxProblems, grp.count() - first);
+      const auto ws = std::find_if(plan.wgrad_ws.begin(), plan.wgrad_ws.end(), [&](const BwdPlan::Partials& r) {
+        return r.rows == grp.rows && r.cols == grp.cols && r.first == first;
+      });
+      if (ws == plan.wgrad_ws.end() || ws->bytes < gts::wgrad_partials_workspace(n_rows, grp.rows, grp.cols, count))
+        return GTS_ERR_SHAPE;
+      GTS_TRY(gts::wgrad_partials(grp.in[0].data() + first, grp.in[1].data() + first, grp.out[0].data() + first,
+                                  grp.out[1].data() + first, count, f32(ws->at), n_rows, grp.rows, grp.cols, st, &sums));
+    }
+  return gts::finish_sums(sums, st);
+}
+
+extern "C" int32_t gts_sage_pool_stack_bwd_f32(const int32_t* t_indptr, const int32_t* t_indices, const int32_t* t_slot,
+                                               const int32_t* sched_rec, int64_t sched_clusters, int32_t sched_rows,
+                                               int32_t sched_srcs, int32_t sched_loc_words, const float* gout, const float* x,
+                                               const float* const* params, int64_t n_rows, const int64_t* widths,
+                                               int32_t n_layers, int32_t arg_bytes, int32_t relu_bits, const void* fwd_arena,
+                                               float* const* grads, float* gx, void* scratch, int64_t scratch_bytes,
+                                               void* stream) {
+  return gts_sage_pool_stack_bwd_forms_f32(t_indptr, t_indices, t_slot, sched_rec, sched_clusters, sched_rows, sched_srcs,
+                                           sched_loc_words, gout, x, params, n_rows, widths, n_layers, arg_bytes, relu_bits,
+                                           fwd_arena, grads, gx, scratch, scratch_bytes, nullptr, nullptr, stream);
+}
diff --git a/gnn-tumor-seg_amd/gts/dist.py b/gnn-tumor-seg_amd/gts/dist.py
--- a/gnn-tumor-seg_amd/gts/dist.py
+++ b/gnn-tumor-seg_amd/gts/dist.py
@@ -108,6 +108,9 @@
     assert_same_layout(params)
     for p in params:
         dist.broadcast(p.data, src=src)
+    from . import nn as gnn
+
+    gnn.invalidate_weight_forms(params)
 
 
 class FlatGradSync:
diff --git a/gnn-tumor-seg_amd/gts/nn.py b/gnn-tumor-seg_amd/gts/nn.py
--- a/gnn-tumor-seg_amd/gts/nn.py
+++ b/gnn-tumor-seg_amd/gts/nn.py
@@ -1,4 +1,5 @@
 import os
+import weakref
 
 import torch
 import torch.nn as nn
@@ -298,6 +299,165 @@
     return hit
 
 
+WEIGHT_FORMS = os.environ.get("GTS_WEIGHT_FORMS", "1") != "0"
+_weight_forms = {}
+
+
+class WeightForms:
+
+    def __init__(self, params):
+        import ctypes
+
+        from . import _lib
+
+        lib = _lib.load()
+        self.refs = [weakref.ref(p) for p in params]
+        self.ptrs = [p.data_ptr() for p in params]
+        self.n_layers = len(params) // 5
+        dev = params[0].device
+        self.weights = []
+        self.packed, self.t_plain, self.t_packed = {}, {}, {}
+        wanted = []
+        for i in range(self.n_layers):
+            for q, j in enumerate((0, 2, 3)):
+                rows, cols = params[5 * i + j].shape
+                slot = 3 * i + q
+                self.weights.append((slot, 5 * i + j))
+                if rows > 128:
+                    wanted.append((self.packed, slot, lib.gts_packed_weight_floats(rows, cols), (-1,)))
+                if cols >= 128 and rows % 4 == 0 and cols % 4 == 0:
+                    wanted.append((self.t_plain, slot, rows * cols, (cols, rows)))
+                    wanted.append((self.t_packed, slot, lib.gts_packed_weight_floats(cols, rows), (-1,)))
+        self.buffer = torch.zeros(sum(k for _, _, k, _ in wanted), dtype=torch.float32, device=dev)
+        at = 0
+        for forms, slot, k, shape in wanted:
+            forms[slot] = self.buffer[at:at + k].view(*shape)
+            at += k
+        self.shapes = {slot: tuple(params[j].shape) for slot, j in self.weights}
+        self.unkept = set()
+        self.stamp = None
+        self.flat_ref = None
+        self._c_tables = None
+        self._optimizer_tables = {}
+        arr = ctypes.c_void_p
+        self._refresh = []
+        for forms, plain, transposed in ((self.packed, None, 0), (self.t_packed, self.t_plain, 1)):
+            by_shape = {}
+            for slot, j in self.weights:
+                if slot in forms:
+                    by_shape.setdefault(self.shapes[slot], []).append((slot, j))
+            for (rows, cols), members in by_shape.items():
+                k = len(members)
+                self._refresh.append(((arr * k)(*[params[j].data_ptr() for _, j in members]),
+                                      (arr * k)(*[forms[slot].data_ptr() for slot, _ in members]),
+                                      (arr * k)(*[plain[slot].data_ptr() for slot, _ in members]) if plain is not None else None,
+                                      k, rows, cols, transposed))
+
+    def params(self):
+        return [r() for r in self.refs]
+
+    def _stamp(self):
+        flat = self.flat_ref() if self.flat_ref is not None else None
+        stamp = [(p.data_ptr(), p._version) if p is not None else None for p in self.params()]
+        if flat is not None:
+            stamp.append((flat.data_ptr(), flat._version))
+        return stamp
+
+    def current(self, params):
+        return self.stamp is not None and all(r() is p for r, p in zip(self.refs, params)) and self.stamp == self._stamp()
+
+    def invalidate(self):
+        self.stamp = None
+
+    def mark_current(self):
+        self.stamp = self._stamp()
+
+    def refresh(self):
+        from . import _lib
+        from ._lib import check, current_stream
+
+        lib = _lib.load()
+        for src, dst, plain, k, rows, cols, transposed in self._refresh:
+            check(lib.gts_pack_weights_f32(src, dst, plain, k, rows, cols, transposed, current_stream()), "gts_pack_weights_f32")
+        self.mark_current()
+
+    def tables(self):
+        import ctypes
+
+        if self._c_tables is None:
+            def table(forms):
+                return (ctypes.c_void_p * (3 * self.n_layers))(*[
+                    forms[slot].data_ptr() if slot in forms and slot not in self.unkept else None
+                    for slot in range(3 * self.n_layers)])
+            self._c_tables = (table(self.packed), table(self.t_plain), table(self.t_packed))
+        return self._c_tables
+
+    def optimizer_table(self, flat):
+        import ctypes
+
+        key = flat.data_ptr()
+        if key not in self._optimizer_tables:
+            params, rows = self.params(), []
+            lo, hi = flat.data_ptr(), flat.data_ptr() + 4 * flat.numel()
+            table = None
+            if all(p is not None and lo <= p.data_ptr() and p.data_ptr() + 4 * p.numel() <= hi for p in params):
+                unkept = set()
+                for slot, j in self.weights:
+                    if slot not in self.packed and slot not in self.t_plain:
+                        continue
+                    off, (r, c) = (params[j].data_ptr() - lo) // 4, self.shapes[slot]
+                    if off % 4 or r % 4 or c % 4 or (params[j].data_ptr() - lo) % 4 or not params[j].is_contiguous():
+                        unkept.add(slot)
+                        continue
+                    rows.append((off, r, c, *[f[slot].data_ptr() if slot in f else None
+                                              for f in (self.packed, self.t_plain, self.t_packed)]))
+                rows.sort()
+                k = len(rows)
+                table = ((ctypes.c_int64 * k)(*[x[0] for x in rows]), (ctypes.c_int64 * k)(*[x[1] for x in rows]),
+                         (ctypes.c_int64 * k)(*[x[2] for x in rows]), (ctypes.c_void_p * k)(*[x[3] for x in rows]),
+                         (ctypes.c_void_p * k)(*[x[4] for x in rows]), (ctypes.c_void_p * k)(*[x[5] for x in rows]), k)
+                if unkept != self.unkept:
+                    self.unkept, self._c_tables = unkept, None
+            self._optimizer_tables = {key: table}
+        return self._optimizer_tables[key]
+
+
+def _forms_of(params, key):
+    forms = _weight_forms.get(key)
+    if forms is None:
+        if len(_weight_forms) >= 8:
+            _weight_forms.clear()
+        forms = _weight_forms[key] = WeightForms(params)
+    if not forms.current(params):
+        forms.refresh()
+    return forms
+
+
+def invalidate_weight_forms(params=None):
+    ids = None if params is None else {id(p) for p in params}
+    for forms in _weight_forms.values():
+        if ids is None or any(id(p) in ids for p in forms.params()):
+            forms.invalidate()
+
+
+def optimizer_forms(flat, params):
+    ids, kept = {id(p) for p in params}, []
+    for key, forms in list(_weight_forms.items()):
+        theirs = forms.params()
+        if any(p is None for p in theirs) or forms.ptrs != [p.data_ptr() for p in theirs]:
+            del _weight_forms[key]
+            continue
+        mine = [id(p) in ids for p in theirs]
+        if not any(mine):
+            continue
+        table = forms.optimizer_table(flat) if WEIGHT_FORMS and all(mine) else None
+        if table is None:
+            forms.invalidate()
+        else:
+            kept.append((forms, table))
+    return kept
+
+
 class _SagePoolStackCall(torch.autograd.Function):
 
     @staticmethod
@@ -319,14 +479,16 @@
             raise _lib.GtsError("gts_sage_pool_stack_fwd_arena rejected the stack's shape")
         arena = torch.empty(max(int(total), 16), dtype=torch.uint8, device=x.device)
         ds = ops._cluster_schedule(g, "in", n, 256, ab if need_bwd else 0) if 256 in widths[:-1] else None
-        check(lib.gts_sage_pool_stack_fwd_f32(
+        forms = _forms_of(params, (*table[:], *widths)) if WEIGHT_FORMS and n > 0 else None
+        check(lib.gts_sage_pool_stack_fwd_forms_f32(
             ptr(d.indptr), ptr(d.indices), *_DeviceSchedule.launch_args(ds), ptr(x), table, n, c_widths, n_layers,
-            1 if need_bwd else 0, ab, relu_bits, arena.data_ptr(), int(total), current_stream()),
-            "gts_sage_pool_stack_fwd_f32")
+            1 if need_bwd else 0, ab, relu_bits, arena.data_ptr(), int(total), forms.tables()[0] if forms else None,
+            current_stream()), "gts_sage_pool_stack_fwd_forms_f32")
         at = int(offsets[4 * (n_layers - 1) + 2])
         out = arena[at:at + 4 * n * widths[-1]].view(torch.float32).view(n, widths[-1])
         if need_bwd:
             ctx.g, ctx.widths, ctx.relu_bits, ctx.ab = g, widths, relu_bits, ab
+            ctx.forms = forms
             ctx.param_ids = [id(p) for p in params]
             ctx.save_for_backward(x, arena, *params)
         return out
@@ -363,10 +525,12 @@
         scratch = torch.empty(max(int(need), 16), dtype=torch.uint8, device=x.device)
         gx = torch.empty_like(x) if ctx.needs_input_grad[1] else None
         ds = ops._cluster_schedule(g, "out", n, 256, ab) if 256 in widths[:-1] else None
-        check(lib.gts_sage_pool_stack_bwd_f32(
+        forms = ctx.forms if ctx.forms is not None and WEIGHT_FORMS and ctx.forms.current(ctx.forms.params()) else None
+        check(lib.gts_sage_pool_stack_bwd_forms_f32(
             ptr(d.t_indptr), ptr(d.t_indices), ptr(d.t_slot), *_DeviceSchedule.launch_args(ds), ptr(gout), ptr(x), table, n,
             c_widths, n_layers, ab, relu_bits, arena.data_ptr(), grads, ptr(gx), scratch.data_ptr(), int(need),
-            current_stream()), "gts_sage_pool_stack_bwd_f32")
+            forms.tables()[1] if forms else None, forms.tables()[2] if forms else None, current_stream()),
+            "gts_sage_pool_stack_bwd_forms_f32")
         if sink is not None:
             sink.filled = True
             return (None, gx, None, *([None] * len(params)))
diff --git a/gnn-tumor-seg_amd/gts/optim.py b/gnn-tumor-seg_amd/gts/optim.py
--- a/gnn-tumor-seg_amd/gts/optim.py
+++ b/gnn-tumor-seg_amd/gts/optim.py
@@ -1,3 +1,5 @@
+import weakref
+
 import torch
 
 from . import _lib
@@ -52,9 +54,21 @@
             raise _lib.GtsError("flat_grad must be one contiguous fp32 tensor with one entry per parameter")
         group = self.param_groups[0]
         self.steps += 1
-        check(_lib.load().gts_adamw_f32(ptr(self.flat_param), ptr(flat_grad), ptr(self.exp_avg),
-                                        ptr(self.exp_avg_sq), self.n, float(group["lr"]),
-                                        float(group["betas"][0]), float(group["betas"][1]), float(group["eps"]),
-                                        float(group["weight_decay"]), self.steps, current_stream()),
-              "gts_adamw_f32")
+        from . import nn as gnn
+
+        lib = _lib.load()
+        args = (ptr(self.flat_param), ptr(flat_grad), ptr(self.exp_avg), ptr(self.exp_avg_sq), self.n, float(group["lr"]),
+                float(group["betas"][0]), float(group["betas"][1]), float(group["eps"]), float(group["weight_decay"]),
+                self.steps)
+        kept = gnn.optimizer_forms(self.flat_param, self._params) if gnn._weight_forms else []
+        for forms, _ in kept[1:]:
+            forms.invalidate()
+        if kept:
+            forms, (offsets, rows, cols, packed, t_plain, t_packed, n_mats) = kept[0]
+            check(lib.gts_adamw_forms_f32(*args, offsets, rows, cols, packed, t_plain, t_packed, n_mats, current_stream()),
+                  "gts_adamw_forms_f32")
+            forms.flat_ref = weakref.ref(self.flat_param)
+            forms.mark_current()
+        else:
+            check(lib.gts_adamw_f32(*args, current_stream()), "gts_adamw_f32")
         return loss
diff --git a/include/gts_hip.h b/include/gts_hip.h
--- a/include/gts_hip.h
+++ b/include/gts_hip.h
@@ -127,6 +127,11 @@
 int32_t gts_adamw_f32(float* param, const float* grad, float* exp_avg, float* exp_avg_sq, int64_t n,
                       double lr, double beta1, double beta2, double eps, double weight_decay,
                       int64_t step, void* stream);
+int32_t gts_adamw_forms_f32(float* param, const float* grad, float* exp_avg, float* exp_avg_sq, int64_t n,
+                            double lr, double beta1, double beta2, double eps, double weight_decay, int64_t step,
+                            const int64_t* mat_offset, const int64_t* mat_rows, const int64_t* mat_cols,
+                            float* const* packed, float* const* t_plain, float* const* t_packed, int32_t n_mats,
+                            void* stream);
 
 int64_t gts_label_confusion_workspace(int64_t n);
 int32_t gts_label_confusion_i16(const int16_t* pred, const int16_t* truth, int64_t* counts,
@@ -194,6 +199,20 @@
                                     int32_t n_layers, int32_t arg_bytes, int32_t relu_bits, const void* fwd_arena,
                                     float* const* grads, float* gx, void* scratch, int64_t scratch_bytes,
                                     void* stream);
+int32_t gts_sage_pool_stack_fwd_forms_f32(const int32_t* indptr, const int32_t* indices, const int32_t* sched_rec,
+                                          int64_t sched_clusters, int32_t sched_rows, int32_t sched_srcs,
+                                          int32_t sched_loc_words, const float* x, const float* const* params,
+                                          int64_t n_rows, const int64_t* widths, int32_t n_layers, int32_t training,
+                                          int32_t arg_bytes, int32_t relu_bits, void* arena, int64_t arena_bytes,
+                                          const float* const* packed_forms, void* stream);
+int32_t gts_sage_pool_stack_bwd_forms_f32(const int32_t* t_indptr, const int32_t* t_indices, const int32_t* t_slot,
+                                          const int32_t* sched_rec, int64_t sched_clusters, int32_t sched_rows,
+                                          int32_t sched_srcs, int32_t sched_loc_words, const float* gout, const float* x,
+                                          const float* const* params, int64_t n_rows, const int64_t* widths,
+                                          int32_t n_layers, int32_t arg_bytes, int32_t relu_bits, const void* fwd_arena,
+                                          float* const* grads, float* gx, void* scratch, int64_t scratch_bytes,
+                                          const float* const* t_plain_forms, const float* const* t_packed_forms,
+                                          void* stream);
 
 int64_t gts_weighted_ce_workspace(int64_t n);
 int32_t gts_weighted_ce_f32(const float* logits, const int64_t* labels, const float* class_w,
```

After: 980.0 graphs/s, median of 6. About the same (+0.7%).
